# michaelwillett/GPU-ICP-SLAM

Hardware: AMD Instinct MI355X
Metric: particle-scan evals/sec (1081 beams x N particles), full particleFilter step, KD path (higher is better)
Workload: dtype f32; 1 GPU; synthetic 1081-beam scans, 100000 particles/GPU, 100000-point KD map, full SLAM step (disperse+score+weights+ICP/SVD+map update+resample); particles_global=100000, parallelism=particles sharded x1, map replicated, kd_size_end=196248

## Files before the change

### gpu-icp-slam_amd/binding.py

```python
import ctypes as C
import os

import numpy as np

from . import build as _build

NODE_DTYPE = np.dtype(
    [("axis", "<i4"), ("left", "<i4"), ("right", "<i4"), ("parent", "<i4"),
     ("x", "<f4"), ("y", "<f4"), ("z", "<f4"), ("w", "<f4")])
PARTICLE_DTYPE = np.dtype(
    {"names": ["x", "y", "theta", "w", "cluster", "map"],
     "formats": ["<f4", "<f4", "<f4", "<f4", "u1", "<u8"],
     "offsets": [0, 4, 8, 12, 16, 24], "itemsize": 32})

SYMBOLS = [
    "pfslam_default_config", "pfslam_create", "pfslam_destroy", "pfslam_last_error", "pfslam_device_count",
    "pfslam_set_stream", "pfslam_synchronize", "pfslam_step", "pfslam_step_grid", "pfslam_shard_disperse", "pfslam_shard_score", "pfslam_shard_weights", "pfslam_shard_finish", "pfslam_shard_stream", "pfslam_get_pose", "pfslam_get_particles",
    "pfslam_get_map", "pfslam_get_grid", "pfslam_get_trace", "pfslam_get_cells", "pfslam_set_map",
    "pfslam_set_particles", "pfslam_shift_particles", "pfslam_set_scan", "pfslam_set_pose", "pfslam_set_grid", "pfslam_motion_update",
    "pfslam_score_kd", "pfslam_measurement_update", "pfslam_icp", "pfslam_update_map_kd", "pfslam_resample",
    "pfslam_score_grid", "pfslam_update_map_grid", "pfslam_traverse", "pfslam_measurement_local",
    "pfslam_measurement_apply", "pfslam_device_ptr", "pfslam_time_score_kd", "pfslam_set_variant", "pfslam_set_lag",
    "pfslam_kd_create", "pfslam_kd_insert_list", "pfslam_kd_insert_node", "pfslam_kd_balance", "pfslam_set_timing", "pfslam_get_timers", "pfslam_resample_plan", "pfslam_resample_gather", "pfslam_maybe_balance", "pfslam_kd_size", "pfslam_topology_update", "pfslam_find_walls",
    "pfslam_check_loop_closure", "pfslam_get_topology", "pfslam_set_topology", "pfslam_get_closures", "pfslam_score_census", "pfslam_set_census", "pfslam_get_census_log", "pfslam_ubench_gather", "pfslam_plan_stats", "pfslam_cell_stats", "pfslam_kd_parallel_sort", "pfslam_kd_sort_threads", "pfslam_kd_whole_node",
    "pfslam_set_serial", "pfslam_set_trig", "pfslam_debug_check_cells", "pfslam_set_probe", "pfslam_get_probe", "pfslam_probe_name", "pfslam_frame_mode",
    "pfslam_time_score_grid", "pfslam_set_shard_balance", "pfslam_shard_balance_due", "pfslam_shard_balance_build", "pfslam_shard_balance_adopt",
]


class Config(C.Structure):
    _fields_ = [("n_particles", C.c_int32), ("n_beams", C.c_int32),
                ("map_scale_x", C.c_float), ("map_scale_y", C.c_float),
                ("map_res_x", C.c_float), ("map_res_y", C.c_float),
                ("kd_capacity", C.c_int32), ("device", C.c_int32),
                ("strict_host_mirror", C.c_int32), ("free_upload_bug", C.c_int32),
                ("balance_period", C.c_int32), ("global_offset", C.c_int32), ("global_n", C.c_int32),
                ("shard_stride", C.c_int32), ("reserved_", C.c_int32 * 2)]


class PfSlamError(RuntimeError):
    pass


_lib = None


def _one_hip_runtime():
    import importlib.util
    import sys
    if "torch" in sys.modules or os.environ.get("PFSLAM_NO_TORCH_HIP"):
        return
    try:
        spec = importlib.util.find_spec("torch")
    except Exception:
        spec = None
    if spec is None or not spec.origin:
        return
    cand = os.path.join(os.path.dirname(spec.origin), "lib", "libamdhip64.so")
    if os.path.exists(cand):
        try:
            C.CDLL(cand, mode=C.RTLD_GLOBAL)
        except OSError:
            pass


def load():
    global _lib
    if _lib is not None:
        return _lib
    path = os.environ.get("PFSLAM_LIB") or _build.LIB
    try:
        if path == _build.LIB and _build.stale():
            _build.build()
    except Exception as e:
        if not os.path.exists(path):
            raise PfSlamError("libpfslam_hip.so is missing and could not be built: %s" % e)
    _one_hip_runtime()
    L = C.CDLL(path)
    vp, i32, f32 = C.c_void_p, C.c_int, C.c_float
    L.pfslam_last_error.restype = C.c_char_p
    L.pfslam_default_config.restype = None
    L.pfslam_default_config.argtypes = [vp]
    L.pfslam_create.argtypes = [vp, vp]
    L.pfslam_destroy.argtypes = [vp]
    L.pfslam_set_stream.argtypes = [vp, vp]
    L.pfslam_synchronize.argtypes = [vp]
    L.pfslam_step.argtypes = [vp, i32, vp]
    L.pfslam_step_grid.argtypes = [vp, i32, vp]
    L.pfslam_shard_disperse.argtypes = [vp, i32, vp, vp]
    L.pfslam_shard_score.argtypes = [vp]
    L.pfslam_shard_weights.argtypes = [vp]
    L.pfslam_shard_finish.argtypes = [vp]
    L.pfslam_shard_stream.argtypes = [vp, i32, vp]
    L.pfslam_time_score_grid.argtypes = [vp, i32, vp, vp]
    L.pfslam_set_shard_balance.argtypes = [vp, i32]
    L.pfslam_shard_balance_due.argtypes = [vp, i32, vp, vp]
    L.pfslam_shard_balance_build.argtypes = [vp, i32]
    L.pfslam_shard_balance_adopt.argtypes = [vp]
    L.pfslam_get_pose.argtypes = [vp, vp]
    L.pfslam_get_particles.argtypes = [vp, vp, vp]
    L.pfslam_get_map.argtypes = [vp, vp, vp]
    L.pfslam_get_grid.argtypes = [vp, vp, vp, vp]
    L.pfslam_get_trace.argtypes = [vp, vp]
    L.pfslam_get_cells.argtypes = [vp, i32, vp, i32, vp]
    L.pfslam_set_map.argtypes = [vp, vp, i32]
    L.pfslam_set_particles.argtypes = [vp, vp, i32]
    L.pfslam_set_scan.argtypes = [vp, vp, i32]
    L.pfslam_shift_particles.argtypes = [vp, vp]
    L.pfslam_set_pose.argtypes = [vp, vp]
    L.pfslam_set_grid.argtypes = [vp, vp, i32, i32]
    L.pfslam_motion_update.argtypes = [vp, i32]
    L.pfslam_score_kd.argtypes = [vp, vp]
    L.pfslam_measurement_update.argtypes = [vp, vp, vp, vp]
    L.pfslam_icp.argtypes = [vp, vp, vp, vp]
    L.pfslam_update_map_kd.argtypes = [vp]
    L.pfslam_resample.argtypes = [vp, i32, vp, vp]
    L.pfslam_resample_plan.argtypes = [vp, i32, vp, vp]
    L.pfslam_resample_gather.argtypes = [vp]
    L.pfslam_maybe_balance.argtypes = [vp, i32]
    L.pfslam_kd_size.argtypes = [vp]
    L.pfslam_topology_update.argtypes = [vp, vp]
    L.pfslam_find_walls.argtypes = [vp, vp, vp, vp]
    L.pfslam_check_loop_closure.argtypes = [vp, vp, i32, vp]
    L.pfslam_get_topology.argtypes = [vp, vp, i32, vp, vp]
    L.pfslam_set_topology.argtypes = [vp, i32]
    L.pfslam_get_closures.argtypes = [vp, vp, i32, vp]
    L.pfslam_score_census.argtypes = [vp, vp]
    L.pfslam_set_census.argtypes = [vp, i32]
    L.pfslam_get_census_log.argtypes = [vp, vp, i32, vp]
    L.pfslam_ubench_gather.argtypes = [vp, vp]
    L.pfslam_plan_stats.argtypes = [vp, vp]
    L.pfslam_cell_stats.argtypes = [vp, vp]
    L.pfslam_set_serial.argtypes = [vp, i32]
    L.pfslam_set_trig.argtypes = [vp, i32]
    L.pfslam_debug_check_cells.argtypes = [vp, vp]
    L.pfslam_set_probe.argtypes = [vp, i32]
    L.pfslam_get_probe.argtypes = [vp, vp, i32, vp, vp]
    L.pfslam_frame_mode.argtypes = [vp, vp]
    L.pfslam_probe_name.argtypes = [i32]
    L.pfslam_probe_name.restype = C.c_char_p
    L.pfslam_score_grid.argtypes = [vp, vp]
    L.pfslam_update_map_grid.argtypes = [vp]
    L.pfslam_traverse.argtypes = [vp, vp, i32, vp]
    L.pfslam_measurement_local.argtypes = [vp]
    L.pfslam_measurement_apply.argtypes = [vp, vp, vp, vp]
    L.pfslam_device_ptr.argtypes = [vp, i32, vp, vp]
    L.pfslam_time_score_kd.argtypes = [vp, i32, vp]
    L.pfslam_set_variant.argtypes = [vp, i32]
    L.pfslam_set_lag.argtypes = [vp, i32]
    L.pfslam_kd_create.argtypes = [vp, i32, vp]
    L.pfslam_kd_insert_node.argtypes = [vp, vp, i32]
    L.pfslam_kd_insert_list.argtypes = [vp, i32, vp, i32, i32]
    L.pfslam_kd_balance.argtypes = [vp, i32]
    L.pfslam_debug_math.argtypes = [vp, i32, vp, i32, vp]
    L.pfslam_set_timing.argtypes = [vp, i32]
    L.pfslam_get_timers.argtypes = [vp, vp]
    _lib = L
    return L


def _p(a):
    return a.ctypes.data_as(C.c_void_p)


def _chk(rc, what=""):
    if rc != 0:
        raise PfSlamError("%s failed: %s" % (what, load().pfslam_last_error().decode()))


def device_count():
    return load().pfslam_device_count()


def kd_create(points_xyzw):
    pts = np.ascontiguousarray(points_xyzw, dtype=np.float32).reshape(-1, 4)
    out = np.zeros(len(pts), dtype=NODE_DTYPE)
    _chk(load().pfslam_kd_create(_p(pts), len(pts), _p(out)), "pfslam_kd_create")
    return out


def kd_insert_node(nodes, size, p4):
    p = np.ascontiguousarray(p4, dtype=np.float32)
    _chk(load().pfslam_kd_insert_node(_p(p), _p(nodes), size), "pfslam_kd_insert_node")


def kd_balance(nodes, size):
    _chk(load().pfslam_kd_balance(_p(nodes), size), "pfslam_kd_balance")


MGPU_SYMBOLS = ["pfslam_mgpu_make_id", "pfslam_mgpu_create", "pfslam_mgpu_destroy", "pfslam_mgpu_step", "pfslam_mgpu_barrier_max",
                "pfslam_mgpu_stats", "pfslam_mgpu_time_collectives", "pfslam_mgpu_last_error"]
MGPU_ID_BYTES = 256
_mgpu = None


def load_mgpu():
    global _mgpu
    if _mgpu is not None:
        return _mgpu
    load()
    path = os.path.join(os.path.dirname(os.path.abspath(__file__)), "host", "libpfslam_mgpu.so")
    if not os.path.exists(path):
        import subprocess
        subprocess.check_call(["make", "-C", os.path.dirname(path), "libpfslam_mgpu.so"], stdout=subprocess.DEVNULL)
    M = C.CDLL(path, mode=C.RTLD_GLOBAL)
    vp, i32 = C.c_void_p, C.c_int32
    M.pfslam_mgpu_last_error.restype = C.c_char_p
    M.pfslam_mgpu_make_id.argtypes = [vp]
    M.pfslam_mgpu_create.argtypes = [vp, i32, i32, vp, vp]
    M.pfslam_mgpu_destroy.argtypes = [vp]
    M.pfslam_mgpu_step.argtypes = [vp, i32, vp]
    M.pfslam_mgpu_barrier_max.argtypes = [vp, vp]
    M.pfslam_mgpu_stats.argtypes = [vp, vp]
    M.pfslam_mgpu_time_collectives.argtypes = [vp, i32, vp]
    _mgpu = M
    return M


# ... 182 lines not shown
        return did.value, neff.value

    def maybe_balance(self, frame):
        _chk(self.L.pfslam_maybe_balance(self._h, frame), "pfslam_maybe_balance")

    @property
    def kd_size(self):
        return self.L.pfslam_kd_size(self._h)

    def topology_update(self):
        n = C.c_int()
        _chk(self.L.pfslam_topology_update(self._h, C.byref(n)), "pfslam_topology_update")
        return n.value

    def find_walls(self, a_xy, b_xy):
        a = np.ascontiguousarray(a_xy, np.float32); b = np.ascontiguousarray(b_xy, np.float32)
        n = C.c_int()
        _chk(self.L.pfslam_find_walls(self._h, _p(a), _p(b), C.byref(n)), "pfslam_find_walls")
        return n.value

    def check_loop_closure(self, cap=4096):
        pairs = np.zeros((cap, 2), np.int32)
        n = C.c_int()
        _chk(self.L.pfslam_check_loop_closure(self._h, _p(pairs), cap, C.byref(n)), "pfslam_check_loop_closure")
        return pairs[:min(n.value, cap)].copy()

    def set_topology(self, enable=True):
        _chk(self.L.pfslam_set_topology(self._h, int(enable)), "pfslam_set_topology")

    def closures(self, cap=65536):
        pairs = np.zeros((cap, 2), np.int32)
        n = C.c_int()
        _chk(self.L.pfslam_get_closures(self._h, _p(pairs), cap, C.byref(n)), "pfslam_get_closures")
        return pairs[:min(n.value, cap)].copy()

    def topology(self, cap=4096):
        nodes = np.zeros((cap, 3), np.float32)
        n, idx = C.c_int(), C.c_int()
        _chk(self.L.pfslam_get_topology(self._h, _p(nodes), cap, C.byref(n), C.byref(idx)), "pfslam_get_topology")
        return nodes[:n.value].copy(), idx.value

    def score_census(self):
        out = (C.c_ulonglong * 8)()
        _chk(self.L.pfslam_score_census(self._h, out), "pfslam_score_census")
        return {"trips": int(out[0]), "visits": int(out[1]), "tests": int(out[2]), "test_lanes": int(out[3]),
                "uniform_trips": int(out[4]), "prefix_trips": int(out[5]), "redescents": int(out[6]), "redescents_noop": int(out[7])}

    def set_census(self, enable=True):
        _chk(self.L.pfslam_set_census(self._h, int(enable)), "pfslam_set_census")

    def census_log(self, cap=1024):
        out = np.zeros((cap, 8), np.uint64)
        n = C.c_int()
        _chk(self.L.pfslam_get_census_log(self._h, _p(out), cap, C.byref(n)), "pfslam_get_census_log")
        keys = ("trips", "visits", "tests", "test_lanes", "uniform_trips", "prefix_trips", "redescents", "redescents_noop")
        return [dict(zip(keys, (int(v) for v in row))) for row in out[:min(n.value, cap)]]

    def plan_stats(self):
        out = (C.c_double * 10)()
        _chk(self.L.pfslam_plan_stats(self._h, out), "pfslam_plan_stats")
        keys = ("rows", "path_len", "candidates", "frac_complete", "frac_no_plan", "frac_full", "box_dx", "box_dy", "box_dtheta", "waves")
        return dict(zip(keys, [float(v) for v in out]))

    def cell_stats(self):
        out = (C.c_double * 16)()
        _chk(self.L.pfslam_cell_stats(self._h, out), "pfslam_cell_stats")
        keys = ("cells", "rows", "candidates", "redescent_candidates", "cells_without_row", "pool_slots", "window_kx", "window_ky",
                "walked_from_root", "extended", "reused", "claimed", "flags", "updates", "wipes", "suspended")
        return dict(zip(keys, [float(v) for v in out]))

    def set_serial(self, on):
        _chk(self.L.pfslam_set_serial(self._h, int(on)), "pfslam_set_serial")

    def check_cells(self):
        out = (C.c_longlong * 16)()
        _chk(self.L.pfslam_debug_check_cells(self._h, out), "pfslam_debug_check_cells")
        keys = ("records", "unwalked", "fresh", "published", "row_words", "pending_words", "fallback_words", "dead",
                "v_unwalked_not_pending", "v_unpublished_word", "v_row_outside_alloc", "v_row_not_candidate", "v_watched_link_has_child",
                "v_bad_link", "v_dead_has_row", "v_counters")
        d = dict(zip(keys, [int(v) for v in out]))
        d["violations"] = sum(v for k, v in d.items() if k.startswith("v_"))
        return d

    def set_trig(self, devlib):
        _chk(self.L.pfslam_set_trig(self._h, 1 if devlib else 0), "pfslam_set_trig")

    def frame_mode(self):
        out = (C.c_int * 4)()
        _chk(self.L.pfslam_frame_mode(self._h, out), "pfslam_frame_mode")
        return {"round5_frame": bool(out[0]), "gates": bool(out[1]), "serial": bool(out[2]), "publish_lag": int(out[3])}

    def set_probe(self, frames):
        _chk(self.L.pfslam_set_probe(self._h, int(frames)), "pfslam_set_probe")

    def probe(self, frames=4096):
        buf = np.zeros((frames, 32), np.uint64)
        n, last = C.c_int(0), C.c_int(0)
        _chk(self.L.pfslam_get_probe(self._h, _p(buf), frames, C.byref(n), C.byref(last)), "pfslam_get_probe")
        names = []
        for k in range(32):
            s = self.L.pfslam_probe_name(k).decode()
            if not s:
                break
            names.append(s)
        t = buf[:n.value, :len(names)].astype(np.float64) * 0.01
        return names, t, last.value

    def ubench_gather(self):
        out = (C.c_double * 4)()
        _chk(self.L.pfslam_ubench_gather(self._h, out), "pfslam_ubench_gather")
        return {"wave_gathers_per_s": out[0], "cus": int(out[1]), "nominal_ghz": out[2], "cycles_per_wave_gather": out[3]}

    def resample_plan(self, frame):
        did, neff = C.c_int(), C.c_float()
        _chk(self.L.pfslam_resample_plan(self._h, frame, C.byref(did), C.byref(neff)), "pfslam_resample_plan")
        return did.value, neff.value

    def resample_gather(self):
        _chk(self.L.pfslam_resample_gather(self._h), "pfslam_resample_gather")

    def score_grid(self):
        fit = np.empty(self.n, np.int32)
        _chk(self.L.pfslam_score_grid(self._h, _p(fit)), "pfslam_score_grid")
        return fit

    def update_map_grid(self):
        _chk(self.L.pfslam_update_map_grid(self._h), "pfslam_update_map_grid")

    def step(self, frame, scan):
        scan = np.ascontiguousarray(scan, dtype=np.float32)
        _chk(self.L.pfslam_step(self._h, frame, _p(scan)), "pfslam_step")

    def shard_disperse(self, frame, scan):
        scan = np.ascontiguousarray(scan, dtype=np.float32)
        seeded = C.c_int(0)
        _chk(self.L.pfslam_shard_disperse(self._h, frame, _p(scan), C.byref(seeded)), "pfslam_shard_disperse")
        return bool(seeded.value)

    def shard_score(self):
        _chk(self.L.pfslam_shard_score(self._h), "pfslam_shard_score")

    def shard_weights(self):
        _chk(self.L.pfslam_shard_weights(self._h), "pfslam_shard_weights")

    def shard_finish(self):
        _chk(self.L.pfslam_shard_finish(self._h), "pfslam_shard_finish")

    def shard_stream(self, which):
        st = C.c_void_p(0)
        _chk(self.L.pfslam_shard_stream(self._h, which, C.byref(st)), "pfslam_shard_stream")
        return st.value or 0

    def set_shard_balance(self, external):
        _chk(self.L.pfslam_set_shard_balance(self._h, 1 if external else 0), "pfslam_set_shard_balance")

    def shard_balance_due(self, frame):
        due, n = C.c_int(0), C.c_int(0)
        _chk(self.L.pfslam_shard_balance_due(self._h, frame, C.byref(due), C.byref(n)), "pfslam_shard_balance_due")
        return bool(due.value), n.value

    def shard_balance_build(self, frame):
        _chk(self.L.pfslam_shard_balance_build(self._h, frame), "pfslam_shard_balance_build")

    def shard_balance_adopt(self):
        _chk(self.L.pfslam_shard_balance_adopt(self._h), "pfslam_shard_balance_adopt")

# ... 62 lines not shown
```

### gpu-icp-slam_amd/csrc/kd_cells.hip.inc

```

#define PF_CELL_SUB 2
#define PF_CELL_WIN (2560 * PF_CELL_SUB)
#define PF_CELL_LIST_CAP (1 << 19)
#define PF_CELL_POOL_CAP (1 << 22)
#define PF_CELL_MAXC 12
#define PF_CELL_RUN 32
#define PF_CELL_MAXR 14
#define PF_CELL_MARK_MAX 4096
#define PF_CELL_PENDING 0xFFFFFFFFu
#define PF_CELL_FALLBACK 0xFFFFFFFEu
enum { PF_CS_COUNT = 0, PF_CS_POOL, PF_CS_SNAP, PF_CS_PAD3, PF_CS_LIST_CAP, PF_CS_POOL_CAP, PF_CS_FLAGS, PF_CS_PAD, PF_CS_ROWS, PF_CS_N1, PF_CS_N2,
       PF_CS_NONE, PF_CS_CUR_FRESH, PF_CS_CUR_EXT, PF_CS_CUR_REUSED, PF_CS_CUR_CLAIMED, PF_CS_WORDS = 32,
       PF_CS_OX = 128, PF_CS_OY = 129, PF_CS_ALLOC = 256 };
#define PF_CF_LIST_FULL 1
#define PF_CF_POOL_FULL 2
#define PF_CF_NEED_ORIGIN 4
#define PF_CF_FAR 8
#define PF_CELL_DRIFT_MAX 120
#define PF_REC_WORDS 96
#define PF_REC_TERM 4
#define PF_REC_CAND 20
#define PF_REC_PAR 36
#define PF_REC_RC 52
#define PF_REC_POOL 76
#define PF_REC_LAST 80
#define PF_ROW_HEADROOM 2
#define PF_RF_FRESH 1
#define PF_RF_DEAD 2
#define PF_RF_ROVER 4

struct CellGeom { float resx, resy, invx, invy; };

__device__ __forceinline__ void pf_stamp(unsigned long long *__restrict__ slot)
{
    if (slot && blockIdx.x == 0 && blockIdx.y == 0 && threadIdx.x == 0) *slot = wall_clock64();
}

#define PF_LATTICE_KMAX (1 << 20)
__host__ __device__ __forceinline__ int lattice_floor(float q, float res, float inv)
{
    int k = (int)floorf(q * inv);
    if ((float)(k + 1) * res <= q) k++;
    else if (!((float)k * res <= q)) k--;
    return k;
}

__host__ __device__ __forceinline__ int sub_index(float q, float res, float inv)
{
    const int k = lattice_floor(q, res, inv);
    const float mid = (float)k * res + 0.5f * res;
    return PF_CELL_SUB * k + (q >= mid ? 1 : 0);
}
#define PF_SUB_MARGIN 3e-7f
__device__ __forceinline__ int sub_index_fast(float q, float inv2, float &clear)
{
    const float t = q * inv2;
    int k;
    asm("v_cvt_flr_i32_f32 %0, %1" : "=v"(k) : "v"(t));
    const float fr = __builtin_amdgcn_fractf(t);
    clear = __builtin_fmaf(fabsf(t), -PF_SUB_MARGIN, 0.5f - 1e-6f) - fabsf(fr - 0.5f);
    return k;
}
__host__ __device__ __forceinline__ void sub_edges(int S, float res, float &lo, float &hi, float &cell_lo)
{
    const int k = S >> 1;
    cell_lo = (float)k * res;
    const float mid = cell_lo + 0.5f * res;
    lo = (S & 1) ? mid : cell_lo;
    hi = (S & 1) ? (float)(k + 1) * res : mid;
}
static_assert(PF_CELL_SUB == 2, "sub_index / sub_edges halve the lattice cell");

__device__ __forceinline__ bool beam_box(const pf::KdGroupBox &b, int j, float r, float &wxlo, float &wxhi, float &wylo, float &wyhi,
                                         const pf::AngleParts *T = nullptr, const pf::BeamParts *beams = nullptr)
{
    const float tc = 0.5f * (b.tlo + b.thi), dth = 0.5f * (b.thi - b.tlo);
    float cx, cy;
    if (T) beam_end_point(beams, j, r, tc, *T, cx, cy);
    else pf::clean_lidar_scan(j, r, tc, cx, cy);
    const float dd = dth + 1e-6f;
    const float eps = 2e-4f + 1e-5f * fabsf(r) + fabsf(r) * 2.0f * 1.1920929e-7f * (fabsf(tc) + 2.4f + dd);
    const float hx = (fabsf(cy) + fabsf(r) * dd) * dd + eps, hy = (fabsf(cx) + fabsf(r) * dd) * dd + eps;
    wxlo = b.xlo + cx - hx; wxhi = b.xhi + cx + hx; wylo = b.ylo + cy - hy; wyhi = b.yhi + cy + hy;
    return (wxlo == wxlo) && (wxhi == wxhi) && (wylo == wylo) && (wyhi == wyhi) && fabsf(wxlo) < 1e6f && fabsf(wxhi) < 1e6f &&
           fabsf(wylo) < 1e6f && fabsf(wyhi) < 1e6f && (wxhi - wxlo) < 4.0f && (wyhi - wylo) < 4.0f && fabsf(r) < PF_RANGE_NEVER;
}

#define PF_MARK_THREADS 256
#define PF_MARK_GROUPS 8
#define PF_MARK_CLAIMS 2048
#define PF_MARK_WORDS 4096
__global__ __launch_bounds__(PF_MARK_THREADS) void k_cells_mark(const pf::KdGroupBox *__restrict__ box, int groups,
                                                                const float *__restrict__ scan, int nb, CellGeom geo, unsigned *tab,
                                                                int *__restrict__ list, int *cs, const pf::AngleParts *__restrict__ gparts,
                                                                const pf::BeamParts *__restrict__ beams, unsigned long long *__restrict__ probe = nullptr)
{
    pf_stamp(probe);
    __shared__ unsigned bm[PF_MARK_WORDS];
    __shared__ int s_red[4][PF_MARK_THREADS / 64];
    const int t = threadIdx.x, lane = t & 63, wave = t >> 6, j = blockIdx.x;
    const int ox = cs[PF_CS_OX], oy = cs[PF_CS_OY];
    const float r = scan[j];
    int kx0[PF_MARK_GROUPS], kx1[PF_MARK_GROUPS], ky0[PF_MARK_GROUPS], ky1[PF_MARK_GROUPS];
    int ux0 = INT_MAX, ux1 = INT_MIN, uy0 = INT_MAX, uy1 = INT_MIN;
#pragma unroll
    for (int q = 0; q < PF_MARK_GROUPS; q++) {
        const int g = blockIdx.y * (PF_MARK_THREADS * PF_MARK_GROUPS) + q * PF_MARK_THREADS + t;
        kx0[q] = ky0[q] = INT_MAX;
        kx1[q] = ky1[q] = INT_MIN;
// ... 13 lines not shown
    }
    for (int off = 32; off >= 1; off >>= 1) {
        ux0 = min(ux0, __shfl_xor(ux0, off, 64)); ux1 = max(ux1, __shfl_xor(ux1, off, 64));
        uy0 = min(uy0, __shfl_xor(uy0, off, 64)); uy1 = max(uy1, __shfl_xor(uy1, off, 64));
    }
    if (lane == 0) { s_red[0][wave] = ux0; s_red[1][wave] = ux1; s_red[2][wave] = uy0; s_red[3][wave] = uy1; }
    __syncthreads();
    for (int k = 0; k < PF_MARK_THREADS / 64; k++) {
        ux0 = min(ux0, s_red[0][k]); ux1 = max(ux1, s_red[1][k]); uy0 = min(uy0, s_red[2][k]); uy1 = max(uy1, s_red[3][k]);
    }
    if (ux0 > ux1) return;
    const int nx = ux1 - ux0 + 1;
    const long long bits = (long long)nx * (uy1 - uy0 + 1);
    __shared__ int s_claim[PF_MARK_CLAIMS];
    __shared__ int s_nclaim, s_base;
    if (t == 0) s_nclaim = 0;
    __syncthreads();
    auto claim = [&](int idx) {
        if (atomicCAS(&tab[idx], 0u, PF_CELL_PENDING) == 0u) {
            const int k = atomicAdd(&s_nclaim, 1);
            if (k < PF_MARK_CLAIMS) s_claim[k] = idx;
            else {
                const int pos = atomicAdd(&cs[PF_CS_COUNT], 1);
                if (pos < cs[PF_CS_LIST_CAP]) list[pos] = idx;
                else {
                    atomicExch(&tab[idx], PF_CELL_FALLBACK);
                    atomicOr(&cs[PF_CS_FLAGS], PF_CF_LIST_FULL);
                }
            }
        }
    };
    auto flush = [&]() {
        __syncthreads();
        const int nc = min(s_nclaim, PF_MARK_CLAIMS);
        if (t == 0 && nc > 0) {
            s_base = atomicAdd(&cs[PF_CS_COUNT], nc);
            atomicAdd(&cs[PF_CS_CUR_CLAIMED], nc);
        }
        __syncthreads();
        for (int k = t; k < nc; k += PF_MARK_THREADS) {
            const int pos = s_base + k;
            if (pos < cs[PF_CS_LIST_CAP]) list[pos] = s_claim[k];
            else {
                atomicExch(&tab[s_claim[k]], PF_CELL_FALLBACK);
                atomicOr(&cs[PF_CS_FLAGS], PF_CF_LIST_FULL);
            }
        }
    };
    if (bits > (long long)PF_MARK_WORDS * 32) {
#pragma unroll
        for (int q = 0; q < PF_MARK_GROUPS; q++) {
            if (kx0[q] > kx1[q] || (long long)(kx1[q] - kx0[q] + 1) * (ky1[q] - ky0[q] + 1) > PF_CELL_MARK_MAX) continue;
            for (int cy = ky0[q]; cy <= ky1[q]; cy++)
                for (int cx = kx0[q]; cx <= kx1[q]; cx++) claim(2 * cy * PF_CELL_WIN + 2 * cx);
        }
        flush();
        return;
    }
    const int words = (int)((bits + 31) >> 5);
    for (int w = t; w < words; w += PF_MARK_THREADS) bm[w] = 0u;
    __syncthreads();
#pragma unroll
    for (int q = 0; q < PF_MARK_GROUPS; q++)
        for (int cy = ky0[q]; cy <= ky1[q]; cy++) {
            const int b0 = (cy - uy0) * nx - ux0 + kx0[q], b1 = b0 + (kx1[q] - kx0[q]);
            for (int w = b0 >> 5; w <= (b1 >> 5); w++) {
                const int lo = max(b0 - (w << 5), 0), hi = min(b1 - (w << 5), 31);
                const unsigned m = (0xFFFFFFFFu >> (31 - hi)) & (0xFFFFFFFFu << lo);
                if ((bm[w] & m) != m) atomicOr(&bm[w], m);
            }
        }
    __syncthreads();
    for (int bit = t; bit < (int)bits; bit += PF_MARK_THREADS)
        if ((bm[bit >> 5] >> (bit & 31)) & 1u) {
            const int cy = bit / nx;
            claim(2 * (uy0 + cy) * PF_CELL_WIN + 2 * (ux0 + (bit - cy * nx)));
        }
    flush();
}

#define PF_CORNER_F 0.999996f
#define PF_CELL_MAXU 16
#define PF_CELL_MAXRU 24
static_assert(PF_REC_RC + PF_CELL_MAXRU <= PF_REC_POOL && PF_REC_POOL + 2 <= PF_REC_LAST && PF_REC_LAST + 4 <= PF_REC_WORDS && PF_REC_CAND == PF_REC_TERM + PF_CELL_MAXU && PF_REC_PAR == PF_REC_CAND + PF_CELL_MAXU && PF_REC_RC == PF_REC_PAR + PF_CELL_MAXU, "record layout");
__device__ __forceinline__ int link_child(const pf::KdView &t, int link)
{
    const int a = link >> 1;
    const uint4 nd = t.hot[a];
    if ((link & 1) == 0 && t.planar && (nd.z >> 30) == 2u) return __float_as_int(t.z[a]);
    return (link & 1) ? (int)nd.w : pf::hot_left(nd.z);
}
#define PF_CELL_FILTER_WORDS 1024
__device__ __forceinline__ unsigned pf_link_hash(int link) { return ((unsigned)link * 2654435761u) >> 17; }
__device__ __forceinline__ int watched_child(const pf::KdView &t, int link)
{
    const uint4 nd = t.hot[link >> 1];
    return (link & 1) ? (int)nd.w : pf::hot_left(nd.z);
}
#ifdef PF_CELLS_PROFILE
#define PF_STAMP(p)                                                                      \
    do {                                                                                 \
        if (PUBLISH) {                                                                   \
            const long long now_ = (long long)wall_clock64();                            \
            if (lane == 0) {                                                             \
                atomicAdd(&cs[64 + 2 * (p)], (int)(now_ - t_prev_));                     \
                atomicMax(&cs[65 + 2 * (p)], (int)(now_ - t_prev_));                     \
            }                                                                            \
            t_prev_ = now_;                                                              \
        }                                                                                \
    } while (0)
#else
#define PF_STAMP(p)
#endif
struct CellPass { const int *lo; int *w_out; const int *hi; const int *bound; int fault; };
template <bool PUBLISH>
__global__ __launch_bounds__(64) void k_cells_update(pf::KdView tree, CellGeom geo, unsigned *tab, const int *__restrict__ list, int *cs,
                                                     uint4 *__restrict__ pool, int *rec_base, int gen, const int *__restrict__ touched, int pass = 0, int recut = 0, int use_snap = 0,
                                                     CellPass cp = CellPass{nullptr, nullptr, nullptr, nullptr, 0}, unsigned long long *__restrict__ probe = nullptr,
                                                     int *__restrict__ signal_word = nullptr, int signal_ticket = 0)
{
    pf_stamp(probe);
    if (signal_word && blockIdx.x == 0 && threadIdx.x == 0) __hip_atomic_store(signal_word, signal_ticket, __ATOMIC_RELEASE, __HIP_MEMORY_SCOPE_AGENT);
    __shared__ int lds[184][64];
#define S_IDX(k) lds[(k)][lane]
#define S_LB(k) (*(float *)&lds[32 + (k)][lane])
#define S_CX(k) (*(float *)&lds[16 + (k)][lane])
#define S_CY(k) (*(float *)&lds[32 + (k)][lane])
#define S_PP(k) (*(uint32_t *)&lds[48 + (k)][lane])
#define S_PC(k) (*(float *)&lds[64 + (k)][lane])
#define S_CT(k) lds[80 + (k)][lane]
#define S_PI(k) lds[96 + (k)][lane]
#define S_R(k) lds[112 + (k)][lane]
#define S_RX(k) (*(float *)&lds[136 + (k)][lane])
#define S_RY(k) (*(float *)&lds[160 + (k)][lane])
    static_assert(PF_CELL_RUN == 32 && PF_CELL_MAXU == 16 && PF_CELL_MAXRU == 24, "LDS layout of k_cells_update");
    __shared__ unsigned s_filter[PF_CELL_FILTER_WORDS];
    const int n_touched = (PUBLISH && touched) ? touched[0] : 0;
    if (PUBLISH && n_touched > 0) {
        for (int w = threadIdx.x; w < PF_CELL_FILTER_WORDS; w += 64) s_filter[w] = 0u;
        __syncthreads();
        for (int k = threadIdx.x; k < n_touched; k += 64) {
            const unsigned hsh = pf_link_hash(touched[1 + k]);
            atomicOr(&s_filter[hsh >> 5], 1u << (hsh & 31));
        }
        __syncthreads();
    }
    auto maybe_touched = [&](int link) -> bool {
        const unsigned hsh = pf_link_hash(link);
        return (s_filter[hsh >> 5] >> (hsh & 31)) & 1u;
    };
    const int lane = threadIdx.x;
    int count = min(cs[PF_CS_COUNT], cs[PF_CS_LIST_CAP]);
    if ((!PUBLISH || use_snap == 2) && threadIdx.x == 0) cs[PF_CS_SNAP] = count;
    if (PUBLISH && use_snap == 1) count = min(count, cs[PF_CS_SNAP]);
    if (PUBLISH && cp.hi && cp.fault != 1) count = min(count, *cp.hi);
    const int first = (!PUBLISH && cp.lo) ? min(*cp.lo, count) : 0;
    const int bound = cp.bound ? *cp.bound : 0x7fffffff;
    if (cp.w_out && threadIdx.x == 0) *cp.w_out = count;
    const int ox = cs[PF_CS_OX], oy = cs[PF_CS_OY];
    int st_rows = 0, st_n1 = 0, st_n2 = 0, st_none = 0, st_fresh = 0, st_ext = 0, st_reused = 0;
#ifdef PF_CELLS_PROFILE
    long long t_prev_ = (long long)wall_clock64();
    const long long t_start_ = t_prev_;
    if (PUBLISH && lane == 0 && blockIdx.x * 64 < count) atomicAdd(&cs[63], 1);
#endif
    auto bounds = [](float xlo, float xhi, float ylo, float yhi, float nx, float ny, float &lb, float &ub) {
        const float dxn = fmaxf(fmaxf(xlo - nx, nx - xhi), 0.0f), dyn = fmaxf(fmaxf(ylo - ny, ny - yhi), 0.0f);
        const float dxf = fmaxf(fabsf(nx - xlo), fabsf(nx - xhi)), dyf = fmaxf(fabsf(ny - ylo), fabsf(ny - yhi));
        lb = (dxn * dxn + dyn * dyn) * 0.99999f;
        ub = (dxf * dxf + dyf * dyf) * 1.00001f;
    };
    auto corner4 = [](float px, float py, float ixlo, float ixhi, float iylo, float iyhi, float d[4]) {
        const float x0 = (px - ixlo) * (px - ixlo), x1 = (px - ixhi) * (px - ixhi), y0 = (py - iylo) * (py - iylo), y1 = (py - iyhi) * (py - iyhi);
        d[0] = x0 + y0; d[1] = x1 + y0; d[2] = x0 + y1; d[3] = x1 + y1;
    };
    auto unbook = [&](unsigned old) {
        if (old == PF_CELL_FALLBACK) st_none--;
        else if (old != 0u && old < 0x40000000u) {
            st_rows--;
            st_n1 -= (int)(old & 15u);
            st_n2 -= ((old >> 4) & 15u) == 15u ? 0 : (int)((old >> 4) & 15u);
        }
    };
    for (int base = first + blockIdx.x * 64; base < count; base += gridDim.x * 64) {
        const int r = base + lane;
        const bool in = r < count;
        int *rec = rec_base + (size_t)(in ? r : 0) * PF_REC_WORDS;
        const int4 hd = in ? *(const int4 *)rec : make_int4(0, 0, 0, gen);
        int4 pre_ct[4], pre_cand[4], pre_par[4], pre_rc[6];
        int2 pre_pool = make_int2(0, 0);
        int4 pre_last = make_int4(0, 0, 0, 0);
        int pre_cell = 0;
        constexpr bool HOIST = PUBLISH;
        if (HOIST) {
#pragma unroll
            for (int q = 0; q < 4; q++) pre_ct[q] = pre_cand[q] = pre_par[q] = make_int4(-1, -1, -1, -1);
#pragma unroll
            for (int q = 0; q < 6; q++) pre_rc[q] = make_int4(0, 0, 0, 0);
            if (in) {
#pragma unroll
                for (int q = 0; q < 4; q++) {
                    pre_ct[q] = *(const int4 *)(rec + PF_REC_TERM + 4 * q);
                    pre_cand[q] = *(const int4 *)(rec + PF_REC_CAND + 4 * q);
                    pre_par[q] = *(const int4 *)(rec + PF_REC_PAR + 4 * q);
                }
#pragma unroll
                for (int q = 0; q < 6; q++) pre_rc[q] = *(const int4 *)(rec + PF_REC_RC + 4 * q);
                pre_pool = *(const int2 *)(rec + PF_REC_POOL);
                pre_last = *(const int4 *)(rec + PF_REC_LAST);
                pre_cell = list[r];
            }
        }
        const bool scratch = in && hd.w != gen;
        bool work = scratch;
        int m_old = 0, nr = 0, rflags = 0, term0 = -1, child0 = -1;
        float U = INFINITY;
        if (PUBLISH && in && !scratch) {
            U = __int_as_float(hd.x);
            term0 = hd.y;
            m_old = hd.z & 0xff;
            nr = (hd.z >> 8) & 0xff;
            rflags = hd.z >> 16;
            if (!(rflags & PF_RF_DEAD)) {
                int ct[PF_CELL_MAXU];
#pragma unroll
                for (int q = 0; q < PF_CELL_MAXU / 4; q++) {
                    const int4 v = HOIST ? pre_ct[q] : *(const int4 *)(rec + PF_REC_TERM + 4 * q);
                    ct[4 * q] = v.x; ct[4 * q + 1] = v.y; ct[4 * q + 2] = v.z; ct[4 * q + 3] = v.w;
                }
                const bool direct = (rflags & PF_RF_FRESH) != 0 && cp.fault != 2;
                bool changed = false;
                if (direct || n_touched > 0) {
                    if (direct || maybe_touched(term0)) child0 = watched_child(tree, term0);
                    changed = child0 >= 0;
                }
#pragma unroll
                for (int k = 0; k < PF_CELL_MAXU; k++)
                    if (k < m_old) {
                        int c = -1;
                        if (ct[k] >= 0 && (direct || (n_touched > 0 && maybe_touched(ct[k])))) c = watched_child(tree, ct[k]);
                        S_CT(k) = c >= 0 ? -c - 2 : ct[k];
                        changed |= c >= 0;
                    }
                work = changed || (rflags & PF_RF_FRESH) != 0 || recut != 0;
                if (changed && !(rflags & PF_RF_FRESH)) st_ext++;
                if (!work) st_reused++;
            }
        }
        PF_STAMP(0);
        if (__builtin_amdgcn_ballot_w64(work) == 0ull) continue;
        const bool active = in && work;
        if (!active) m_old = nr = 0;
        if (active && scratch) st_fresh++;
        const int cell = HOIST ? pre_cell : (in ? list[r] : 0);
        const int cyw = cell / PF_CELL_WIN, cxw = cell - cyw * PF_CELL_WIN;
        const int Kx = (ox + cxw) >> 1, Ky = (oy + cyw) >> 1;
        const float cxlo = (float)Kx * geo.resx, cxhi = (float)(Kx + 1) * geo.resx, xmid = cxlo + 0.5f * geo.resx;
        const float cylo = (float)Ky * geo.resy, cyhi = (float)(Ky + 1) * geo.resy, ymid = cylo + 0.5f * geo.resy;
        int n = 0, old_off = 0, old_len = 0;
        if (active && !scratch) {
            old_off = HOIST ? pre_pool.x : rec[PF_REC_POOL];
            old_len = recut ? 0 : (HOIST ? pre_pool.y : rec[PF_REC_POOL + 1]);
#pragma unroll
            for (int g4 = 0; g4 < PF_CELL_MAXU / 4; g4++) {
                const int k0 = 4 * g4;
                if (k0 < m_old) {
                    const int4 ci = HOIST ? pre_cand[g4] : *(const int4 *)(rec + PF_REC_CAND + k0);
                    const int4 pi = HOIST ? pre_par[g4] : *(const int4 *)(rec + PF_REC_PAR + k0);
                    const int cv[4] = {ci.x, ci.y, ci.z, ci.w}, pv[4] = {pi.x, pi.y, pi.z, pi.w};
#pragma unroll
                    for (int q = 0; q < 4; q++)
                        if (k0 + q < m_old) {
                            S_IDX(k0 + q) = cv[q];
                            S_LB(k0 + q) = 0.0f;
                            S_PI(k0 + q) = pv[q];
                        }
                }
            }
#pragma unroll
            for (int g4 = 0; g4 < PF_CELL_MAXRU / 4; g4++) {
                const int k0 = 4 * g4;
                if (k0 < nr) {
                    const int4 rv = HOIST ? pre_rc[g4] : *(const int4 *)(rec + PF_REC_RC + k0);
                    const int rw[4] = {rv.x, rv.y, rv.z, rv.w};
#pragma unroll
                    for (int q = 0; q < 4; q++)
                        if (k0 + q < nr) S_R(k0 + q) = rw[q];
                }
            }
            n = m_old;
        }
        int head = !active ? -1 : scratch ? 0 : child0;
        bool give_up = false;
        uint4 nd = tree.hot[max(head, 0)];
        while (head >= 0) {
            int cl = pf::hot_left(nd.z), cr = (int)nd.w;
            if (cl >= bound) cl = -1;
            if (cr >= bound) cr = -1;
            uint4 ndl = nd, ndr = nd;
            if (cl >= 0) ndl = tree.hot[cl];
            if (cr >= 0) ndr = tree.hot[cr];
            const float nx = __uint_as_float(nd.x), ny = __uint_as_float(nd.y);
            const uint32_t axis = nd.z >> 30;
            if (!(fabsf(nx) < 1e6f && fabsf(ny) < 1e6f)) { give_up = true; break; }
            float lb, ub;
            bounds(cxlo, cxhi, cylo, cyhi, nx, ny, lb, ub);
            U = fminf(U, ub);
            if (lb <= U) {
                if (n == PF_CELL_RUN) {
                    int m = 0;
                    for (int k = 0; k < PF_CELL_RUN; k++) {
                        const int ci = S_IDX(k);
                        const float cl = S_LB(k);
                        if (cl <= U) {
                            S_IDX(m) = ci;
                            S_LB(m) = cl;
                            m++;
                        }
                    }
                    n = m;
                    if (n == PF_CELL_RUN) { give_up = true; break; }
                }
                S_IDX(n) = head;
                S_LB(n) = lb;
                n++;
            }
            const bool lt = axis == 0 ? cxlo < nx : (axis == 1 ? cylo < ny : false);
            term0 = head * 2 + (lt ? 0 : 1);
            head = lt ? cl : cr;
            nd = lt ? ndl : ndr;
        }
        PF_STAMP(1);
        int m = 0;
        if (!give_up)
            for (int k = 0; k < n; k++)
                if (S_LB(k) <= U) S_IDX(m++) = S_IDX(k);
        bool dead = active && (give_up || m == 0 || m > PF_CELL_MAXU);
        if (dead || !active) m = 0;
        if (dead) m_old = nr = 0;
        auto parent_plane = [&](int k, const uint4 pn) {
            const uint32_t paxis = pn.z >> 30;
            const bool none = S_PI(k) < 0;
            S_PP(k) = none ? 3u << 30 : paxis << 30;
            S_PC(k) = none ? 0.0f : __uint_as_float(paxis == 0 ? pn.x : pn.y);
        };
        for (int k0 = 0; k0 < max(m, nr); k0 += 4) {
            uint4 cn[4], pn[4], rn[4];
            int par[4];
#pragma unroll
            for (int q = 0; q < 4; q++) {
                const int k = k0 + q;
                if (k < m) {
                    const int ci = S_IDX(k);
                    cn[q] = tree.hot[ci];
                    if (k >= m_old) par[q] = tree.parent[ci];
                    else pn[q] = tree.hot[max(S_PI(k), 0)];
                }
                if (k < nr) rn[q] = tree.hot[S_R(k) & 0x7ffffff];
            }
#pragma unroll
            for (int q = 0; q < 4; q++) {
                const int k = k0 + q;
                if (k < m) {
                    S_CX(k) = __uint_as_float(cn[q].x);
                    S_CY(k) = __uint_as_float(cn[q].y);
                    if (k >= m_old) S_PI(k) = par[q];
                    else parent_plane(k, pn[q]);
                }
                if (k < nr) {
                    S_RX(k) = __uint_as_float(rn[q].x);
                    S_RY(k) = __uint_as_float(rn[q].y);
                }
            }
        }
        PF_STAMP(2);
        if (m > 0 && (m > 1 || m_old > 0)) {
            const uint32_t mask = (1u << m) - 1u;
            uint32_t kept = mask;
            for (int k = 0; k < m_old; k++) {
                float lb, ub;
                bounds(cxlo, cxhi, cylo, cyhi, S_CX(k), S_CY(k), lb, ub);
                if (!(lb <= U)) kept &= ~(1u << k);
            }
            if (m > 1) {
                const float ixlo = nextafterf(cxlo, INFINITY), ixhi = nextafterf(cxhi, -INFINITY), iylo = nextafterf(cylo, INFINITY),
                            iyhi = nextafterf(cyhi, -INFINITY);
                for (int ka = 0; ka < m; ka++) {
// ... 58 lines not shown
                if (k0 + q < m) {
                    const int k = k0 + q, pi = S_PI(k);
                    parent_plane(k, pn[q]);
                    int start = -1, link = -1;
                    if (pi >= 0) {
                        const uint32_t paxis = pn[q].z >> 30;
                        if (paxis == 2) start = __float_as_int(zl[q]);
                        else {
                            const bool plt = (paxis == 0 ? cxlo : cylo) < S_PC(k);
                            link = pi * 2 + (plt ? 1 : 0);
                            start = plt ? (int)pn[q].w : pf::hot_left(pn[q].z);
                        }
                        if (start >= bound) start = -1;
                    }
                    S_CT(k) = start >= 0 ? -start - 2 : link;
                }
        }
        PF_STAMP(3);
        bool r_over = (rflags & PF_RF_ROVER) != 0;
#ifdef PF_CELLS_PROFILE
        const int nr_before_walks_ = nr;
#endif
        {
            int k = -1, h2 = -1, link = -1;
            uint4 nd = make_uint4(0u, 0u, 0u, 0u);
            for (;;) {
                if (h2 < 0 && k < m) {
                    if (k >= 0) S_CT(k) = link;
                    for (k++; k < m && !r_over; k++) {
                        const int c = S_CT(k);
                        if (c <= -2) {
                            h2 = -c - 2;
                            break;
                        }
                    }
                    if (r_over) k = m;
                    if (k < m) nd = tree.hot[h2];
                }
                if (__builtin_amdgcn_ballot_w64(k < m) == 0ull) break;
                if (k < m) {
                    int cl = pf::hot_left(nd.z), cr = (int)nd.w;
                    if (cl >= bound) cl = -1;
                    if (cr >= bound) cr = -1;
                    uint4 ndl = nd, ndr = nd;
                    if (cl >= 0) ndl = tree.hot[cl];
                    if (cr >= 0) ndr = tree.hot[cr];
                    const float nx = __uint_as_float(nd.x), ny = __uint_as_float(nd.y);
                    const uint32_t axis = nd.z >> 30;
                    float lb, ub;
                    bounds(cxlo, cxhi, cylo, cyhi, nx, ny, lb, ub);
                    if (lb <= U || !(fabsf(nx) < 1e6f && fabsf(ny) < 1e6f)) {
                        if (nr == PF_CELL_MAXRU) r_over = true;
                        else {
                            S_R(nr) = h2 | (k << 27);
                            S_RX(nr) = nx;
                            S_RY(nr) = ny;
                            nr++;
                        }
                    }
                    const bool lt = axis == 0 ? cxlo < nx : (axis == 1 ? cylo < ny : false);
                    link = h2 * 2 + (lt ? 0 : 1);
                    h2 = lt ? cl : cr;
                    nd = lt ? ndl : ndr;
                    if (r_over) { h2 = -1; k = m; }
                }
            }
        }
        PF_STAMP(4);
#ifdef PF_CELLS_PROFILE
        if (PUBLISH && active && !scratch && !(rflags & PF_RF_FRESH) && !recut) {
            atomicAdd(&cs[60], 1);
            if (m == m_old && nr == nr_before_walks_) atomicAdd(&cs[61], 1);
        }
#endif
        if (active) {
            const int fl = (dead ? PF_RF_DEAD : 0) | (r_over ? PF_RF_ROVER : 0) | (PUBLISH ? 0 : PF_RF_FRESH);
            *(int4 *)rec = make_int4(__float_as_int(U), term0, m | (nr << 8) | (fl << 16), gen);
            for (int k = 0; k < m; k++) {
                rec[PF_REC_CAND + k] = S_IDX(k);
                rec[PF_REC_TERM + k] = r_over ? -1 : S_CT(k);
                rec[PF_REC_PAR + k] = S_PI(k);
            }
            for (int k = 0; k < nr; k++) rec[PF_REC_RC + k] = S_R(k);
            if (!PUBLISH) rec[PF_REC_POOL] = rec[PF_REC_POOL + 1] = 0;
        }
        PF_STAMP(5);
        if (!PUBLISH) continue;
        float Ub[4] = {INFINITY, INFINITY, INFINITY, INFINITY};
        uint32_t keep[4] = {0u, 0u, 0u, 0u};
        int mb[4], rb[4] = {0, 0, 0, 0}, total = 0;
        const float bxlo[4] = {cxlo, xmid, cxlo, xmid}, bxhi[4] = {xmid, cxhi, xmid, cxhi}, bylo[4] = {cylo, cylo, ymid, ymid}, byhi[4] = {ymid, ymid, cyhi, cyhi};
        for (int k = 0; k < m; k++) {
            const float px = S_CX(k), py = S_CY(k);
#pragma unroll
            for (int b4 = 0; b4 < 4; b4++) {
                float lb, ub;
                bounds(bxlo[b4], bxhi[b4], bylo[b4], byhi[b4], px, py, lb, ub);
                Ub[b4] = fminf(Ub[b4], ub);
            }
        }
        for (int k = 0; k < m; k++) {
            const float px = S_CX(k), py = S_CY(k);
#pragma unroll
            for (int b4 = 0; b4 < 4; b4++) {
                float lb, ub;
                bounds(bxlo[b4], bxhi[b4], bylo[b4], byhi[b4], px, py, lb, ub);
                if (lb <= Ub[b4]) keep[b4] |= 1u << k;
            }
        }
#pragma unroll
        for (int b4 = 0; b4 < 4; b4++) {
            const uint32_t mask = keep[b4];
            uint32_t kept = mask;
            if (mask & (mask - 1u)) {
                const float ixlo = nextafterf(bxlo[b4], INFINITY), ixhi = nextafterf(bxhi[b4], -INFINITY), iylo = nextafterf(bylo[b4], INFINITY),
                            iyhi = nextafterf(byhi[b4], -INFINITY);
                for (uint32_t ra = mask; ra; ra &= ra - 1u) {
                    const int ka = __ffs(ra) - 1;
                    float a[4];
                    corner4(S_CX(ka), S_CY(ka), ixlo, ixhi, iylo, iyhi, a);
                    for (uint32_t rc = mask & ~(1u << ka); rc; rc &= rc - 1u) {
                        const int kc = __ffs(rc) - 1;
                        float c[4];
                        corner4(S_CX(kc), S_CY(kc), ixlo, ixhi, iylo, iyhi, c);
                        if (c[0] < a[0] * PF_CORNER_F && c[1] < a[1] * PF_CORNER_F && c[2] < a[2] * PF_CORNER_F && c[3] < a[3] * PF_CORNER_F) {
                            kept &= ~(1u << ka);
                            break;
                        }
                    }
                }
            }
            keep[b4] = kept;
        }
        for (int k = 0; k < nr; k++) {
            const float rx = S_RX(k), ry = S_RY(k);
            const int ow = (S_R(k) >> 27) & 15;
#pragma unroll
            for (int b4 = 0; b4 < 4; b4++) {
                float lb, ub;
                bounds(bxlo[b4], bxhi[b4], bylo[b4], byhi[b4], rx, ry, lb, ub);
                rb[b4] += (lb <= Ub[b4] || !(lb == lb)) && ((keep[b4] >> ow) & 1u);
            }
        }
#pragma unroll
        for (int b4 = 0; b4 < 4; b4++) {
            int mm = __popc(keep[b4]);
            if (r_over || rb[b4] > PF_CELL_MAXR) rb[b4] = 15;
            if (mm > PF_CELL_MAXC) mm = 0;
            mb[b4] = mm;
            total += mm ? mm + (rb[b4] == 15 ? 0 : rb[b4]) : 0;
        }
        PF_STAMP(6);
        const bool in_place = active && total <= old_len;
        const int alloc = (!active || in_place || total == 0) ? 0 : total + PF_ROW_HEADROOM;
        int incl = alloc;
        for (int off = 1; off < 64; off <<= 1) {
            const int u = __shfl_up(incl, off, 64);
            if (lane >= off) incl += u;
        }
        const int wave_total = __shfl(incl, 63, 64);
        int wave_base = 0;
        if (lane == 0 && wave_total > 0) wave_base = atomicAdd(&cs[PF_CS_POOL], wave_total);
        wave_base = __shfl(wave_base, 0, 64);
        int off = in_place ? old_off : wave_base + incl - alloc;
        PF_STAMP(7);
        if (!active) continue;
        const bool pool_full = !in_place && off + alloc > cs[PF_CS_POOL_CAP];
        if (pool_full && total > 0) atomicOr(&cs[PF_CS_FLAGS], PF_CF_POOL_FULL);
        rec[PF_REC_POOL] = pool_full ? 0 : off;
        rec[PF_REC_POOL + 1] = pool_full ? 0 : (in_place ? old_len : alloc);
        unsigned word[4];
#pragma unroll
        for (int b4 = 0; b4 < 4; b4++) {
            if (mb[b4] == 0 || pool_full) {
                word[b4] = PF_CELL_FALLBACK;
                st_none++;
                continue;
            }
            const float xlo = bxlo[b4], xhi = bxhi[b4], ylo = bylo[b4], yhi = byhi[b4];
            const float u = Ub[b4];
            const uint32_t kept = keep[b4];
            int w = off;
            for (int k = 0; k < m; k++)
                if ((kept >> k) & 1u)
                    pool[w++] = make_uint4(__float_as_uint(S_CX(k)), __float_as_uint(S_CY(k)), (uint32_t)S_IDX(k) | S_PP(k),
                                           __float_as_uint(S_PC(k)));
            if (rb[b4] != 15)
                for (int k = 0; k < nr; k++) {
                    float lb, ub;
                    const int e = S_R(k), ow = (e >> 27) & 15;
                    bounds(xlo, xhi, ylo, yhi, S_RX(k), S_RY(k), lb, ub);
                    if ((lb <= u || !(lb == lb)) && ((kept >> ow) & 1u))
                        pool[w++] = make_uint4(__float_as_uint(S_RX(k)), __float_as_uint(S_RY(k)), (uint32_t)(e & 0x7ffffff),
                                               (uint32_t)S_IDX(ow));
                }
            word[b4] = ((uint32_t)off << 8) | ((uint32_t)rb[b4] << 4) | (uint32_t)mb[b4];
            off = w;
            st_rows++;
            st_n1 += mb[b4];
            st_n2 += rb[b4] == 15 ? 0 : rb[b4];
        }
        const int4 last_words = HOIST ? pre_last : *(const int4 *)(rec + PF_REC_LAST);
        *(int4 *)(rec + PF_REC_LAST) = make_int4((int)word[0], (int)word[1], (int)word[2], (int)word[3]);
        if (!(scratch || (rflags & PF_RF_FRESH))) {
            const int4 last = last_words;
            unbook((unsigned)last.x); unbook((unsigned)last.y); unbook((unsigned)last.z); unbook((unsigned)last.w);
        }
#pragma unroll
        for (int b4 = 0; b4 < 4; b4++) __hip_atomic_store(&tab[cell + (b4 & 1) + ((b4 & 2) ? PF_CELL_WIN : 0)], word[b4], __ATOMIC_RELAXED, __HIP_MEMORY_SCOPE_AGENT);
        PF_STAMP(8);
    }
#ifdef PF_CELLS_PROFILE
    if (PUBLISH && lane == 0) {
        const int dt = (int)((long long)wall_clock64() - t_start_);
        atomicMax(&cs[96 + (pass & 15)], dt);
        if (dt > 2000) atomicAdd(&cs[112 + (pass & 15)], 1);
    }
#endif
    for (int off = 32; off >= 1; off >>= 1) {
        st_rows += __shfl_xor(st_rows, off, 64); st_n1 += __shfl_xor(st_n1, off, 64);
        st_n2 += __shfl_xor(st_n2, off, 64); st_none += __shfl_xor(st_none, off, 64);
        st_fresh += __shfl_xor(st_fresh, off, 64); st_ext += __shfl_xor(st_ext, off, 64); st_reused += __shfl_xor(st_reused, off, 64);
    }
    if (PUBLISH && probe && lane == 0) atomicMax(probe + (PB_UPDATE_END - PB_UPDATE), (unsigned long long)wall_clock64());
    if (lane == 0) {
        if (st_rows) atomicAdd(&cs[PF_CS_ROWS], st_rows);
        if (st_n1) atomicAdd(&cs[PF_CS_N1], st_n1);
        if (st_n2) atomicAdd(&cs[PF_CS_N2], st_n2);
        if (st_none) atomicAdd(&cs[PF_CS_NONE], st_none);
        if (st_fresh) atomicAdd(&cs[PF_CS_CUR_FRESH], st_fresh);
        if (st_ext) atomicAdd(&cs[PF_CS_CUR_EXT], st_ext);
        if (st_reused) atomicAdd(&cs[PF_CS_CUR_REUSED], st_reused);
    }
}

#undef S_IDX
#undef S_LB
#undef S_CX
#undef S_CY
#undef S_PP
#undef S_PC
#undef S_CT
#undef S_PI
#undef S_R
#undef S_RX
#undef S_RY
__device__ __forceinline__ float cell_dist2(const uint4 cd, float wx, float wy)
{
    typedef float f32x2 __attribute__((ext_vector_type(2)));
    const f32x2 nxy = {__uint_as_float(cd.x), __uint_as_float(cd.y)};
    const f32x2 pxy = {wx, wy};
    const f32x2 d = nxy - pxy;
    const f32x2 dd = d * d;
    return dd.x + dd.y;
}
__device__ __forceinline__ bool cell_visit(const uint4 cd, float wx, float wy, float &sBest)
{
    const float s = cell_dist2(cd, wx, wy);
    const float sGuard = sBest * PF_GUARD_K;
    bool take = s < sGuard;
    const bool inBand = (s < sBest) != take;
    if (__builtin_amdgcn_ballot_w64(inBand) != 0ull) {
        float sb = sBest;
        asm volatile("" : "+v"(sb));
        take = take | (inBand && pf::fsqrt(s) < pf::fsqrt(sb));
    }
    sBest = take ? s : sBest;
    return take;
}

#define PF_ROW_SLACK 4
template <bool CENSUS = false, int GUARD = 1>
__global__ __launch_bounds__(64) void k_score_kd_cells(const float *__restrict__ px, const float *__restrict__ py,
                                                       const float *__restrict__ pth, int n, const float *__restrict__ scan,
                                                       const pf::BeamParts *__restrict__ beams, int nb, int beams_per_chunk, pf::KdView tree,
                                                       CellGeom geo, const unsigned *__restrict__ tab, const uint4 *__restrict__ pool,
                                                       const int *__restrict__ cs, const int *__restrict__ order, int direct,
                                                       float *__restrict__ out, int out_mode, pf::KdCensus *__restrict__ census = nullptr,
                                                       unsigned long long *__restrict__ probe = nullptr, const double2 *__restrict__ tparts = nullptr)
{
    pf_stamp(probe);
    const int g = blockIdx.x, slot = g * 64 + threadIdx.x;
    const int j0 = blockIdx.y * beams_per_chunk;
    const int j1 = min(nb, j0 + beams_per_chunk);
    const bool real = slot < n;
    const int i = order ? order[min(slot, n - 1)] : min(slot, n - 1);
    const float x = px[i], y = py[i], th = pth[i];
    pf::AngleParts T;
    if (tparts) {
        const double2 tp = tparts[i];
        T.c = tp.x;
        T.s = tp.y;
        T.a = (double)th;
    } else T = pf::angle_parts(th);
    const int ox = cs[PF_CS_OX], oy = cs[PF_CS_OY];
    const float inv2x = 2.0f * geo.invx, inv2y = 2.0f * geo.invy;
    const pf::kd_rsrc_t tab_rsrc = pf::kd_rsrc(tab), pool_rsrc = pf::kd_rsrc(pool);
    float acc = 0.0f, wpend = 0.0f;
    pf::KdCensusLocal cl = {0, 0, 0, 0, 0, 0, 0, 0};
    auto stage_a = [&](int j, float &wx, float &wy, unsigned &e) -> bool {
        const float r = scan[j];
        if (!(fabsf(r) < PF_RANGE_NEVER)) return false;
        beam_end_point<GUARD>(beams, j, r, th, T, wx, wy);
        if (!(fabsf(wx) < PF_LIDAR_RANGE && fabsf(wy) < PF_LIDAR_RANGE)) return false;
        wx += x;
        wy += y;
        e = 0u;
        float gx, gy;
        int cx = sub_index_fast(wx, inv2x, gx), cy = sub_index_fast(wy, inv2y, gy);
        const float g = fminf(gx, gy);
        bool ok = g > 0.0f;
        if (__builtin_amdgcn_fcmpf(g, 0.0f, 2 ) != __builtin_amdgcn_ballot_w64(true)) {
            if (!ok && fabsf(wx) < 1e6f && fabsf(wy) < 1e6f) {
                cx = sub_index(wx, geo.resx, geo.invx);
                cy = sub_index(wy, geo.resy, geo.invy);
                float lox, loy, hi, cell_lo;
                sub_edges(cx, geo.resx, lox, hi, cell_lo);
                sub_edges(cy, geo.resy, loy, hi, cell_lo);
                ok = wx != lox && wy != loy;
            }
        }
        cx -= ox;
        cy -= oy;
        if (ok && (unsigned)cx < (unsigned)PF_CELL_WIN && (unsigned)cy < (unsigned)PF_CELL_WIN) {
            if (CENSUS) { unsigned dummy = 0; pf::census_add(cl.uniform, dummy); }
            int off;
            asm("v_mad_u32_u24 %0, %1, %2, %3" : "=v"(off) : "v"(cy), "s"(PF_CELL_WIN * 4), "v"(cx << 2));
            e = (unsigned)pf::kd_load_i32_bytes(tab_rsrc, off);
        }
        return true;
    };
    auto resolve = [&](float wx, float wy, float sBest, int b, int roff, int n2) -> int {
        bool changed = n2 == 15;
        if (n2 != 15) {
            const uint32_t owner = (uint32_t)b;
            for (int k0 = 0; k0 < n2; k0 += 2) {
                uint4 cd[2];
                const int base = (roff + k0) << 4;
#pragma unroll
                for (int q = 0; q < 2; q++) cd[q] = pf::kd_load_hot_at(pool_rsrc, base, q * 16);
                if (CENSUS) for (int q = 0; q < 2; q++) pf::census_add(cl.trips, cl.lanes);
#pragma unroll
                for (int q = 0; q < 2; q++)
                    if (k0 + q < n2 && cd[q].w == owner && cell_visit(cd[q], wx, wy, sBest)) {
                        b = (int)cd[q].z;
                        changed = true;
                    }
            }
        }
        if (changed) {
            if (CENSUS) cl.redesc++;
            b = pf::kd_resume<true, CENSUS>(tree, wx, wy, 0.0f, sBest, b, -1, &cl);
        }
// ... 82 lines not shown
```

### gpu-icp-slam_amd/csrc/pfslam_frame.hip.inc

```

#define PF_FRAME_RING 4
enum { PF_FS_BOUND = 0, PF_FS_WALKED = 4, PF_FS_TICKET = 8, PF_FS_ICP = 9, PF_FS_WORDS = 16 };
enum { PF_WC_WALLS = 0, PF_WC_NEW, PF_WC_FLAGS, PF_WC_SIZE, PF_WC_WORDS = 4 };

enum { PF_FL_REDUCED = 0, PF_FL_TREE, PF_FL_ORDER, PF_FL_ICP, PF_FL_SCAN, PF_FL_FTAIL, PF_FL_POSEG , PF_FL_WORDS = 8 };
__device__ __forceinline__ void flag_store(int *word, int ticket) { __hip_atomic_store(word, ticket, __ATOMIC_RELEASE, __HIP_MEMORY_SCOPE_AGENT); }
__device__ __forceinline__ bool flag_wait(const int *word, int ticket, int *err)
{
    const unsigned long long t0 = wall_clock64(), limit = g_gate_ticks;
    while (__hip_atomic_load(word, __ATOMIC_ACQUIRE, __HIP_MEMORY_SCOPE_AGENT) - ticket < 0) {
        __builtin_amdgcn_s_sleep(8);
        if (wall_clock64() - t0 > limit) {
            if (err) __hip_atomic_store(err, ticket, __ATOMIC_RELAXED, __HIP_MEMORY_SCOPE_SYSTEM);
            return false;
        }
    }
    return true;
}
__global__ void k_gate(const int *__restrict__ word, int ticket, int *__restrict__ err)
{
    if (threadIdx.x == 0) flag_wait(word, ticket, err);
}
__global__ void k_gate_signal(int *__restrict__ done_word, int done_ticket, const int *__restrict__ word, int ticket, int *__restrict__ err)
{
// ... 363 lines not shown
            pend = __syncthreads_or(pend);
        }
        for (int k = threadIdx.x; k < n_ins; k += 1024) {
            const int g = old + k, ax = lax[k];
            const int left = ll[k] == PF_KD_NULL ? -1 : old + (int)ll[k], right = lr[k] == PF_KD_NULL ? -1 : old + (int)lr[k];
            hot[g] = pf::pack_hot(lx[k], ly[k], ax, left, right, planar);
            parent[g] = lpar[k];
            kz[g] = (planar && ax == 2) ? __int_as_float(left) : lz[k];
            kw[g] = -100.0f;
        }
    }
    __syncthreads();
    if (threadIdx.x == 0) {
        if (touched) touched[0] = s_touched;
        const int cf = cell_state ? cell_state[PF_CS_FLAGS] : 0;
        const int cflag = ((cf & PF_CF_FAR) ? PF_HDR_CELLS_WIPE : 0) | ((cf & (PF_CF_LIST_FULL | PF_CF_POOL_FULL)) ? PF_HDR_CELLS_FULL : 0);
        wcounts[PF_WC_WALLS] = n;
        wcounts[PF_WC_NEW] = n_new;
        wcounts[PF_WC_FLAGS] = (full ? PF_HDR_KD_FULL : 0) | cflag;
        wcounts[PF_WC_SIZE] = old + n_ins;
        kd_state[0] = old + n_ins;
        *bound_next = old + n_ins;
        if (probe) probe[PB_WALLS_END - PB_WALLS] = wall_clock64();
    }
}

__global__ __launch_bounds__(64) void k_wall_runs(const float *__restrict__ scan, const pf::BeamParts *__restrict__ beams, int nb, PoseSrc src,
                                                  float *__restrict__ start_out, float *__restrict__ pose_out, long long *__restrict__ stats_next, int cx,
                                                  int cy, int dimx, int dimy, float resx, float resy, uint32_t *__restrict__ runs_g,
                                                  uint32_t *__restrict__ keys_s, unsigned long long *__restrict__ probe, int *__restrict__ flags, int ticket,
                                                  int *__restrict__ gate_err, int wait_poseg, int trig)
{
    pf_stamp(probe);
    const int lane = threadIdx.x;
    if (flags) {
        if (lane == 0) {
            if (blockIdx.x == 0) flag_store(flags + PF_FL_REDUCED, ticket);
            flag_wait(flags + PF_FL_ICP, ticket, gate_err);
            if (wait_poseg) flag_wait(flags + PF_FL_POSEG, ticket, gate_err);
        }
        __syncthreads();
    }
    float ps[3], st[3];
    frame_pose(src, st, ps);
    if (blockIdx.x == 0 && lane == 0) {
        for (int k = 0; k < 3; k++) { start_out[k] = st[k]; pose_out[k] = ps[k]; }
        start_out[3] = 0.0f;
        pose_out[3] = 0.0f;
        stats_next[0] = LLONG_MIN;
        stats_next[1] = LLONG_MIN;
    }
    const float pt = ps[2];
    const pf::AngleParts T = pf::angle_parts(pt);
    const int j = blockIdx.x * 64 + lane;
    uint32_t key = 0xFFFFFFFFu;
    if (j < nb) {
        float wx, wy;
        beam_end_point_rt(beams, j, scan[j], pt, T, wx, wy, trig);
        if (fabsf(wx) < PF_LIDAR_RANGE && fabsf(wy) < PF_LIDAR_RANGE) {
            wx = roundf(pf::fdiv(wx, resx));
            wy = roundf(pf::fdiv(wy, resy));
            wx += (float)cx;
            wy += (float)cy;
            if (wx >= 0 && wx < dimx && wy >= 0 && wy < dimy) key = (uint32_t)(int)(wx * dimx + wy);
        }
    }
#pragma unroll
    for (int k = 2; k <= 64; k <<= 1)
#pragma unroll
        for (int q = k >> 1; q > 0; q >>= 1) {
            const uint32_t other = (uint32_t)__shfl_xor((int)key, q, 64);
            const bool asc = (lane & k) == 0, lower = (lane & q) == 0;
            key = (lower == asc) ? min(key, other) : max(key, other);
        }
    runs_g[j] = key;
    keys_s[j] = 0xFFFFFFFFu;
    if (probe && blockIdx.x == 0 && lane == 0) probe[PB_WALLS_KEYS - PB_WALLS] = wall_clock64();
}

template <bool PLANAR>
__global__ __launch_bounds__(64) void k_walls_rank_traverse(const uint32_t *__restrict__ runs_g, int sort_n, const float *__restrict__ pose, int dimx, float resx,
                                                            float resy, float scalex, float scaley, pf::KdView tree, uint32_t *__restrict__ keys_s,
                                                            float2 *__restrict__ xy_s, int *__restrict__ c2_s, int *__restrict__ leaf_s,
                                                            int *__restrict__ new_s, unsigned long long *__restrict__ probe, int split)
{
    pf_stamp(probe);
    extern __shared__ uint32_t s_dyn[];
    uint32_t *runs = s_dyn;
    const int lane = threadIdx.x, n_runs = sort_n >> 6, mine = blockIdx.x / split, per = 64 / split, pos = (blockIdx.x % split) * per + lane;
    for (int i = lane; i < sort_n; i += 64) runs[i] = runs_g[i];
    __syncthreads();
    if (lane >= per) return;
    const int i = mine * 64 + pos;
    const uint32_t key = runs[i];
    if (key == 0xFFFFFFFFu) return;
    int rank = pos;
    bool dup = pos > 0 && runs[i - 1] == key;
    for (int r0 = 0; r0 < n_runs; r0 += 4) {
        int lo[4] = {0, 0, 0, 0};
        uint32_t pk[4];
        bool on[4];
#pragma unroll
        for (int u = 0; u < 4; u++) {
            const int r = r0 + u;
            on[u] = r < n_runs && r != mine && !(r > mine && key == 0u);
            pk[u] = r < mine ? key : key - 1u;
        }
#pragma unroll
        for (int step = 32; step >= 1; step >>= 1)
#pragma unroll
            for (int u = 0; u < 4; u++)
                if (on[u]) lo[u] += (runs[(r0 + u) * 64 + lo[u] + step - 1] <= pk[u]) ? step : 0;
#pragma unroll
        for (int u = 0; u < 4; u++)
            if (on[u]) {
                const int cnt = lo[u] + ((lo[u] == 63 && runs[(r0 + u) * 64 + 63] <= pk[u]) ? 1 : 0);
                rank += cnt;
                if (r0 + u < mine && cnt > 0 && runs[(r0 + u) * 64 + cnt - 1] == key) dup = true;
            }
    }
    if (dup) return;
    const float4 p = cell_to_point((int)key, dimx, resx, resy, scalex, scaley, pose[0], pose[1]);
    int leaf;
    const int b = pf::kd_resume<PLANAR, false, true>(tree, p.x, p.y, p.z, INFINITY, 0, 0, nullptr, &leaf);
    const float cellDiag = pf::fsqrt(resx * resx + resy * resy), minDist = cellDiag / 2.0f;
    keys_s[rank] = key;
    xy_s[rank] = make_float2(p.x, p.y);
    c2_s[rank] = b;
    leaf_s[rank] = leaf;
    new_s[rank] = node_dist(tree, b, p) > minDist ? 1 : 0;
}

template <bool PLANAR>
__global__ __launch_bounds__(256) void k_free_traverse(float4 *__restrict__ free_pts, int *__restrict__ free_idx, int free_cap, int wall_cap,
                                                       const int *__restrict__ counts, pf::KdView tree, int zero_tail, float *kw, float resx,
                                                       float resy, const int *__restrict__ bound_ptr, unsigned long long *__restrict__ probe)
{
    pf_stamp(probe);
    const int n_wall = min(counts[0], wall_cap), n_free = min(counts[1], free_cap);
    const int bound = *bound_ptr;
    const float cellDiag = pf::fsqrt(resx * resx + resy * resy);
    for (int i = blockIdx.x * 256 + threadIdx.x; i < n_free; i += gridDim.x * 256) {
        float4 p = free_pts[i];
        if (zero_tail && i >= n_wall) {
            p = make_float4(0.0f, 0.0f, 0.0f, 0.0f);
            free_pts[i] = p;
        }
        const int b = pf::kd_resume<PLANAR, false, false, true>(tree, p.x, p.y, p.z, INFINITY, 0, 0, nullptr, nullptr, bound);
        free_idx[i] = b;
        const bool hit = node_dist(tree, b, p) < cellDiag;
        if (zero_tail && i >= n_wall) {
            const unsigned long long m = __ballot(hit);
            if (hit && (int)(threadIdx.x & 63) == __ffsll((long long)m) - 1) map_weight_add(kw, b, PF_FREE_WEIGHT, __popcll(m));
        } else if (hit) map_weight_add(kw, b, PF_FREE_WEIGHT);
    }
}

__global__ __launch_bounds__(1024) void k_wall_weights(const float4 *__restrict__ wall_pts, const int *__restrict__ wall_cell, int wall_cap,
                                                      const int *__restrict__ wall_c2, const int *__restrict__ counts,
                                                      const int *__restrict__ wcounts, pf::KdView tree, float *kw, float resx, float resy,
                                                      const float *__restrict__ pose, HostHeader *__restrict__ hdr, int seq,
                                                      unsigned long long *__restrict__ probe)
{
    pf_stamp(probe);
    const int n_wall = min(counts[0], wall_cap);
    const float cellDiag = pf::fsqrt(resx * resx + resy * resy);
    for (int i = threadIdx.x; i < n_wall; i += 1024) {
        const int b = wall_c2[i];
        if (node_dist(tree, b, wall_pts[i]) < cellDiag) map_weight_add(kw, b, PF_OCCUPIED_WEIGHT);
    }
    if (threadIdx.x != 0 || !hdr) return;
    const int bad = counts[0] != wcounts[PF_WC_WALLS] ? PF_HDR_INTERNAL : 0;
    hdr->n_wall = counts[0];
    hdr->n_free = counts[1];
    hdr->n_new = wcounts[PF_WC_NEW];
    hdr->kd_size = wcounts[PF_WC_SIZE];
    hdr->flags = wcounts[PF_WC_FLAGS] | bad;
    for (int k = 0; k < 4; k++) hdr->pose[k] = pose[k];
    __threadfence_system();
    __hip_atomic_store(&hdr->seq, seq, __ATOMIC_RELEASE, __HIP_MEMORY_SCOPE_SYSTEM);
}

__global__ __launch_bounds__(256) void k_weights_tiles(float *__restrict__ w, float *__restrict__ wm, const float *__restrict__ fit, int n,
                                                       int mirror_count, const long long *__restrict__ stats, float *__restrict__ tile_r,
                                                       float *__restrict__ tile_r2, float *__restrict__ tile_tot,
                                                       unsigned long long *__restrict__ probe)
{
    pf_stamp(probe);
    __shared__ float s_w[PF_SUM_TILE];
    const int t0 = blockIdx.x * PF_SUM_TILE, cnt = min(PF_SUM_TILE, n - t0);
    const long long kmax = stats[0], kmin = stats[1];
    const float fmax = ordered_to_f32((int)(kmax >> 32));
    const float fmin = -ordered_to_f32((int)(kmin >> 32));
    const float rng = fmax - fmin;
    float c = 0.0f;
    int mint = 0;
    if (rng > 0.0f) {
        c = pf::fdiv(1.0f, rng);
        mint = (int)fmin;
    }
    for (int k = threadIdx.x; k < cnt; k += 256) {
        const int i = t0 + k;
        float wi = w[i];
        if (rng > 0.0f) wi = wi * (fit[i] - (float)mint) * c;
        w[i] = wi;
        if (i < mirror_count) wm[i] = wi;
        s_w[k] = wi;
    }
    __syncthreads();
    const int lane = threadIdx.x & 63, wave = threadIdx.x >> 6;
    const int c0 = wave * PF_SCAN_TILE + lane * PF_SCAN_CHUNK;
    if (wave * PF_SCAN_TILE < cnt) {
        float local[PF_SCAN_CHUNK];
// ... 399 lines not shown
}

static int probe_slot_ptr(pfslam_handle *h, int id, unsigned long long **out)
{
    *out = (h->probe && h->probe_frames > 0) ? h->probe + (size_t)(h->cur_seq % h->probe_frames) * PF_PROBE_SLOTS + id : nullptr;
    return 0;
}
#define PB(id) (h->probe ? h->probe + (size_t)(seq % h->probe_frames) * PF_PROBE_SLOTS + (id) : (unsigned long long *)nullptr)

struct FvCtx {
    hipStream_t P, C, F, K;
    int seq, s4, s2, lag, groups, world;
    bool gates, serial, sync_cells, sharded, multi, ftail_gate;
    CellGeom geo;
    pf::KdView tv;
    long long *stats, *stats_next;
    float *sig, *sig_next, *icp_dbg;
    int *order, *fl;
    HostHeader *hdr;
    PoseSrc psrc;
};
static FvCtx fv_ctx(pfslam_handle *h)
{
    FvCtx c;
    const auto &fv = h->fv;
    c.serial = fv.serial;
    c.sync_cells = fv.sync_cells;
    c.sharded = fv.sharded;
    c.world = h->world;
    c.multi = fv.sharded && h->world > 1;
    c.gates = fv.gates;
    c.ftail_gate = fv.ftail_gate;
    c.P = h->stream;
    c.C = c.serial ? c.P : h->aux;
    c.F = c.serial ? c.P : h->fstream;
    c.K = c.serial ? c.P : h->cstream;
    c.seq = h->cur_seq;
    c.s4 = c.seq & 3;
    c.s2 = c.seq & 1;
    c.lag = h->publish_lag;
    c.groups = (h->n + 63) / 64;
    c.geo = CellGeom{h->cfg.map_res_x, h->cfg.map_res_y, 1.0f / h->cfg.map_res_x, 1.0f / h->cfg.map_res_y};
    c.tv = kd_view(h);
    c.stats = h->fstats + 4 * c.s2;
    c.stats_next = h->fstats + 4 * (c.s2 ^ 1);
    c.sig = h->sigr + 80 * c.s4;
    c.sig_next = h->sigr + 80 * ((c.seq + 1) & 3);
    c.order = h->order_ring + (size_t)c.s4 * h->n;
    c.hdr = header_dev(h, c.seq);
    c.fl = h->flags;
    c.icp_dbg = h->icp_dbg + 32 * c.s2;
    c.psrc = PoseSrc{(const long long *)c.stats, h->x_frame, h->y_frame, h->th_frame, (const float *)c.icp_dbg, h->n,
                     c.multi ? (const long long *)h->gkeys : (const long long *)nullptr, c.multi ? (const float *)h->gpose : (const float *)nullptr, h->world, h->stride};
    return c;
}
#define FV_EDGE_WAIT(st, word, ev, back)                                                                                                      \
    do {                                                                                                                                      \
        if (c.gates) {                                                                                                                        \
            hipLaunchKernelGGL(k_gate, dim3(1), dim3(64), 0, st, (const int *)(c.fl + (word)), seq - (back), h->gate_err_dev);                \
            HIPCHK(hipGetLastError());                                                                                                        \
        } else HIPCHK(hipStreamWaitEvent(st, ev, 0));                                                                                         \
    } while (0)

static int fv_cells_passes(pfslam_handle *h, const FvCtx &c)
{
    const int seq = c.seq, s4 = c.s4, groups = c.groups;
    hipStream_t K = c.K;
    const bool mark_early = h->mark_early != 0;
    if (!c.sync_cells) {
        if (mark_early) FV_EDGE_WAIT(K, PF_FL_ORDER, h->ev_order, 0);
        else FV_EDGE_WAIT(K, PF_FL_REDUCED, h->ev_reduced, 0);
    }
    hipLaunchKernelGGL(k_group_box, dim3(groups), dim3(64), 0, K, h->x_frame, h->y_frame, h->th_frame, h->n, (const int *)c.order, h->group_box, h->group_parts, h->d_sigma);
    const int per_block = PF_MARK_THREADS * PF_MARK_GROUPS;
    hipLaunchKernelGGL(k_cells_mark, dim3(h->nb, (groups + per_block - 1) / per_block), dim3(PF_MARK_THREADS), 0, K, (const pf::KdGroupBox *)h->group_box,
                       groups, (const float *)h->scan, h->nb, c.geo, h->cell_tab, h->cell_list, h->cell_state, (const pf::AngleParts *)h->group_parts,
                       (const pf::BeamParts *)h->beam_angle, PB(PB_MARK));
    HIPCHK(hipGetLastError());
    HIPCHK(hipEventRecord(h->ev_marked_r[s4], K));
    if (!c.sync_cells && h->pipe_live) FV_EDGE_WAIT(K, PF_FL_TREE, h->ev_tree2, 1);
    if (c.sync_cells) {
        h->cells_passes++;
        hipLaunchKernelGGL(k_cells_update<true>, dim3(PF_CELLS_GRID), dim3(64), 0, K, c.tv, c.geo, h->cell_tab, (const int *)h->cell_list, h->cell_state, h->cell_pool,
                           h->cell_rec, h->cells_gen, (const int *)nullptr, 0, 0, 0, CellPass{nullptr, nullptr, nullptr, nullptr, 0}, PB(PB_WALK));
        hipLaunchKernelGGL(k_fs_walked, dim3(1), dim3(64), 0, K, h->fs, (const int *)h->cell_state);
    } else {
        hipLaunchKernelGGL(k_cells_update<false>, dim3(PF_CELLS_WALK_GRID), dim3(64), 0, K, c.tv, c.geo, h->cell_tab, (const int *)h->cell_list, h->cell_state,
                           h->cell_pool, h->cell_rec, h->cells_gen, (const int *)nullptr, 0, 0, 0,
                           CellPass{h->fs + PF_FS_WALKED + ((seq - 1) & 3), h->fs + PF_FS_WALKED + s4, nullptr, h->fs + PF_FS_BOUND + s4, 0}, PB(PB_WALK));
    }
    HIPCHK(hipGetLastError());
    HIPCHK(hipEventRecord(h->ev_walked_r[s4], K));
    return 0;
}

static int frame_v2_begin(pfslam_handle *h, int frame, const float *scan_host, int used, int bpc, bool sharded)
{
    CHK(frame_alloc(h));
    if (!h->cell_tab) CHK(cells_alloc(h));
    const int groups = (h->n + 63) / 64;
    if (!h->group_box) CHK(dalloc(&h->group_box, (size_t)groups));
    if (!h->group_parts) CHK(dalloc(&h->group_parts, (size_t)groups));
    {
        const size_t need = (size_t)groups * used * 64;
        if (need > h->pgroup_elems) {
            if (h->pgroup) HIPCHK(hipFree(h->pgroup));
            h->pgroup = nullptr;
            CHK(dalloc(&h->pgroup, need));
            h->pgroup_elems = need;
        }
    }
    bool gates = false;
    CHK(gates_decide(h, &gates));
    const bool sync_cells = h->cells_wipe_pending;
    const bool serial = h->serial != 0 || sync_cells;
    if (!h->pipe_live) {
        CHK(settle(h));
        HIPCHK(hipStreamSynchronize(h->stream));
        HIPCHK(hipStreamSynchronize(h->aux));
        HIPCHK(hipStreamSynchronize(h->cstream));
        HIPCHK(hipStreamSynchronize(h->istream));
        hipLaunchKernelGGL(k_fs_init, dim3(1), dim3(64), 0, h->stream, h->fs, (const int *)h->kd_state,
                           sync_cells ? (const int *)nullptr : (const int *)h->cell_state, h->fstats);
        HIPCHK(hipMemsetAsync(h->sigr, 0, (size_t)PF_FRAME_RING * 80 * 4, h->stream));
        HIPCHK(hipGetLastError());
        h->cloud_valid = false;
        h->shift_pending = false;
        h->icp_forked = h->map_forked = h->walk_pending = h->cells_snap = h->tree_event = h->mark_on_aux = false;
        HIPCHK(hipStreamSynchronize(h->stream));
    } else if (serial) {
        CHK(join_all(h));
    }
    const int seq = ++h->seq;
    h->cur_seq = seq;
    h->cur_frame = frame;
    h->fv.used = used;
    h->fv.bpc = bpc;
    h->fv.frame = frame;
    h->fv.sync_cells = sync_cells;
    h->fv.serial = serial;
    h->fv.sharded = sharded;
    h->fv.gates = gates;
    h->fv.ftail_gate = gates && !serial;
    h->x_frame = h->x; h->y_frame = h->y; h->th_frame = h->th;
    const FvCtx c = fv_ctx(h);
    hipStream_t P = c.P, F = c.F;
    int *fl = c.fl;
    const bool ftail_gate = c.ftail_gate;

    if (sync_cells) CHK(cells_wipe(h));
    {
        const int bits = h->n <= 400000 ? 6 : PF_CELL_BITS_MAX, ncell = 1 << (3 * bits);
        int *hist = h->cells, *cursor = h->cells + ncell, *tile_tot = h->cells + 2 * ncell;
        float *cloud_in = h->cloud + 4 * (c.s2 ^ 1), *cloud_out = h->cloud + 4 * c.s2;
        {
            float *hs = h->h_scan + (size_t)(seq % PF_HDR_SLOTS) * h->nb;
            h->scan = h->scan_base + (size_t)(seq % PF_HDR_SLOTS) * h->nb;
            memcpy(hs, scan_host, (size_t)h->nb * 4);
            scan_reach_of(h, hs);
            if (h->probe && h->probe_frames > 0)
                HIPCHK(hipMemsetAsync(h->probe + (size_t)(seq % h->probe_frames) * PF_PROBE_SLOTS, 0, (size_t)PF_PROBE_SLOTS * 8, P));
            HIPCHK(hipMemcpyAsync(h->scan, hs, (size_t)h->nb * 4, hipMemcpyHostToDevice, P));
            if (gates && !serial) hipLaunchKernelGGL(k_signal, dim3(1), dim3(64), 0, P, fl + PF_FL_SCAN, seq);
        }
        const float reach = h->scan_reach;
        h->tparts_cur = nullptr;
        if (!h->cloud_valid) {
            hipLaunchKernelGGL(k_cloud_seed, dim3(1), dim3(256), 0, P, (const float *)h->x, (const float *)h->y, (const float *)h->th, h->n, reach, cloud_in, c.sig);
            h->cloud_valid = true;
        }
        hipLaunchKernelGGL(k_motion_count, dim3((h->n + 255) / 256), dim3(256), 0, P, h->x, h->y, h->th, h->w, (const float *)h->wm, h->n, frame, h->goff,
// ... 38 lines not shown
static int frame_v2_score(pfslam_handle *h)
{
    const FvCtx c = fv_ctx(h);
    const int seq = c.seq, used = h->fv.used, bpc = h->fv.bpc, groups = c.groups;
    hipStream_t P = c.P, C = c.C;
    if (c.multi) {
        hipLaunchKernelGGL(k_theta_gmax, dim3(std::min(256, (h->world * h->stride + 255) / 256)), dim3(256), 0, P, (const float *)h->gpose, h->world, h->stride, h->gtheta,
                           seq, c.gates ? c.fl + PF_FL_POSEG : (int *)nullptr);
        HIPCHK(hipGetLastError());
        if (!c.gates) HIPCHK(hipEventRecord(h->ev_poseg, P));
    }
    FV_EDGE_WAIT(C, PF_FL_ORDER, h->ev_order, 0);
    hipEvent_t t_a = nullptr, t_b = nullptr;
    if (h->timing) {
        CHK(timer_event(h, &t_a));
        CHK(timer_event(h, &t_b));
        HIPCHK(hipEventRecord(t_a, C));
    }
    const bool guard = !(h->theta_bound < 0.5f * PF_SUM_THETA_MAX) || (c.multi && !h->theta_global_known);
    const dim3 grid64(groups, used);
#define PF_CELLS_ARGS grid64, dim3(64), 0, C, h->x_frame, h->y_frame, h->th_frame, h->n, h->scan, (const pf::BeamParts *)h->beam_angle, h->nb, bpc, c.tv, c.geo, \
                      (const unsigned *)h->cell_tab, (const uint4 *)h->cell_pool, (const int *)h->cell_state, (const int *)c.order, 0
    if (h->trig) hipLaunchKernelGGL((k_score_kd_cells<false, PF_TRIG_DEVLIB>), PF_CELLS_ARGS, (float *)h->pgroup, 4, (pf::KdCensus *)nullptr, PB(PB_SCORE), (const double2 *)nullptr);
    else if (guard) hipLaunchKernelGGL((k_score_kd_cells<false, true>), PF_CELLS_ARGS, (float *)h->pgroup, 4, (pf::KdCensus *)nullptr, PB(PB_SCORE), (const double2 *)nullptr);
    else hipLaunchKernelGGL((k_score_kd_cells<false, false>), PF_CELLS_ARGS, (float *)h->pgroup, 4, (pf::KdCensus *)nullptr, PB(PB_SCORE), (const double2 *)nullptr);
    HIPCHK(hipGetLastError());
    if (t_a) {
        HIPCHK(hipEventRecord(t_b, C));
        h->ev_pending.push_back(pfslam_handle::TimedSpan{t_a, t_b, PF_T_SCORE});
    }
    if (h->census_log && h->census_n < PF_CENSUS_LOG) {
        if (h->trig) hipLaunchKernelGGL((k_score_kd_cells<true, PF_TRIG_DEVLIB>), PF_CELLS_ARGS, (float *)h->pgroup, 2, h->census_log + h->census_n++, (unsigned long long *)nullptr);
        else hipLaunchKernelGGL((k_score_kd_cells<true, true>), PF_CELLS_ARGS, (float *)h->pgroup, 2, h->census_log + h->census_n++, (unsigned long long *)nullptr);
        HIPCHK(hipGetLastError());
    }
#undef PF_CELLS_ARGS
    if (!c.gates) HIPCHK(hipStreamWaitEvent(C, h->ev_icp, 0));
    if (used >= 256)
        hipLaunchKernelGGL((k_reduce_groups<4>), dim3(groups), dim3(256), 0, C, (const short *)h->pgroup, h->n, groups, used, (const int *)c.order, h->fit, c.stats,
                           PB(PB_REDUCE), h->goff);
    else {
        hipLaunchKernelGGL((k_reduce_groups<1>), dim3(std::min((groups + 3) / 4, PF_REDUCE_WGS)), dim3(256), 0, C, (const short *)h->pgroup, h->n, groups, used,
                           (const int *)c.order, h->fit, c.stats, PB(PB_REDUCE), h->goff);
    }
    HIPCHK(hipGetLastError());
    return 0;
}

static int frame_v2_chain(pfslam_handle *h)
{
    const FvCtx c = fv_ctx(h);
    const int seq = c.seq, s4 = c.s4, lag = c.lag;
    hipStream_t P = c.P, C = c.C;
    const bool gates = c.gates, serial = c.serial, sync_cells = c.sync_cells;
    int *fl = c.fl;
    {
        if (!gates) {
            HIPCHK(hipEventRecord(h->ev_reduced, C));
            if (c.multi) HIPCHK(hipStreamWaitEvent(C, h->ev_poseg, 0));
        }
        if (!sync_cells && h->mark_early == 0) CHK(fv_cells_passes(h, c));
        const int sort_n = (h->nb + 63) / 64 * 64;
        const size_t lds = (size_t)sort_n * 9 * sizeof(uint32_t);
        if (!h->walls_attr_set) {
            HIPCHK(hipFuncSetAttribute((const void *)k_walls<0>, hipFuncAttributeMaxDynamicSharedMemorySize, (int)lds));
            HIPCHK(hipFuncSetAttribute((const void *)k_walls<3>, hipFuncAttributeMaxDynamicSharedMemorySize, (int)lds));
            h->walls_attr_set = true;
        }
        const int cx = (int)roundf(0.5f * h->dimx + h->cfg.map_res_x / 2), cy = (int)roundf(0.5f * h->dimy + h->cfg.map_res_y / 2);
        const int wait_poseg = c.multi ? 1 : 0;
#define PF_WALLS_ARGS dim3(1), dim3(1024), lds, C, (const float *)h->scan, (const pf::BeamParts *)h->beam_angle, h->nb, sort_n, c.psrc, h->start, h->pose, c.stats_next, \
                      cx, cy, h->dimx, h->dimy, h->cfg.map_res_x, h->cfg.map_res_y, h->cfg.map_scale_x, h->cfg.map_scale_y, c.tv, h->hot, h->parent, h->kz, h->kw,   \
                      h->kd_state, h->kd_cap, sort_n, h->wall_c2, h->wcounts, h->fs + PF_FS_BOUND + ((seq + 1) & 3), (const int *)h->cell_state, h->cell_touched
        if (h->planar == 0) {
            hipLaunchKernelGGL(k_walls<0>, PF_WALLS_ARGS, PB(PB_WALLS), h->wall_xy2, h->wall_leaf2, h->wall_new2, gates ? fl : (int *)nullptr, seq, h->gate_err_dev,
                               (const uint32_t *)nullptr, (const int *)nullptr, wait_poseg, h->trig);
        } else {
            hipLaunchKernelGGL(k_wall_runs, dim3(sort_n / 64), dim3(64), 0, C, (const float *)h->scan, (const pf::BeamParts *)h->beam_angle, h->nb, c.psrc, h->start, h->pose,
                               c.stats_next, cx, cy, h->dimx, h->dimy, h->cfg.map_res_x, h->cfg.map_res_y, h->wall_runs, h->wall_keys_s, PB(PB_WALLS),
                               gates ? fl : (int *)nullptr, seq, h->gate_err_dev, wait_poseg, h->trig);
            const int walls_split = 4;
            hipLaunchKernelGGL(k_walls_rank_traverse<true>, dim3(sort_n / 64 * walls_split), dim3(64), (size_t)sort_n * 4, C, (const uint32_t *)h->wall_runs, sort_n,
                               (const float *)h->pose, h->dimx, h->cfg.map_res_x, h->cfg.map_res_y, h->cfg.map_scale_x, h->cfg.map_scale_y, c.tv, h->wall_keys_s,
                               h->wall_xy2, h->wall_c2s, h->wall_leaf2, h->wall_new2, PB(PB_WALLS_REP), walls_split);
            hipLaunchKernelGGL(k_walls<3>, PF_WALLS_ARGS, PB(PB_WALLS), h->wall_xy2, h->wall_leaf2, h->wall_new2, (int *)nullptr, seq, (int *)nullptr,
                               (const uint32_t *)h->wall_keys_s, (const int *)h->wall_c2s);
        }
#undef PF_WALLS_ARGS
        HIPCHK(hipGetLastError());
        if (!gates) HIPCHK(hipEventRecord(h->ev_tree2, C));
        const int recut = h->cells_passes > 0 && h->cells_passes % PF_CELLS_RECUT_EVERY == 0 ? 1 : 0;
        if (recut) HIPCHK(hipMemsetAsync(h->cell_state + PF_CS_POOL, 0, 4, C));
        hipLaunchKernelGGL(k_cells_update<true>, dim3(PF_CELLS_GRID), dim3(64), 0, C, c.tv, c.geo, h->cell_tab, (const int *)h->cell_list, h->cell_state, h->cell_pool,
                           h->cell_rec, h->cells_gen, (const int *)h->cell_touched, (int)(h->cells_passes & 15), recut, 0,
                           CellPass{nullptr, nullptr, h->fs + PF_FS_WALKED + ((seq - (sync_cells ? 0 : lag)) & 3), nullptr, h->fault}, PB(PB_UPDATE),
                           gates ? fl + PF_FL_TREE : (int *)nullptr, seq);
        HIPCHK(hipGetLastError());
        h->cells_passes++;
    }
    {
        FV_EDGE_WAIT(P, PF_FL_REDUCED, h->ev_reduced, 0);
        if (!serial) {
            HIPCHK(hipStreamWaitEvent(P, h->ev_marked_r[(seq - 1) & 3], 0));
            HIPCHK(hipStreamWaitEvent(P, h->ev_walked_r[(seq + 1 - lag) & 3], 0));
        }
        if (c.sharded) {
            hipLaunchKernelGGL(k_weights_apply_sharded, dim3((h->n + 255) / 256), dim3(256), 0, P, h->w, h->wm, (const float *)h->fit, h->n, h->goff, mirror_count(h),
                               (const long long *)c.stats, c.multi ? (const long long *)h->gkeys : (const long long *)nullptr, h->world, (const float *)h->gpose, h->stride,
                               h->mkeys, (float *)nullptr, (const float *)nullptr, (float *)nullptr, PB(PB_WEIGHTS));
            HIPCHK(hipGetLastError());
        }
    }
    (void)s4;
    return 0;
}

static int frame_v2_finish(pfslam_handle *h)
{
    const FvCtx c = fv_ctx(h);
    const int seq = c.seq, s4 = c.s4, frame = h->fv.frame;
    hipStream_t P = c.P, F = c.F;
    {
        const double thr = PF_EFFECTIVE_PARTICLES * h->gn;
        if (c.sharded) {
            const int gn = h->gn, n = h->n;
            const int nts = (gn + PF_SUM_TILE - 1) / PF_SUM_TILE, nt = (gn + PF_SCAN_TILE - 1) / PF_SCAN_TILE;
            hipLaunchKernelGGL(k_weight_scan_tiles, dim3(nts), dim3(256), 0, P, (const float *)h->gw, gn, h->tile_r, h->tile_r2, h->tile_tot);
            hipLaunchKernelGGL(k_scan_apply2, dim3(nt), dim3(64), 0, P, (const float *)h->gw, gn, (const float *)h->tile_r, (const float *)h->tile_r2, nts,
                               (const float *)h->tile_tot, h->sums, h->cdf, h->chunk_max, h->tile_pmax, thr, c.hdr, seq, (const long long *)h->mkeys,
                               (const float *)c.sig, PB(PB_APPLY), c.multi ? (const float *)(h->gtheta + s4) : (const float *)nullptr);
            if (c.multi)
                hipLaunchKernelGGL((k_sample_gather<true, true>), dim3((n + 255) / 256), dim3(256), 0, P, (const float *)h->cdf, (const float *)h->chunk_max,
                                   (const float *)h->tile_pmax, gn, n, h->goff, frame, (const float *)h->sums, h->src, (const float *)h->gpose, h->pblk2, h->stride, h->w,
                                   h->wm, thr);
            else
                hipLaunchKernelGGL((k_sample_gather<true, false>), dim3((n + 255) / 256), dim3(256), 0, P, (const float *)h->cdf, (const float *)h->chunk_max,
                                   (const float *)h->tile_pmax, n, n, 0, frame, (const float *)h->sums, h->src, (const float *)h->pblk, h->pblk2, h->stride, h->w,
                                   h->wm, thr);
        } else {
            const int n = h->n;
            if (n <= PF_SUM_TILE) {
                hipLaunchKernelGGL(k_weights_small<float>, dim3(1), dim3(256), 0, P, h->w, h->wm, (const float *)h->fit, n, mirror_count(h), (const long long *)c.stats,
                                   h->x, h->y, h->th, (float *)nullptr, h->sums, (const float *)nullptr, h->pose);
                hipLaunchKernelGGL(k_header_a, dim3(1), dim3(64), 0, P, (const float *)h->sums, (const long long *)c.stats, (const float *)c.sig, c.hdr, seq);
                hipLaunchKernelGGL(k_resample_small, dim3(1), dim3(1024), 0, P, (const float *)h->w, n, h->cdf, h->chunk_max, h->tile_pmax, frame,
                                   (const float *)h->sums, h->src, (const float *)h->pblk, h->pblk2, h->stride, h->w, h->wm, thr);
            } else {
                const int nts = (n + PF_SUM_TILE - 1) / PF_SUM_TILE, nt = (n + PF_SCAN_TILE - 1) / PF_SCAN_TILE;
                hipLaunchKernelGGL(k_weights_tiles, dim3(nts), dim3(256), 0, P, h->w, h->wm, (const float *)h->fit, n, mirror_count(h), (const long long *)c.stats,
                                   h->tile_r, h->tile_r2, h->tile_tot, PB(PB_WEIGHTS));
                hipLaunchKernelGGL(k_scan_apply2, dim3(nt), dim3(64), 0, P, (const float *)h->w, n, (const float *)h->tile_r, (const float *)h->tile_r2, nts,
                                   (const float *)h->tile_tot, h->sums, h->cdf, h->chunk_max, h->tile_pmax, thr, c.hdr, seq, (const long long *)c.stats,
                                   (const float *)c.sig, PB(PB_APPLY));
                hipLaunchKernelGGL((k_sample_gather<true, false>), dim3((n + 255) / 256), dim3(256), 0, P, (const float *)h->cdf, (const float *)h->chunk_max,
                                   (const float *)h->tile_pmax, n, n, 0, frame, (const float *)h->sums, h->src, (const float *)h->pblk, h->pblk2, h->stride, h->w,
                                   h->wm, thr);
            }
        }
        HIPCHK(hipGetLastError());
        swap_pose_blocks(h);
    }
    {
        FV_EDGE_WAIT(F, PF_FL_REDUCED, h->ev_reduced, 0);
        if (c.multi) FV_EDGE_WAIT(F, PF_FL_POSEG, h->ev_poseg, 0);
        const int cx = (int)roundf(0.5f * h->dimx + h->cfg.map_res_x / 2), cy = (int)roundf(0.5f * h->dimy + h->cfg.map_res_y / 2);
        const int M = h->dimx * h->dimy, nblk = (M + 4095) / 4096;
        if (!h->masks_cleared) HIPCHK(hipMemsetAsync(h->free_mask, 0, (size_t)2 * M, F));
        hipLaunchKernelGGL(k_get_walls, dim3((h->nb + 3) / 4), dim3(256), 0, F, h->scan, h->nb, h->pose, cx, cy, h->free_mask, h->wall_mask, h->dimx, h->dimy,
                           h->cfg.map_res_x, h->cfg.map_res_y, 0, c.psrc, h->trig);
        hipLaunchKernelGGL(k_count_cells, dim3(nblk), dim3(256), 0, F, h->free_mask, h->wall_mask, M, h->blk_cnt);
        hipLaunchKernelGGL(k_scatter_cells, dim3(nblk), dim3(256), 0, F, h->free_mask, h->wall_mask, M, h->blk_cnt, h->counts, h->dimx, h->cfg.map_res_x,
                           h->cfg.map_res_y, h->cfg.map_scale_x, h->cfg.map_scale_y, h->pose, h->wall_cell, h->wall_pts, h->max_wall, h->free_cell,
                           h->free_pts, h->max_free, 1, c.psrc);
        h->masks_cleared = true;
        if (h->planar)
            hipLaunchKernelGGL(k_free_traverse<true>, dim3(1024), dim3(256), 0, F, h->free_pts, h->free_c, h->max_free, h->max_wall, (const int *)h->counts, c.tv,
                               h->cfg.free_upload_bug, h->kw, h->cfg.map_res_x, h->cfg.map_res_y, (const int *)(h->fs + PF_FS_BOUND + s4), PB(PB_FREE));
// ... 37 lines not shown
```

### gpu-icp-slam_amd/csrc/pfslam_hip.hip

```cpp
#include "../../include/pfslam.h"
#include "kd_device.h"
#include "pf_math.h"

#include <hip/hip_runtime.h>

#include <algorithm>
#include <atomic>
#include <deque>
#include <thread>
#include <cmath>
#include <cstdio>
#include <chrono>
#include <cstring>
#include <string>
#include <vector>

#define PF_LIDAR_RANGE 20.0f
#define PF_RANGE_NEVER 28.4f
#define PF_FREE_WEIGHT (-1)
#define PF_OCCUPIED_WEIGHT 4
#define PF_EFFECTIVE_PARTICLES .7
#define PF_CLAMP_VAL 113.0f
#define PF_SVD_EPSILON 0.00001f
#define PF_SUM_TILE 4096
// ... 72 lines not shown
    int *order2 = nullptr;
    int *cells = nullptr;
    int64_t *stats = nullptr;
    float *pose = nullptr;
    float *start = nullptr;
    float h_pose[3] = {0, 0, 0};
    float *icp_tar = nullptr, *icp_cor = nullptr, *icp_dbg = nullptr;
    uint8_t *free_mask = nullptr, *wall_mask = nullptr;
    int *blk_cnt = nullptr;
    int *wall_cell = nullptr, *free_cell = nullptr;
    float4 *wall_pts = nullptr, *free_pts = nullptr;
    int *wall_c = nullptr, *free_c = nullptr;
    int *wall_leaf = nullptr;
    int *counts = nullptr;
    int *kd_state = nullptr;
    int max_free = 0, max_wall = 0;
    float *tile_r = nullptr, *tile_r2 = nullptr, *sums = nullptr;
    float *cdf = nullptr, *chunk_max = nullptr, *tile_tot = nullptr, *tile_off = nullptr, *tile_pmax = nullptr;
    int *src = nullptr;
    int8_t *grid = nullptr;
    int32_t *fit_i = nullptr;
    std::vector<int8_t> h_grid;
    struct TopoNode { float x, y, dist; };
    std::vector<TopoNode> topo_nodes{TopoNode{0.0f, 0.0f, 0.0f}};
    std::vector<std::vector<unsigned>> topo_edges{std::vector<unsigned>()};
    unsigned topo_idx = 0;
    int *d_count = nullptr;
    int topo_in_step = 0;
    hipStream_t topo_stream = nullptr;
    std::vector<int32_t> frame_closures;
    HostHeader *h_hdr = nullptr, *hdr_dev = nullptr;
    float *h_scan = nullptr;
    struct Frame { int seq, frame, kind; bool boxes = false; bool v2 = false; bool gtheta = false; };
    std::deque<Frame> in_flight;
    int seq = 0;
    int cur_seq = 0, cur_frame = 0;
    int shard_stage = 0;
    bool shard_v2 = false;
    bool shard_call = false;
    bool theta_global_known = true;
    struct FrameV2 { int used = 0, bpc = 0, frame = 0; bool sync_cells = false, serial = false, sharded = false, gates = false, ftail_gate = false; } fv;
    bool gates_tested = false;
    bool gates_ok = false;
    bool gates_live = false;
    hipEvent_t ev_poseg = nullptr;
    int lag = 1;
    float scan_reach = 8.0f;
    std::vector<pfslam_particle> h_particles;
    std::vector<float> h_tmp;
    int32_t trace[8] = {0};
    hipEvent_t ev0 = nullptr, ev1 = nullptr;
    hipStream_t aux = nullptr;
    hipEvent_t ev_fork = nullptr, ev_join = nullptr;
    hipEvent_t ev_mapfork = nullptr, ev_map = nullptr;
    bool map_forked = false;
    bool scan_front_done = false;
    bool header_packed = false;
    bool lds_attr_set = false;
    bool mirror_stale = false;
    int mirror_n = 0;
    bool icp_forked = false;
    bool icp_delta_ready = false;
    bool masks_cleared = false;
    bool stats_clean = false;
    int timing = 0;
    struct TimedSpan { hipEvent_t a, b; int slot; bool keep_b = false; };
    std::vector<hipEvent_t> ev_pool;
    std::vector<TimedSpan> ev_pending;
    hipEvent_t phase_ev = nullptr;
    double timer_ms[PF_TIMER_SLOTS] = {0};
    long timer_count[PF_TIMER_SLOTS] = {0};
    pf::KdCensus *d_census = nullptr;
    pf::KdCensus *census_store = nullptr, *census_log = nullptr;
    int census_n = 0;
    pf::KdPlanRow *plan = nullptr;
    size_t plan_rows = 0;
    bool plan_valid = false;
    pf::KdGroupBox *group_box = nullptr;
    pf::AngleParts *group_parts = nullptr;
    bool lattice_ok = false;
    bool cells_valid = false;
    unsigned *cell_tab = nullptr;
    int *cell_list = nullptr, *cell_state = nullptr, *cell_rec = nullptr;
    int *cell_touched = nullptr;
    uint4 *cell_pool = nullptr;
    bool cells_wipe_pending = false;
    float cloud_sigma = 0.0f;
    float *d_sigma = nullptr;
    float theta_bound = 0.0f, theta_shift = 0.0f;
    int theta_shift_seq = 0;
    bool cells_suspended = false;
    int cells_full_frame = -1;
    bool balance_external = false;
    int cells_wipe_seq = 0;
    bool score_on_aux = false;
    bool scored_on_aux = false;
    hipEvent_t ev_scored = nullptr;
    bool cells_async = false;
    long cells_wipes = 0;
    long cells_passes = 0;
    int cells_gen = 0;
    hipEvent_t ev_boxes = nullptr;
    hipEvent_t ev_marked = nullptr;
    bool mark_on_aux = false;
    hipStream_t istream = nullptr;
    hipEvent_t ev_tree = nullptr;
    void *pin_tree = nullptr;
    bool tree_event = false;
    hipStream_t cstream = nullptr;
    hipEvent_t ev_walked = nullptr;
    bool walk_pending = false;
    bool update_unsnapped = false;
    bool cells_snap = false;
    pf::BeamParts *beam_angle = nullptr;
    int trig = 0;
    int serial = 0;
    bool pipe_live = false;
    bool cloud_valid = false;
    int publish_lag = 2;
    int *fs = nullptr;
    int *wcounts = nullptr;
    float2 *wall_xy2 = nullptr;
    int *wall_leaf2 = nullptr, *wall_new2 = nullptr;
    int *wall_c2 = nullptr;
    uint32_t *wall_runs = nullptr, *wall_keys_s = nullptr;
    double2 *tparts = nullptr, *tparts_cur = nullptr;
    int *wall_c2s = nullptr;
    long long *fstats = nullptr;
    float *cloud = nullptr;
    float *sigr = nullptr;
    int *order_ring = nullptr;
    short *pgroup = nullptr;
    size_t pgroup_elems = 0;
    hipStream_t fstream = nullptr;
    hipEvent_t ev_reduced = nullptr, ev_tree2 = nullptr, ev_order = nullptr, ev_icp = nullptr, ev_ftail = nullptr, ev_shift = nullptr;
    hipEvent_t ev_marked_r[4] = {nullptr, nullptr, nullptr, nullptr}, ev_walked_r[4] = {nullptr, nullptr, nullptr, nullptr};
    hipEvent_t ev_tail[3] = {nullptr, nullptr, nullptr};
    int fault = 0;
    int stable_order = 0;
    int *order_tmp = nullptr;
    int mark_early = 1;
    int gates = 1;
    bool ftail_recorded = false;
    int *flags = nullptr;
    int *gate_err = nullptr, *gate_err_dev = nullptr;
    const float *x_frame = nullptr, *y_frame = nullptr, *th_frame = nullptr;
    bool shift_pending = false;
    bool balance_done = false;
    bool walls_attr_set = false;
    unsigned long long *probe = nullptr;
    int probe_frames = 0;
};
#define PF_PROBE_SLOTS 32
enum { PB_ICP = 0, PB_MOTION, PB_SCATTER, PB_BOX, PB_MARK, PB_WALK, PB_SCORE, PB_REDUCE, PB_WALLS, PB_UPDATE, PB_WEIGHTS, PB_APPLY, PB_GATHER, PB_RAYS, PB_COUNT,
       PB_LISTS, PB_FREE, PB_WALLW, PB_REDUCE_LAST, PB_WALLS_KEYS, PB_WALLS_SORTED, PB_WALLS_TRAV, PB_WALLS_END, PB_WALLS_REP, PB_ICP_SOLVE, PB_ICP_END, PB_UPDATE_END, PB_REDUCE_END, PB_END };
static const char *const pb_names[PB_END] = {"K icp", "P motion+cells", "P scatter", "K boxes", "K mark", "K walk", "C scan-match", "C reduce", "C walls+insert",
                                             "C cells update", "P weights", "P scan apply", "P sample+gather", "F rays", "F count", "F lists", "F free pass", "F wall weights",
                                             "C reduce: last wg", "C walls: keys", "C walls: sorted", "C walls: traversed", "C walls: end", "C walls: traversal launch", "K icp: solve", "K icp: end", "C cells update: last wg ends", "C reduce: last wg ends"};
static_assert(PB_END <= PF_PROBE_SLOTS, "probe slots");


__global__ __launch_bounds__(256) void k_motion(float *__restrict__ x, float *__restrict__ y,
                                                float *__restrict__ th, float *__restrict__ w,
                                                const float *__restrict__ wm, int n, int frame, int goff, int trig = 0)
{
    int i = blockIdx.x * 256 + threadIdx.x;
// ... 577 lines not shown
}

extern "C" int pfslam_create(const pfslam_config *cfg, pfslam_handle **out)
{
    if (!cfg || !out) return fail("pfslam_create: null argument");
    if (cfg->n_particles <= 0 || cfg->n_beams <= 0 || cfg->kd_capacity <= 0)
        return fail("pfslam_create: n_particles, n_beams and kd_capacity must be positive");
    if (cfg->n_particles > (1 << 24)) return fail("pfslam_create: at most 2^24 particles per handle");
    if (cfg->n_beams > 4096) return fail("pfslam_create: at most 4096 beams per scan (the map insert keeps a frame's new walls in LDS)");
    if (cfg->kd_capacity > PF_KD_MAX_NODES) return fail("pfslam_create: kd_capacity above 2^27 - 1 nodes (32-bit byte offsets of the map records)");
    if (!(cfg->map_res_x > 0.0f && cfg->map_res_y > 0.0f && cfg->map_scale_x > 0.0f && cfg->map_scale_y > 0.0f))
        return fail("pfslam_create: map scale and resolution must be positive");
    {
        const int dx = (int)(cfg->map_scale_x / cfg->map_res_x), dy = (int)(cfg->map_scale_y / cfg->map_res_y);
        if (dx != dy) return fail("pfslam_create: the map must have as many cells in x as in y (reference cell index is x * dim.x + y)");
        if (dx < 2 || dx > 16384) return fail("pfslam_create: map dimensions out of range (2 .. 16384 cells per side)");
    }
    int ndev = 0;
    hipError_t e = hipGetDeviceCount(&ndev);
    if (e != hipSuccess || ndev <= 0)
        return fail(std::string("pfslam_create: no HIP device available (") + hipGetErrorString(e) +
                    "); this library has no CPU fallback");
    if (cfg->device < 0 || cfg->device >= ndev) return fail("pfslam_create: bad device ordinal");
    HIPCHK(hipSetDevice(cfg->device));
    pfslam_handle *h = new pfslam_handle();
    g_live_handles.fetch_add(1);
    h->cfg = *cfg;
    const int rc = create_impl(h);
    if (rc) {
        const std::string msg = g_err;
        pfslam_destroy(h);
        g_err = msg;
        return rc;
    }
    *out = h;
    return 0;
}

extern "C" int pfslam_destroy(pfslam_handle *h)
{
    if (!h) return 0;
    (void)hipSetDevice(h->cfg.device);
    (void)settle(h);
    if (h->stream) (void)hipStreamSynchronize(h->stream);
    void *bufs[] = {h->pblk, h->pblk2, h->w, h->wm, h->gkeys, h->mkeys, h->gtheta, h->scan_base, h->hot, h->parent, h->kz, h->kw,
                    h->fit, h->fit_i, h->partial, h->mkey, h->order2, h->cells, h->stats, h->pose, h->start, h->icp_tar, h->icp_cor, h->icp_dbg,
                    h->free_mask, h->blk_cnt, h->wall_cell, h->free_cell, h->wall_pts, h->free_pts,
                    h->wall_c, h->free_c, h->counts, h->tile_r, h->tile_r2, h->sums, h->cdf,
                    h->chunk_max, h->tile_tot, h->tile_off, h->tile_pmax, h->src, h->grid, h->d_count, h->wall_leaf, h->kd_state, h->d_sigma};
    for (void *b : bufs)
        if (b) (void)hipFree(b);
    if (h->own_global) {
        (void)hipFree(h->gw); (void)hipFree(h->gpose);
    }
    if (h->pin_tree) (void)hipHostFree(h->pin_tree);
    if (h->h_hdr) (void)hipHostFree(h->h_hdr);
    if (h->h_scan) (void)hipHostFree(h->h_scan);
    if (h->ev0) (void)hipEventDestroy(h->ev0);
    if (h->ev1) (void)hipEventDestroy(h->ev1);
    if (h->aux) { (void)hipStreamSynchronize(h->aux); (void)hipStreamDestroy(h->aux); }
    if (h->cstream) { (void)hipStreamSynchronize(h->cstream); (void)hipStreamDestroy(h->cstream); }
    if (h->istream) { (void)hipStreamSynchronize(h->istream); (void)hipStreamDestroy(h->istream); }
    if (h->ev_tree) (void)hipEventDestroy(h->ev_tree);
    if (h->ev_scored) (void)hipEventDestroy(h->ev_scored);
    if (h->ev_walked) (void)hipEventDestroy(h->ev_walked);
    if (h->topo_stream) { (void)hipStreamSynchronize(h->topo_stream); (void)hipStreamDestroy(h->topo_stream); }
    if (h->ev_fork) (void)hipEventDestroy(h->ev_fork);
    if (h->ev_join) (void)hipEventDestroy(h->ev_join);
    if (h->ev_mapfork) (void)hipEventDestroy(h->ev_mapfork);
    if (h->ev_map) (void)hipEventDestroy(h->ev_map);
    for (auto &e : h->ev_pool) (void)hipEventDestroy(e);
    for (auto &e : h->ev_pending) { (void)hipEventDestroy(e.a); if (!e.keep_b) (void)hipEventDestroy(e.b); }
    if (h->phase_ev) (void)hipEventDestroy(h->phase_ev);
    if (h->d_census) (void)hipFree(h->d_census);
    if (h->census_store) (void)hipFree(h->census_store);
    if (h->plan) (void)hipFree(h->plan);
    if (h->group_box) (void)hipFree(h->group_box);
    if (h->group_parts) (void)hipFree(h->group_parts);
    if (h->cell_tab) (void)hipFree(h->cell_tab);
    if (h->cell_list) (void)hipFree(h->cell_list);
    if (h->cell_state) (void)hipFree(h->cell_state);
    if (h->cell_pool) (void)hipFree(h->cell_pool);
    if (h->cell_rec) (void)hipFree(h->cell_rec);
    if (h->cell_touched) (void)hipFree(h->cell_touched);
    if (h->ev_boxes) (void)hipEventDestroy(h->ev_boxes);
    if (h->ev_marked) (void)hipEventDestroy(h->ev_marked);
    if (h->beam_angle) (void)hipFree(h->beam_angle);
    frame_free(h);
    if (h->own_stream && h->stream) (void)hipStreamDestroy(h->stream);
    delete h;
    g_live_handles.fetch_sub(1);
    return 0;
}

extern "C" int pfslam_set_stream(pfslam_handle *h, void *hip_stream)
{
    if (!h) return fail("null handle");
    CHK(settle(h));
    if (h->stream) HIPCHK(hipStreamSynchronize(h->stream));
    if (h->own_stream && h->stream) {
        HIPCHK(hipStreamSynchronize(h->stream));
        HIPCHK(hipStreamDestroy(h->stream));
    }
    h->stream = (hipStream_t)hip_stream;
    h->own_stream = false;
    h->gates_tested = false;
    return 0;
}

extern "C" int pfslam_synchronize(pfslam_handle *h)
{
    if (!h) return fail("null handle");
    CHK(settle(h));
    HIPCHK(hipStreamSynchronize(h->stream));
    return 0;
}

static int flush_timers(pfslam_handle *h)
{
    for (auto &e : h->ev_pending) {
        HIPCHK(hipEventSynchronize(e.b));
        float ms = 0.0f;
        HIPCHK(hipEventElapsedTime(&ms, e.a, e.b));
        h->timer_ms[e.slot] += ms;
        h->timer_count[e.slot] += 1;
        h->ev_pool.push_back(e.a);
        if (!e.keep_b) h->ev_pool.push_back(e.b);
    }
    h->ev_pending.clear();
    return 0;
}
static int timer_event(pfslam_handle *h, hipEvent_t *e)
{
    if (h->ev_pending.size() >= 512) CHK(flush_timers(h));
    if (h->ev_pool.empty()) {
        HIPCHK(pf_event_create(e, 0));
    } else {
        *e = h->ev_pool.back();
        h->ev_pool.pop_back();
    }
    return 0;
}
static int phase_begin(pfslam_handle *h)
{
    if (h->timing < 2) return 0;
    if (h->phase_ev) h->ev_pool.push_back(h->phase_ev);
    CHK(timer_event(h, &h->phase_ev));
    HIPCHK(hipEventRecord(h->phase_ev, h->stream));
    return 0;
}
static int phase_end(pfslam_handle *h, int slot)
{
    if (h->timing < 2 || !h->phase_ev) return 0;
    hipEvent_t e = nullptr;
    CHK(timer_event(h, &e));
    HIPCHK(hipEventRecord(e, h->stream));
    h->ev_pending.push_back(pfslam_handle::TimedSpan{h->phase_ev, e, slot});
    h->phase_ev = nullptr;
    CHK(timer_event(h, &h->phase_ev));
    HIPCHK(hipEventRecord(h->phase_ev, h->stream));
    return 0;
}
extern "C" int pfslam_set_timing(pfslam_handle *h, int enable)
{
    if (!h) return fail("null handle");
    CHK(flush_timers(h));
// ... 309 lines not shown
    return 0;
}

extern "C" int pfslam_get_trace(pfslam_handle *h, int32_t out[8])
{
    if (!h || !out) return fail("pfslam_get_trace: bad argument");
    CHK(settle(h));
    memcpy(out, h->trace, sizeof(h->trace));
    return 0;
}

extern "C" int pfslam_motion_update(pfslam_handle *h, int frame)
{
    if (!h) return fail("null handle");
    HIPCHK(hipSetDevice(h->cfg.device));
    CHK(settle_staged(h));
    hipLaunchKernelGGL(k_motion, dim3((h->n + 255) / 256), dim3(256), 0, h->stream, h->x, h->y, h->th, h->w, h->wm,
                       h->n, frame, h->goff, h->trig);
    HIPCHK(hipGetLastError());
    h->theta_bound += 0.1f;
    return 0;
}

__global__ __launch_bounds__(256) void k_shift(float *__restrict__ x, float *__restrict__ y, float *__restrict__ th, int n, float dx, float dy,
                                               float dt, float *__restrict__ pose, float *__restrict__ cloud)
{
    const int i = blockIdx.x * 256 + threadIdx.x;
    if (i == 0) { pose[0] = pose[0] + dx; pose[1] = pose[1] + dy; pose[2] = pose[2] + dt; }
    if (i < 2 && cloud) {
        cloud[4 * i] += dx; cloud[4 * i + 1] += dy; cloud[4 * i + 2] += dt;
    }
    if (i >= n) return;
    x[i] = x[i] + dx;
    y[i] = y[i] + dy;
    th[i] = th[i] + dt;
}
extern "C" int pfslam_shift_particles(pfslam_handle *h, const float delta[3])
{
    if (!h || !delta) return fail("pfslam_shift_particles: bad argument");
    HIPCHK(hipSetDevice(h->cfg.device));
    CHK(join_map(h));
    if (h->pipe_live && !h->serial) {
        HIPCHK(hipEventRecord(h->ev_tail[0], h->aux));
        HIPCHK(hipStreamWaitEvent(h->stream, h->ev_tail[0], 0));
        if (!h->ftail_recorded) {
            HIPCHK(hipEventRecord(h->ev_ftail, h->fstream));
            h->ftail_recorded = true;
        }
        HIPCHK(hipStreamWaitEvent(h->stream, h->ev_ftail, 0));
    }
    const float ad = delta[2] == delta[2] ? fabsf(delta[2]) : INFINITY;
    h->theta_shift += ad;
    h->theta_bound += ad;
    h->theta_shift_seq = h->seq;
    hipLaunchKernelGGL(k_shift, dim3((h->n + 255) / 256), dim3(256), 0, h->stream, h->x, h->y, h->th, h->n, delta[0], delta[1], delta[2], h->pose,
                       h->cloud_valid ? h->cloud : (float *)nullptr);
    HIPCHK(hipGetLastError());
    if (h->pipe_live) {
        HIPCHK(hipEventRecord(h->ev_shift, h->stream));
        h->shift_pending = true;
    }
    return 0;
}

static int score_chunks(const pfslam_handle *h)
{
    const int groups = (h->n + 63) / 64;
    const int target = std::max(24576, std::min(65536, groups * 160));
    int chunks = (target + groups - 1) / groups;
    chunks = std::max(1, std::min(chunks, h->nb));
    if (!h->integral_w) chunks = 1;
    return chunks;
}

#define PF_CELLS_WALK_GRID 32
#define PF_CELLS_GRID 512
#define PF_CELLS_RECUT_EVERY 16
#define PF_CELLS_BOX_MAX 24.0f
struct CellArgs { unsigned *tab; int *list, *cs; uint4 *pool; int *rec; };
__global__ void k_cells_reset(int *cs, int list_cap, int pool_cap)
{
    if (threadIdx.x < PF_CS_WORDS)
        cs[threadIdx.x] = threadIdx.x == PF_CS_FLAGS ? PF_CF_NEED_ORIGIN : threadIdx.x == PF_CS_LIST_CAP ? list_cap : threadIdx.x == PF_CS_POOL_CAP ? pool_cap : 0;
}
static int cells_wipe(pfslam_handle *h)
{
    HIPCHK(hipMemsetAsync(h->cell_tab, 0, (size_t)PF_CELL_WIN * PF_CELL_WIN * 4, h->stream));
    static const int list_cap = getenv("PFSLAM_CELL_LIST_CAP") ? std::min(std::max(atoi(getenv("PFSLAM_CELL_LIST_CAP")), 64), PF_CELL_LIST_CAP) : PF_CELL_LIST_CAP;
    static const int pool_cap = getenv("PFSLAM_CELL_POOL_CAP") ? std::min(std::max(atoi(getenv("PFSLAM_CELL_POOL_CAP")), 64), PF_CELL_POOL_CAP) : PF_CELL_POOL_CAP;
    hipLaunchKernelGGL(k_cells_reset, dim3(1), dim3(64), 0, h->stream, h->cell_state, list_cap, pool_cap);
    HIPCHK(hipGetLastError());
    h->cells_wipe_pending = false;
    h->cells_wipe_seq = h->seq;
    h->cells_wipes++;
    h->cells_gen++;
    h->cells_passes = 0;
    return 0;
}
static int launch_cells_update(pfslam_handle *h, hipStream_t st)
{
    if (!h->cell_tab || h->cells_wipe_pending) return 0;
    const CellGeom geo{h->cfg.map_res_x, h->cfg.map_res_y, 1.0f / h->cfg.map_res_x, 1.0f / h->cfg.map_res_y};
    const int recut = h->cells_passes > 0 && h->cells_passes % PF_CELLS_RECUT_EVERY == 0 ? 1 : 0;
    if (recut) HIPCHK(hipMemsetAsync(h->cell_state + PF_CS_POOL, 0, 4, st));
    hipLaunchKernelGGL(k_cells_update<true>, dim3(PF_CELLS_GRID), dim3(64), 0, st, kd_view(h), geo, h->cell_tab, (const int *)h->cell_list, h->cell_state,
                       h->cell_pool, h->cell_rec, h->cells_gen, (const int *)h->cell_touched, (int)(h->cells_passes & 15), recut, h->cells_snap ? 1 : 0);
    h->update_unsnapped = !h->cells_snap;
    h->cells_snap = false;
    HIPCHK(hipGetLastError());
    h->cells_passes++;
    return 0;
}

static int plan_min_particles()
{
    static const int v = getenv("PFSLAM_PLAN_MIN_N") ? atoi(getenv("PFSLAM_PLAN_MIN_N")) : 4608;
    return v;
}
static bool org_use_cells(const pfslam_handle *h, bool *use_plan, bool frame_loop = false)
{
    static const bool env_min = getenv("PFSLAM_PLAN_MIN_N") != nullptr;
    const int plan_min_n = (frame_loop && !env_min) ? 65 : plan_min_particles();
    const bool organised = h->planar && h->variant != 2 && h->variant != 1 && h->n > 64 && (h->n >= plan_min_n || h->variant >= 3);
    const float Dside = h->n <= 400000 ? 64.0f : 128.0f;
    const float box_cells = 2.0f * (6.4f * h->cloud_sigma / Dside) * cbrtf(64.0f * Dside * Dside * Dside / (float)h->n) / std::min(h->cfg.map_res_x, h->cfg.map_res_y);
    const bool narrow = h->variant == 3 || !(box_cells > PF_CELLS_BOX_MAX);
    const bool use_cells = organised && h->lattice_ok && h->variant != 4 && !h->cells_suspended && narrow;
    if (use_plan) *use_plan = !use_cells && h->planar && h->variant != 2 && (h->n >= plan_min_n || h->variant >= 3);
    return use_cells;
}
__global__ void k_reduce_partials_minmax(const float *partial, int n, int chunks, const int *order, float *fit, int goff, long long *stats,
                                         const float *x, const float *y, const float *th, int p16);
__global__ void k_reduce_partials_minmax_wide(const float *partial, int n, int chunks, const int *order, float *fit, long long *stats);
template <typename T> __global__ void k_minmax(const T *fit, int n, int goff, long long *stats);
static int join_icp(pfslam_handle *h);
static int launch_stats_reset(pfslam_handle *h, hipStream_t st);

static int cells_alloc(pfslam_handle *h)
{
    CHK(dalloc(&h->cell_tab, (size_t)PF_CELL_WIN * PF_CELL_WIN));
    CHK(dalloc(&h->cell_list, (size_t)PF_CELL_LIST_CAP));
    HIPCHK(hipMemsetAsync(h->cell_list, 0, (size_t)PF_CELL_LIST_CAP * 4, h->stream));
    CHK(dalloc(&h->cell_state, PF_CS_ALLOC));
    HIPCHK(hipMemsetAsync(h->cell_state, 0, PF_CS_ALLOC * 4, h->stream));
    CHK(dalloc(&h->cell_rec, (size_t)PF_CELL_LIST_CAP * PF_REC_WORDS));
    HIPCHK(hipMemsetAsync(h->cell_rec, 0, (size_t)PF_CELL_LIST_CAP * PF_REC_WORDS * 4, h->stream));
    CHK(dalloc(&h->cell_pool, (size_t)PF_CELL_POOL_CAP + PF_ROW_SLACK));
    CHK(dalloc(&h->cell_touched, (size_t)h->max_wall + 1));
    HIPCHK(hipMemsetAsync(h->cell_touched, 0, 4, h->stream));
    HIPCHK(pf_event_create(&h->ev_boxes, hipEventDisableTiming));
    HIPCHK(pf_event_create(&h->ev_marked, hipEventDisableTiming));
    HIPCHK(pf_event_create(&h->ev_walked, hipEventDisableTiming));
    h->cells_wipe_pending = true;
    return 0;
}

static int launch_score(pfslam_handle *h, bool fuse_minmax = false, pf::KdCensus *census = nullptr, bool sharded = false)
{
    if (h->kd_size <= 0) return fail("pfslam_score_kd: no map loaded");
    const int chunks = score_chunks(h);
    const int bpc = (h->nb + chunks - 1) / chunks;
    const int used = (h->nb + bpc - 1) / bpc;
    float *out = h->fit;
    if (used > 1) {
        const size_t need = (size_t)used * h->n;
        if (need > h->partial_elems) {
            if (h->partial) HIPCHK(hipFree(h->partial));
            h->partial = nullptr;
            CHK(dalloc(&h->partial, need));
            h->partial_elems = need;
        }
        out = h->partial;
    }
    const int *order = nullptr;
    bool use_plan_ = false;
    const bool use_cells_ = org_use_cells(h, &use_plan_);
    const bool use_cells = use_cells_, use_plan = use_plan_;
    const CellGeom geo{h->cfg.map_res_x, h->cfg.map_res_y, 1.0f / h->cfg.map_res_x, 1.0f / h->cfg.map_res_y};
    if (use_cells && !h->cell_tab) CHK(cells_alloc(h));
    const bool cells_sync = use_cells && (!h->cells_async || h->cells_wipe_pending || census != nullptr);
    if (use_cells && h->cells_wipe_pending) {
        CHK(join_map(h));
        CHK(cells_wipe(h));
    }
    if (h->variant != 1 && h->n > 64) {
        const int bits = h->n <= 400000 ? 6 : PF_CELL_BITS_MAX, ncell = 1 << (3 * bits);
        int *hist = h->cells, *cursor = h->cells + ncell, *tile_tot = h->cells + 2 * ncell;
        hipLaunchKernelGGL(k_cell_count, dim3((h->n + 255) / 256), dim3(256), 0, h->stream, h->x, h->y, h->th, h->n, h->scan_reach, bits, h->mkey, hist,
                           use_cells ? h->cell_state : (int *)nullptr, geo, h->d_sigma);
        hipLaunchKernelGGL(k_cell_scan, dim3(ncell / 1024), dim3(256), 0, h->stream, hist, cursor, tile_tot);
        hipLaunchKernelGGL(k_cell_scatter, dim3((h->n + 255) / 256), dim3(256), 0, h->stream, h->mkey, h->n, cursor, tile_tot, ncell / 1024, h->order2);
        HIPCHK(hipGetLastError());
        order = h->order2;
    }
    const int direct = used > 1 ? 0 : 1;
    const bool wide_reduce = used >= 256 && fuse_minmax && !sharded && h->goff == 0;
    const bool p16 = use_cells && h->integral_w && used > 1 && fuse_minmax && !wide_reduce && (float)bpc * h->w_absmax <= 32767.0f;
    h->plan_valid = use_plan;
    h->cells_valid = use_cells;
    if (use_plan || use_cells) {
        const int groups = (h->n + 63) / 64;
        if (!h->group_box) CHK(dalloc(&h->group_box, (size_t)groups));
        if (!h->group_parts) CHK(dalloc(&h->group_parts, (size_t)groups));
        const size_t rows = (size_t)groups * h->nb;
        if (use_plan && rows > h->plan_rows) {
            if (h->plan) HIPCHK(hipFree(h->plan));
            h->plan = nullptr;
            CHK(dalloc(&h->plan, rows));
            h->plan_rows = rows;
        }
        if (h->mark_on_aux) {
            HIPCHK(hipStreamWaitEvent(h->stream, h->ev_marked, 0));
            h->mark_on_aux = false;
        }
        hipLaunchKernelGGL(k_group_box, dim3(groups), dim3(64), 0, h->stream, h->x, h->y, h->th, h->n, order, h->group_box, h->group_parts, h->d_sigma);
    }
    hipEvent_t t_a = nullptr, t_b = nullptr;
    if (h->timing && !census) {
        CHK(timer_event(h, &t_a));
        CHK(timer_event(h, &t_b));
        HIPCHK(hipEventRecord(t_a, h->stream));
    }
    const CellArgs ca{h->cell_tab, h->cell_list, h->cell_state, h->cell_pool, h->cell_rec};
    if (use_cells) {
        hipStream_t st = h->stream;
        if (!cells_sync) {
            HIPCHK(hipEventRecord(h->ev_boxes, h->stream));
            HIPCHK(hipStreamWaitEvent(h->cstream, h->ev_boxes, 0));
            st = h->cstream;
        }
        if (h->update_unsnapped) {
            HIPCHK(hipStreamWaitEvent(st, h->ev_map, 0));
            h->update_unsnapped = false;
        }
        const int groups = (h->n + 63) / 64, per_block = PF_MARK_THREADS * PF_MARK_GROUPS;
        hipLaunchKernelGGL(k_cells_mark, dim3(h->nb, (groups + per_block - 1) / per_block), dim3(PF_MARK_THREADS), 0, st,
                           (const pf::KdGroupBox *)h->group_box, groups, (const float *)h->scan, h->nb, geo, h->cell_tab, h->cell_list, h->cell_state,
                           (const pf::AngleParts *)h->group_parts, (const pf::BeamParts *)h->beam_angle);
        if (!cells_sync) {
            HIPCHK(hipEventRecord(h->ev_marked, st));
            h->mark_on_aux = true;
            HIPCHK(hipStreamWaitEvent(st, h->ev_map, 0));
            hipLaunchKernelGGL(k_cells_update<false>, dim3(PF_CELLS_WALK_GRID), dim3(64), 0, st, kd_view(h), geo, ca.tab, (const int *)ca.list, ca.cs, ca.pool, ca.rec, h->cells_gen, (const int *)nullptr, 0);
            HIPCHK(hipEventRecord(h->ev_walked, st));
            h->walk_pending = true;
            h->cells_snap = true;
        }
        HIPCHK(hipGetLastError());
    }
    const bool on_aux = h->score_on_aux && use_cells && !cells_sync && fuse_minmax && !census && !sharded;
    h->scored_on_aux = on_aux;
    struct StreamSwap {
        pfslam_handle *h;
        hipStream_t keep;
        ~StreamSwap() { h->stream = keep; }
    } swap_guard{h, h->stream};
    if (on_aux) {
        HIPCHK(hipStreamWaitEvent(h->aux, h->ev_boxes, 0));
        h->stream = h->aux;
    }
    CHK(join_map(h));
    const dim3 grid64((h->n + 63) / 64, used), grid256((h->n + 255) / 256, used);
    auto scan_match = [&](pf::KdCensus *cen) {
        if (use_cells) {
#define PF_CELLS_ARGS grid64, dim3(64), 0, h->stream, h->x, h->y, h->th, h->n, h->scan, (const pf::BeamParts *)h->beam_angle, h->nb, bpc, kd_view(h), geo, \
                      (const unsigned *)h->cell_tab, (const uint4 *)h->cell_pool, (const int *)h->cell_state, order, direct
            const bool guard = !(h->theta_bound < 0.5f * PF_SUM_THETA_MAX) || h->own_global;
            if (h->trig && cen) hipLaunchKernelGGL((k_score_kd_cells<true, PF_TRIG_DEVLIB>), PF_CELLS_ARGS, out, p16 ? 3 : 0, cen);
            else if (h->trig) hipLaunchKernelGGL((k_score_kd_cells<false, PF_TRIG_DEVLIB>), PF_CELLS_ARGS, out, p16 ? 3 : 0, (pf::KdCensus *)nullptr);
            else if (cen) hipLaunchKernelGGL((k_score_kd_cells<true, true>), PF_CELLS_ARGS, out, p16 ? 3 : 0, cen);
            else if (guard) hipLaunchKernelGGL((k_score_kd_cells<false, true>), PF_CELLS_ARGS, out, p16 ? 3 : 0, (pf::KdCensus *)nullptr);
            else hipLaunchKernelGGL((k_score_kd_cells<false, false>), PF_CELLS_ARGS, out, p16 ? 3 : 0, (pf::KdCensus *)nullptr);
#undef PF_CELLS_ARGS
        } else if (use_plan) {
            if (cen)
                hipLaunchKernelGGL((k_score_kd_plan<true>), grid64, dim3(64), 0, h->stream, h->x, h->y, h->th, h->n, h->scan, (const pf::BeamParts *)h->beam_angle, h->nb, bpc,
                                   kd_view(h), (const pf::KdPlanRow *)h->plan, order, direct, out, cen, h->trig);
            else
                hipLaunchKernelGGL((k_score_kd_plan<false>), grid64, dim3(64), 0, h->stream, h->x, h->y, h->th, h->n, h->scan, (const pf::BeamParts *)h->beam_angle, h->nb, bpc,
                                   kd_view(h), (const pf::KdPlanRow *)h->plan, order, direct, out, (pf::KdCensus *)nullptr, h->trig);
        } else if (h->planar && cen)
            hipLaunchKernelGGL((k_score_kd<true, true>), grid64, dim3(64), 0, h->stream, h->x, h->y, h->th, h->n, h->scan, (const pf::BeamParts *)h->beam_angle, h->nb, bpc,
                               kd_view(h), order, direct, out, cen, h->trig);
        else if (cen)
            hipLaunchKernelGGL((k_score_kd<false, true>), grid256, dim3(256), 0, h->stream, h->x, h->y, h->th, h->n, h->scan, (const pf::BeamParts *)h->beam_angle, h->nb, bpc,
                               kd_view(h), order, direct, out, cen, h->trig);
        else if (h->planar)
            hipLaunchKernelGGL((k_score_kd<true, false>), grid64, dim3(64), 0, h->stream, h->x, h->y, h->th, h->n, h->scan, (const pf::BeamParts *)h->beam_angle, h->nb, bpc,
                               kd_view(h), order, direct, out, (pf::KdCensus *)nullptr, h->trig);
        else
            hipLaunchKernelGGL((k_score_kd<false, false>), grid256, dim3(256), 0, h->stream, h->x, h->y, h->th, h->n, h->scan, (const pf::BeamParts *)h->beam_angle, h->nb, bpc,
                               kd_view(h), order, direct, out, (pf::KdCensus *)nullptr, h->trig);
    };
    if (use_plan || use_cells) {
        const int groups = (h->n + 63) / 64;
        if (use_cells) {
            if (cells_sync) h->cells_passes++;
            if (cells_sync)
                hipLaunchKernelGGL(k_cells_update<true>, dim3(PF_CELLS_GRID), dim3(64), 0, h->stream, kd_view(h), geo, ca.tab, (const int *)ca.list, ca.cs, ca.pool, ca.rec, h->cells_gen, (const int *)nullptr, 0, 0, 2);
            if (cells_sync) h->cells_snap = true;
        } else
            hipLaunchKernelGGL(k_plan, dim3((groups + 63) / 64, h->nb), dim3(64), 0, h->stream, (const pf::KdGroupBox *)h->group_box, groups,
                               (const float *)h->scan, h->nb, kd_view(h), h->plan);
        if (t_a) {
            hipEvent_t t_p = nullptr;
            CHK(timer_event(h, &t_p));
            HIPCHK(hipEventRecord(t_p, h->stream));
            h->ev_pending.push_back(pfslam_handle::TimedSpan{t_a, t_p, PF_T_PLAN, true});
            t_a = t_p;
        }
    }
    scan_match(census);
    HIPCHK(hipGetLastError());
    if (t_a) {
        HIPCHK(hipEventRecord(t_b, h->stream));
        h->ev_pending.push_back(pfslam_handle::TimedSpan{t_a, t_b, PF_T_SCORE});
    }
    if (h->census_log && !census && h->census_n < PF_CENSUS_LOG) {
        scan_match(h->census_log + h->census_n++);
        HIPCHK(hipGetLastError());
    }
    if (fuse_minmax) {
        if (h->icp_forked) CHK(join_icp(h));
        if (!h->stats_clean) CHK(launch_stats_reset(h, h->stream));
        h->stats_clean = false;
    }
    if (wide_reduce) {
        hipLaunchKernelGGL(k_reduce_partials_minmax_wide, dim3((h->n + 63) / 64), dim3(1024), 0, h->stream, h->partial, h->n, used, order,
                           h->fit, (long long *)h->stats);
        HIPCHK(hipGetLastError());
    } else if (used > 1 && fuse_minmax) {
#define PF_REDUCE4_WGS 128
        hipLaunchKernelGGL(k_reduce_partials_minmax, dim3(std::min((h->n + 255) / 256, PF_REDUCE4_WGS)), dim3(256), 0, h->stream, h->partial, h->n,
                           used, order, h->fit, h->goff, (long long *)h->stats, h->x, h->y, h->th, p16 ? 1 : 0);
        HIPCHK(hipGetLastError());
    } else {
        if (used > 1) {
            hipLaunchKernelGGL(k_reduce_partials, dim3((h->n + 255) / 256), dim3(256), 0, h->stream, h->partial, h->n,
                               used, order, h->fit);
            HIPCHK(hipGetLastError());
        }
        if (fuse_minmax) {
            const int blocks = std::min(1024, (h->n + 255) / 256);
            hipLaunchKernelGGL(k_minmax<float>, dim3(blocks), dim3(256), 0, h->stream, (const float *)h->fit, h->n, h->goff, (long long *)h->stats);
            HIPCHK(hipGetLastError());
        }
    }
    return 0;
}

extern "C" int pfslam_score_census(pfslam_handle *h, unsigned long long out[8])
{
    if (!h || !out) return fail("pfslam_score_census: bad argument");
    HIPCHK(hipSetDevice(h->cfg.device));
    CHK(settle_staged(h));
    if (!h->d_census) CHK(dalloc(&h->d_census, 1));
    HIPCHK(hipMemsetAsync(h->d_census, 0, sizeof(pf::KdCensus), h->stream));
    CHK(launch_score(h, false, h->d_census));
    pf::KdCensus c;
    HIPCHK(hipMemcpyAsync(&c, h->d_census, sizeof(c), hipMemcpyDeviceToHost, h->stream));
    HIPCHK(hipStreamSynchronize(h->stream));
    out[0] = c.trips; out[1] = c.lanes; out[2] = c.tests; out[3] = c.test_lanes; out[4] = c.uniform; out[5] = c.prefix; out[6] = c.redesc; out[7] = c.redesc_noop;
    return 0;
}

extern "C" int pfslam_set_census(pfslam_handle *h, int enable)
{
    if (!h) return fail("null handle");
    HIPCHK(hipSetDevice(h->cfg.device));
    CHK(settle(h));
    HIPCHK(hipStreamSynchronize(h->stream));
    if (enable) {
        if (!h->census_store) CHK(dalloc(&h->census_store, (size_t)PF_CENSUS_LOG));
        HIPCHK(hipMemsetAsync(h->census_store, 0, sizeof(pf::KdCensus) * PF_CENSUS_LOG, h->stream));
        HIPCHK(hipStreamSynchronize(h->stream));
        h->census_n = 0;
    }
    h->census_log = enable ? h->census_store : nullptr;
    return 0;
}
extern "C" int pfslam_get_census_log(pfslam_handle *h, unsigned long long *out, int cap, int *n)
{
// ... 133 lines not shown
#endif
    return 0;
}

__global__ __launch_bounds__(256) void k_cells_check(pf::KdView tree, const unsigned *__restrict__ tab, const int *__restrict__ list, const int *__restrict__ cs,
                                                     const uint4 *__restrict__ pool, const int *__restrict__ rec_base, int gen, unsigned long long *__restrict__ out)
{
    const int count = min(cs[PF_CS_COUNT], cs[PF_CS_LIST_CAP]);
    unsigned long long c[16] = {0};
    for (int r = blockIdx.x * 256 + threadIdx.x; r < count; r += gridDim.x * 256) {
        const int *rec = rec_base + (size_t)r * PF_REC_WORDS;
        const int cell = list[r];
        c[0]++;
        const unsigned w0 = tab[cell];
        if (rec[3] != gen) { c[1]++; if (w0 != PF_CELL_PENDING) c[8]++; continue; }
        const int m = rec[2] & 0xff, fl = rec[2] >> 16;
        if (fl & PF_RF_FRESH) { c[2]++; if (w0 != PF_CELL_PENDING) c[9]++; continue; }
        const unsigned wd[4] = {w0, tab[cell + 1], tab[cell + PF_CELL_WIN], tab[cell + PF_CELL_WIN + 1]};
        if (fl & PF_RF_DEAD) {
            c[7]++;
            for (int b = 0; b < 4; b++) if (wd[b] != PF_CELL_FALLBACK || (unsigned)rec[PF_REC_LAST + b] != wd[b]) c[14]++;
            continue;
        }
        c[3]++;
        const int p0 = rec[PF_REC_POOL], plen = rec[PF_REC_POOL + 1];
        for (int b = 0; b < 4; b++) {
            if ((unsigned)rec[PF_REC_LAST + b] != wd[b]) { c[10]++; continue; }
            if (wd[b] == PF_CELL_FALLBACK) continue;
            if (wd[b] == 0u || wd[b] >= 0x40000000u) { c[9]++; continue; }
            const int n1 = (int)(wd[b] & 15u), n2 = (int)((wd[b] >> 4) & 15u), off = (int)(wd[b] >> 8);
            if (off < p0 || off + n1 + (n2 == 15 ? 0 : n2) > p0 + plen || n1 < 1) { c[10]++; continue; }
            int pos = 0;
            for (int k = 0; k < n1; k++) {
                const int node = (int)(pool[off + k].z & 0x3fffffffu);
                while (pos < m && rec[PF_REC_CAND + pos] != node) pos++;
                if (pos == m) { c[11]++; break; }
                pos++;
            }
        }
        if (rec[1] < 0 || watched_child(tree, rec[1]) >= 0) c[12]++;
        if (!(fl & PF_RF_ROVER))
            for (int k = 0; k < m; k++) {
                const int ct = rec[PF_REC_TERM + k];
                if (ct < -1) c[13]++;
                else if (ct >= 0 && watched_child(tree, ct) >= 0) c[12]++;
            }
    }
    for (size_t i = (size_t)blockIdx.x * 256 + threadIdx.x; i < (size_t)PF_CELL_WIN * PF_CELL_WIN; i += (size_t)gridDim.x * 256) {
        const unsigned w = tab[i];
        if (w == 0u) continue;
        if (w == PF_CELL_PENDING) c[5]++;
        else if (w == PF_CELL_FALLBACK) c[6]++;
        else c[4]++;
    }
    for (int k = 0; k < 15; k++) {
        unsigned long long v = c[k];
        for (int off = 32; off >= 1; off >>= 1) v += __shfl_xor(v, off, 64);
        if ((threadIdx.x & 63) == 0 && v) atomicAdd(&out[k], v);
    }
}
extern "C" int pfslam_debug_check_cells(pfslam_handle *h, long long out[16])
{
    if (!h || !out) return fail("pfslam_debug_check_cells: bad argument");
    for (int k = 0; k < 16; k++) out[k] = 0;
    if (!h->cell_tab || !h->cells_valid || h->cells_wipe_pending) return 0;
    HIPCHK(hipSetDevice(h->cfg.device));
    CHK(settle(h));
    unsigned long long *d = nullptr;
    CHK(dalloc(&d, 16));
    HIPCHK(hipMemsetAsync(d, 0, 128, h->stream));
    hipLaunchKernelGGL(k_cells_check, dim3(2048), dim3(256), 0, h->stream, kd_view(h), (const unsigned *)h->cell_tab, (const int *)h->cell_list,
                       (const int *)h->cell_state, (const uint4 *)h->cell_pool, (const int *)h->cell_rec, h->cells_gen, d);
    HIPCHK(hipGetLastError());
    int cs[PF_CS_WORDS];
    HIPCHK(hipMemcpyAsync(out, d, 128, hipMemcpyDeviceToHost, h->stream));
    HIPCHK(hipMemcpyAsync(cs, h->cell_state, sizeof(cs), hipMemcpyDeviceToHost, h->stream));
    HIPCHK(hipStreamSynchronize(h->stream));
    HIPCHK(hipFree(d));
    if (!(cs[PF_CS_FLAGS] & (PF_CF_LIST_FULL | PF_CF_POOL_FULL)))
        out[15] = (out[4] != cs[PF_CS_ROWS]) + (out[6] != cs[PF_CS_NONE]) + (out[5] != out[1] + out[2]);
    return 0;
}

extern "C" int pfslam_set_probe(pfslam_handle *h, int frames)
{
    if (!h || frames < 0 || frames > 4096) return fail("pfslam_set_probe: 0 .. 4096 frames");
    HIPCHK(hipSetDevice(h->cfg.device));
    CHK(settle(h));
    HIPCHK(hipStreamSynchronize(h->stream));
    if (h->probe) HIPCHK(hipFree(h->probe));
    h->probe = nullptr;
    h->probe_frames = 0;
    if (frames > 0) {
        CHK(dalloc(&h->probe, (size_t)frames * PF_PROBE_SLOTS));
        HIPCHK(hipMemset(h->probe, 0, (size_t)frames * PF_PROBE_SLOTS * 8));
        h->probe_frames = frames;
    }
    return 0;
}
extern "C" int pfslam_get_probe(pfslam_handle *h, unsigned long long *out, int cap_frames, int *n_frames, int *last_ticket)
{
    if (!h || !n_frames || (cap_frames > 0 && !out)) return fail("pfslam_get_probe: bad argument");
    *n_frames = 0;
    if (last_ticket) *last_ticket = h->seq;
    if (!h->probe) return 0;
    HIPCHK(hipSetDevice(h->cfg.device));
    CHK(settle(h));
    HIPCHK(hipStreamSynchronize(h->stream));
    const int n = std::min(std::min(cap_frames, h->probe_frames), h->seq);
    std::vector<unsigned long long> all((size_t)h->probe_frames * PF_PROBE_SLOTS);
    HIPCHK(hipMemcpy(all.data(), h->probe, all.size() * 8, hipMemcpyDeviceToHost));
    for (int k = 0; k < n; k++) {
        const int ticket = h->seq - n + 1 + k;
        memcpy(out + (size_t)k * PF_PROBE_SLOTS, &all[(size_t)(ticket % h->probe_frames) * PF_PROBE_SLOTS], PF_PROBE_SLOTS * 8);
    }
    *n_frames = n;
    return 0;
}
extern "C" int pfslam_frame_mode(pfslam_handle *h, int out[4])
{
    if (!h || !out) return fail("pfslam_frame_mode: bad argument");
    out[0] = h->pipe_live ? 1 : 0;
    out[1] = h->pipe_live ? (h->gates_live ? 1 : 0) : h->gates;
    out[2] = h->serial;
    out[3] = h->publish_lag;
    return 0;
}
extern "C" const char *pfslam_probe_name(int slot) { return slot >= 0 && slot < PB_END ? pb_names[slot] : ""; }
extern "C" int pfslam_set_trig(pfslam_handle *h, int devlib)
{
    if (!h || devlib < 0 || devlib > 1) return fail("pfslam_set_trig: 0 (specification) or 1 (device library)");
    HIPCHK(hipSetDevice(h->cfg.device));
    CHK(settle(h));
    h->trig = devlib;
    return 0;
}
extern "C" int pfslam_set_serial(pfslam_handle *h, int serial)
{
    if (!h) return fail("null handle");
    HIPCHK(hipSetDevice(h->cfg.device));
    CHK(settle(h));
    HIPCHK(hipStreamSynchronize(h->stream));
    h->serial = serial != 0;
    h->pipe_live = false;
    return 0;
}

__global__ __launch_bounds__(256) void k_ubench_gather(const unsigned *__restrict__ table, int n_rec, int iters, unsigned *__restrict__ out)
{
    const pf::kd_rsrc_t r = pf::kd_rsrc(table);
    const unsigned gid = blockIdx.x * 256 + threadIdx.x;
    unsigned state = (gid >> 6) * 2654435761u + 12345u, acc = 0;
    for (int it = 0; it < iters; it++) {
        int idx[8];
#pragma unroll
        for (int k = 0; k < 8; k++) {
            state = state * 1664525u + 1013904223u;
            idx[k] = (int)((state >> 8) & (unsigned)(n_rec - 1));
        }
#pragma unroll
        for (int k = 0; k < 8; k++) {
            const uint4 v = pf::kd_load_hot(r, idx[k]);
            acc += v.x ^ v.y ^ v.z ^ v.w;
        }
    }
    out[gid] = acc;
// ... 127 lines not shown
```

### gpu-icp-slam_amd/csrc/pfslam_stages.hip.inc

```

__device__ __forceinline__ long long wave_max_i64(long long v)
{
    for (int off = 32; off >= 1; off >>= 1) {
        long long o = __shfl_xor(v, off, 64);
        v = o > v ? o : v;
    }
    return v;
}
__device__ __forceinline__ float wave_max_f32(float v)
{
    for (int off = 32; off >= 1; off >>= 1) v = fmaxf(v, __shfl_xor(v, off, 64));
    return v;
}
template <typename F>
__device__ __forceinline__ float wave_sum_canonical(int n, F elem)
{
    const int lane = threadIdx.x & 63;
    float acc = 0.0f;
    for (int i = lane; i < n; i += 64) acc = acc + elem(i);
    for (int off = 32; off >= 1; off >>= 1) acc = acc + __shfl_xor(acc, off, 64);
    return acc;
}

__device__ __forceinline__ int f32_to_ordered(float f)
// ... 534 lines not shown
        long long kmax, kmin;
        frame_keys(s.stats, s.gkeys, s.world, kmax, kmin);
        const uint32_t best = 0xFFFFFFFFu - (uint32_t)(kmax & 0xFFFFFFFFll);
        const uint32_t r = best / (uint32_t)s.stride, j = best - r * (uint32_t)s.stride;
        const bool ok = r < (uint32_t)s.world;
        const float *blk = s.gpose + (size_t)(ok ? r : 0u) * 3 * s.stride;
        start[0] = ok ? blk[j] : 0.0f;
        start[1] = ok ? blk[s.stride + j] : 0.0f;
        start[2] = ok ? blk[2 * s.stride + j] : 0.0f;
    } else {
        const uint32_t best = 0xFFFFFFFFu - (uint32_t)(s.stats[0] & 0xFFFFFFFFll);
        const bool mine = best < (uint32_t)s.n;
        start[0] = mine ? s.x[best] : 0.0f;
        start[1] = mine ? s.y[best] : 0.0f;
        start[2] = mine ? s.th[best] : 0.0f;
    }
    pose[0] = start[0] + s.icp[24];
    pose[1] = start[1] + s.icp[25];
    pose[2] = start[2] + s.icp[27];
}
__global__ __launch_bounds__(256) void k_get_walls(const float *__restrict__ scan, int nb, const float *__restrict__ pose,
                                                   int cx, int cy, uint8_t *__restrict__ free_mask,
                                                   uint8_t *__restrict__ wall_mask, int dimx, int dimy, float resx, float resy,
                                                   int centre_from_pose, PoseSrc src = PoseSrc{nullptr, nullptr, nullptr, nullptr, nullptr, 0, nullptr, nullptr, 1, 0},
                                                   int trig = 0)
{
    const int i = blockIdx.x * 4 + (threadIdx.x >> 6);
    const int lane = threadIdx.x & 63;
    if (i >= nb) return;
    float ps[3], st[3];
    if (src.stats) frame_pose(src, st, ps);
    else { ps[0] = pose[0]; ps[1] = pose[1]; ps[2] = pose[2]; }
    if (centre_from_pose) {
        cx = (int)roundf(0.5f * (float)dimx + pf::fdiv(ps[0], resx) + resx / 2);
        cy = (int)roundf(0.5f * (float)dimy + pf::fdiv(ps[1], resy) + resy / 2);
    }
    float wx, wy;
    pf::clean_lidar_scan(i, scan[i], ps[2], wx, wy, trig);
    if (fabsf(wx) < PF_LIDAR_RANGE && fabsf(wy) < PF_LIDAR_RANGE) {
        wx = roundf(pf::fdiv(wx, resx));
        wy = roundf(pf::fdiv(wy, resy));
        wx += (float)cx;
        wy += (float)cy;
        trace_ray_wave(cx, cy, (int)wx, (int)wy, dimx, dimy, free_mask, lane);
        if (lane == 0 && wx >= 0 && wx < dimx && wy >= 0 && wy < dimy) wall_mask[(int)(wx * dimx + wy)] = 1;
    }
}

__device__ __forceinline__ int popcount_bytes16(const uint4 v)
{
    return __popc(v.x) + __popc(v.y) + __popc(v.z) + __popc(v.w);
}

__global__ __launch_bounds__(256) void k_count_cells(const uint8_t *__restrict__ free_mask, const uint8_t *__restrict__ wall_mask,
                                                     int M, int *__restrict__ blk_cnt)
{
    const int base = (blockIdx.x * 256 + threadIdx.x) * 16;
    int cw = 0, cf = 0;
    if (base + 16 <= M) {
        cw = popcount_bytes16(*(const uint4 *)(wall_mask + base));
        cf = popcount_bytes16(*(const uint4 *)(free_mask + base));
    } else {
        for (int k = base; k < M; k++) {
            cw += wall_mask[k] != 0;
            cf += free_mask[k] != 0;
        }
    }
    for (int off = 32; off >= 1; off >>= 1) {
        cw += __shfl_xor(cw, off, 64);
        cf += __shfl_xor(cf, off, 64);
    }
    __shared__ int sw[4], sf[4];
    if ((threadIdx.x & 63) == 0) {
        sw[threadIdx.x >> 6] = cw;
        sf[threadIdx.x >> 6] = cf;
    }
    __syncthreads();
    if (threadIdx.x == 0) {
        blk_cnt[2 * blockIdx.x] = sw[0] + sw[1] + sw[2] + sw[3];
        blk_cnt[2 * blockIdx.x + 1] = sf[0] + sf[1] + sf[2] + sf[3];
    }
}

__device__ __forceinline__ float4 cell_to_point(int idx, int dimx, float resx, float resy, float scalex, float scaley,
                                                float rx, float ry)
{
    const int cx = idx / dimx, cy = idx - cx * dimx;
    float px = (float)cx * resx - scalex / 2.0f + rx;
    float py = (float)cy * resy - scaley / 2.0f + ry;
    px = roundf(pf::fdiv(px, resx)) * resx;
    py = roundf(pf::fdiv(py, resy)) * resy;
    return make_float4(px, py, 0.0f, 0.0f);
}

__global__ __launch_bounds__(256) void k_scatter_cells(uint8_t *free_mask, uint8_t *wall_mask,
                                                       int M, const int *__restrict__ blk_cnt, int *__restrict__ counts, int dimx, float resx, float resy,
                                                       float scalex, float scaley, const float *__restrict__ pose,
                                                       int *__restrict__ wall_cell, float4 *__restrict__ wall_pts, int wall_cap,
                                                       int *__restrict__ free_cell, float4 *__restrict__ free_pts, int free_cap, int clear,
                                                       PoseSrc src = PoseSrc{nullptr, nullptr, nullptr, nullptr, nullptr, 0, nullptr, nullptr, 1, 0})
{
    const int base = (blockIdx.x * 256 + threadIdx.x) * 16;
    uint8_t mw[16], mf[16];
    int cw = 0, cf = 0;
    if (base + 16 <= M) {
        const uint4 vw = *(const uint4 *)(wall_mask + base), vf = *(const uint4 *)(free_mask + base);
        if (clear) {
            if (vw.x | vw.y | vw.z | vw.w) *(uint4 *)(wall_mask + base) = make_uint4(0, 0, 0, 0);
            if (vf.x | vf.y | vf.z | vf.w) *(uint4 *)(free_mask + base) = make_uint4(0, 0, 0, 0);
        }
        const uint32_t ww[4] = {vw.x, vw.y, vw.z, vw.w}, wf[4] = {vf.x, vf.y, vf.z, vf.w};
#pragma unroll
        for (int k = 0; k < 16; k++) {
            mw[k] = (ww[k >> 2] >> (8 * (k & 3))) & 0xff;
            mf[k] = (wf[k >> 2] >> (8 * (k & 3))) & 0xff;
            cw += mw[k] != 0;
            cf += mf[k] != 0;
        }
    } else {
        for (int k = 0; k < 16; k++) {
            const bool in = base + k < M;
            mw[k] = in ? wall_mask[base + k] : 0;
            mf[k] = in ? free_mask[base + k] : 0;
            cw += mw[k] != 0;
            cf += mf[k] != 0;
            if (clear && in) wall_mask[base + k] = free_mask[base + k] = 0;
        }
    }
    const int lane = threadIdx.x & 63, wave = threadIdx.x >> 6;
    int iw = cw, jf = cf;
    for (int off = 1; off < 64; off <<= 1) {
        const int a = __shfl_up(iw, off, 64), b = __shfl_up(jf, off, 64);
        if (lane >= off) {
            iw += a;
            jf += b;
        }
    }
    __shared__ int sw[4], sf[4];
    if (lane == 63) {
        sw[wave] = iw;
        sf[wave] = jf;
    }
    int pw = 0, pfr = 0;
    for (int b = threadIdx.x; b < (int)blockIdx.x; b += 256) {
        pw += blk_cnt[2 * b];
        pfr += blk_cnt[2 * b + 1];
    }
    for (int off = 32; off >= 1; off >>= 1) {
        pw += __shfl_xor(pw, off, 64);
        pfr += __shfl_xor(pfr, off, 64);
    }
    __shared__ int spw[4], spf[4];
    if (lane == 0) {
        spw[wave] = pw;
        spf[wave] = pfr;
    }
    __syncthreads();
    const int base_w = spw[0] + spw[1] + spw[2] + spw[3], base_f = spf[0] + spf[1] + spf[2] + spf[3];
    if (blockIdx.x == gridDim.x - 1 && threadIdx.x == 0) {
        counts[0] = base_w + sw[0] + sw[1] + sw[2] + sw[3];
        counts[1] = base_f + sf[0] + sf[1] + sf[2] + sf[3];
    }
    __shared__ unsigned short lw[4096], lf[4096];
    int ow = iw - cw, of = jf - cf;
    for (int k = 0; k < wave; k++) {
        ow += sw[k];
        of += sf[k];
    }
    const int tw = sw[0] + sw[1] + sw[2] + sw[3], tf = sf[0] + sf[1] + sf[2] + sf[3];
    if (tw == 0 && tf == 0) return;
    const int local = threadIdx.x * 16;
#pragma unroll
    for (int k = 0; k < 16; k++) {
        if (mw[k]) lw[ow++] = (unsigned short)(local + k);
        if (mf[k]) lf[of++] = (unsigned short)(local + k);
// ... 1964 lines not shown
```

### include/pfslam.h

```cpp
#ifndef PFSLAM_H
#define PFSLAM_H

#include <stddef.h>
#include <stdint.h>

#ifdef __cplusplus
extern "C" {
#endif

typedef struct pfslam_node {
    int32_t axis, left, right, parent;
    float x, y, z, w;
} pfslam_node;

typedef struct pfslam_particle {
    float x, y, theta, w;
    uint8_t cluster;
    uint8_t pad_[7];
    void *map;
} pfslam_particle;

typedef struct pfslam_config {
    int32_t n_particles;
    int32_t n_beams;
// ... 8 lines not shown
    int32_t global_n;
    int32_t shard_stride;
    int32_t reserved_[2];
} pfslam_config;

typedef struct pfslam_handle pfslam_handle;

void pfslam_default_config(pfslam_config *cfg);
int pfslam_create(const pfslam_config *cfg, pfslam_handle **out);
int pfslam_destroy(pfslam_handle *h);
const char *pfslam_last_error(void);
int pfslam_device_count(void);
int pfslam_set_stream(pfslam_handle *h, void *hip_stream);
int pfslam_synchronize(pfslam_handle *h);

int pfslam_step(pfslam_handle *h, int frame, const float *scan_host);
int pfslam_set_lag(pfslam_handle *h, int frames);
int pfslam_step_grid(pfslam_handle *h, int frame, const float *scan_host);

int pfslam_get_pose(pfslam_handle *h, float pose[3]);
int pfslam_get_particles(pfslam_handle *h, const pfslam_particle **out, int *n);
int pfslam_get_map(pfslam_handle *h, const pfslam_node **out, int *n);
int pfslam_get_grid(pfslam_handle *h, const int8_t **grid, int *dimx, int *dimy);
int pfslam_get_trace(pfslam_handle *h, int32_t out[8]);
int pfslam_get_cells(pfslam_handle *h, int which, int32_t *out, int cap, int *n);

int pfslam_set_map(pfslam_handle *h, const pfslam_node *nodes, int n);
int pfslam_set_particles(pfslam_handle *h, const pfslam_particle *p, int n);
int pfslam_set_scan(pfslam_handle *h, const float *scan_host, int n_beams);
int pfslam_set_pose(pfslam_handle *h, const float pose[3]);
int pfslam_set_grid(pfslam_handle *h, const int8_t *grid, int dimx, int dimy);

int pfslam_motion_update(pfslam_handle *h, int frame);
int pfslam_shift_particles(pfslam_handle *h, const float delta[3]);
int pfslam_score_kd(pfslam_handle *h, float *fit_host);
int pfslam_measurement_update(pfslam_handle *h, int *best, float *fmin, float *fmax);
int pfslam_icp(pfslam_handle *h, const float start[3], float pose_out[3], float *dbg29);
int pfslam_update_map_kd(pfslam_handle *h);
int pfslam_resample(pfslam_handle *h, int frame, int *resampled, float *neff);
int pfslam_resample_plan(pfslam_handle *h, int frame, int *resampled, float *neff);
int pfslam_resample_gather(pfslam_handle *h);
int pfslam_score_grid(pfslam_handle *h, int32_t *fit_host);
int pfslam_update_map_grid(pfslam_handle *h);

int pfslam_traverse(pfslam_handle *h, const float *xyz_host, int n, int32_t *best_host);

int pfslam_set_topology(pfslam_handle *h, int enable);
int pfslam_get_closures(pfslam_handle *h, int32_t *pairs, int cap, int *n);
int pfslam_topology_update(pfslam_handle *h, int *n_nodes);
int pfslam_find_walls(pfslam_handle *h, const float a_xy[2], const float b_xy[2], int *n_walls);
int pfslam_check_loop_closure(pfslam_handle *h, int32_t *pairs, int cap, int *n);
int pfslam_get_topology(pfslam_handle *h, float *nodes_xyd, int cap, int *n, int *node_idx);

int pfslam_maybe_balance(pfslam_handle *h, int frame);
int pfslam_kd_size(pfslam_handle *h);

int pfslam_shard_disperse(pfslam_handle *h, int frame, const float *scan_host, int *seeded);
int pfslam_shard_score(pfslam_handle *h);
int pfslam_shard_weights(pfslam_handle *h);
int pfslam_shard_finish(pfslam_handle *h);
int pfslam_shard_stream(pfslam_handle *h, int which, void **hip_stream);
int pfslam_set_shard_balance(pfslam_handle *h, int external);
int pfslam_shard_balance_due(pfslam_handle *h, int frame, int *due, int *n_nodes);
int pfslam_shard_balance_build(pfslam_handle *h, int frame);
int pfslam_shard_balance_adopt(pfslam_handle *h);
int pfslam_measurement_local(pfslam_handle *h);
int pfslam_measurement_apply(pfslam_handle *h, int *best_global, float *fmin, float *fmax);
int pfslam_device_ptr(pfslam_handle *h, int which, void **ptr, size_t *bytes);

int pfslam_time_score_kd(pfslam_handle *h, int iters, float *ms_per_launch);
int pfslam_set_timing(pfslam_handle *h, int enable);
int pfslam_get_timers(pfslam_handle *h, double out[12]);
int pfslam_score_census(pfslam_handle *h, unsigned long long out[8]);
int pfslam_set_census(pfslam_handle *h, int enable);
int pfslam_get_census_log(pfslam_handle *h, unsigned long long *out, int cap, int *n);
int pfslam_ubench_gather(pfslam_handle *h, double out[4]);
int pfslam_plan_stats(pfslam_handle *h, double out[10]);
int pfslam_cell_stats(pfslam_handle *h, double out[16]);
int pfslam_time_score_grid(pfslam_handle *h, int iters, float *ms_kernel, float *ms_pass);
int pfslam_set_variant(pfslam_handle *h, int variant);
int pfslam_set_trig(pfslam_handle *h, int devlib);
int pfslam_set_serial(pfslam_handle *h, int serial);
int pfslam_debug_check_cells(pfslam_handle *h, long long out[16]);
int pfslam_set_probe(pfslam_handle *h, int frames);
int pfslam_get_probe(pfslam_handle *h, unsigned long long *out, int cap_frames, int *n_frames, int *last_ticket);
const char *pfslam_probe_name(int slot);
int pfslam_frame_mode(pfslam_handle *h, int out[4]);

int pfslam_kd_create(const float *pts_xyzw, int n, pfslam_node *out);
int pfslam_kd_insert_list(const float *pts_xyzw, int n, pfslam_node *list, int idx, int parent);
int pfslam_kd_insert_node(const float p[4], pfslam_node *list, int list_size);
int pfslam_kd_balance(pfslam_node *list, int n);
int pfslam_kd_parallel_sort(void);
int pfslam_kd_sort_threads(void);
void pfslam_kd_whole_node(int on);

#ifdef __cplusplus
}
#endif
#endif
```

Before: 174.2 million particle-scan evals/s.

## Memoize per-cell nearest KD node to seed wall-point traversal

During the cell walk, each cell record now tracks the nearest tree node to its corner and stores it with its distance in a new memo slot. A new cell map indexes records by lattice coordinate. The wall rank/traverse kernel looks up that memo and resumes the KD search from the stored best instead of descending from the root. This cuts tree traversal work for wall points in map update. In exchange it adds a memo store per walk, a map memset on wipe, counters, and a debug checker, and it relies on the memo staying valid for the current generation.

Result: no change. 174.7 million particle-scan evals/s, median of 4 (+0.3%).

```diff
diff --git a/gpu-icp-slam_amd/binding.py b/gpu-icp-slam_amd/binding.py
--- a/gpu-icp-slam_amd/binding.py
+++ b/gpu-icp-slam_amd/binding.py
@@ -23,7 +23,7 @@
     "pfslam_measurement_apply", "pfslam_device_ptr", "pfslam_time_score_kd", "pfslam_set_variant", "pfslam_set_lag",
     "pfslam_kd_create", "pfslam_kd_insert_list", "pfslam_kd_insert_node", "pfslam_kd_balance", "pfslam_set_timing", "pfslam_get_timers", "pfslam_resample_plan", "pfslam_resample_gather", "pfslam_maybe_balance", "pfslam_kd_size", "pfslam_topology_update", "pfslam_find_walls",
     "pfslam_check_loop_closure", "pfslam_get_topology", "pfslam_set_topology", "pfslam_get_closures", "pfslam_score_census", "pfslam_set_census", "pfslam_get_census_log", "pfslam_ubench_gather", "pfslam_plan_stats", "pfslam_cell_stats", "pfslam_kd_parallel_sort", "pfslam_kd_sort_threads", "pfslam_kd_whole_node",
-    "pfslam_set_serial", "pfslam_set_trig", "pfslam_debug_check_cells", "pfslam_set_probe", "pfslam_get_probe", "pfslam_probe_name", "pfslam_frame_mode",
+    "pfslam_set_serial", "pfslam_set_trig", "pfslam_debug_check_cells", "pfslam_debug_wall_memo", "pfslam_set_probe", "pfslam_get_probe", "pfslam_probe_name", "pfslam_frame_mode",
     "pfslam_time_score_grid", "pfslam_set_shard_balance", "pfslam_shard_balance_due", "pfslam_shard_balance_build", "pfslam_shard_balance_adopt",
 ]
 
@@ -134,6 +134,7 @@
     L.pfslam_set_serial.argtypes = [vp, i32]
     L.pfslam_set_trig.argtypes = [vp, i32]
     L.pfslam_debug_check_cells.argtypes = [vp, vp]
+    L.pfslam_debug_wall_memo.argtypes = [vp, vp]
     L.pfslam_set_probe.argtypes = [vp, i32]
     L.pfslam_get_probe.argtypes = [vp, vp, i32, vp, vp]
     L.pfslam_frame_mode.argtypes = [vp, vp]
@@ -482,6 +483,11 @@
         d["violations"] = sum(v for k, v in d.items() if k.startswith("v_"))
         return d
 
+    def wall_memo(self):
+        out = (C.c_longlong * 4)()
+        _chk(self.L.pfslam_debug_wall_memo(self._h, out), "pfslam_debug_wall_memo")
+        return dict(zip(("walls_memo", "walls_generic", "checked", "differing"), [int(v) for v in out]))
+
     def set_trig(self, devlib):
         _chk(self.L.pfslam_set_trig(self._h, 1 if devlib else 0), "pfslam_set_trig")
 
diff --git a/gpu-icp-slam_amd/csrc/kd_cells.hip.inc b/gpu-icp-slam_amd/csrc/kd_cells.hip.inc
--- a/gpu-icp-slam_amd/csrc/kd_cells.hip.inc
+++ b/gpu-icp-slam_amd/csrc/kd_cells.hip.inc
@@ -11,7 +11,8 @@
 #define PF_CELL_FALLBACK 0xFFFFFFFEu
 enum { PF_CS_COUNT = 0, PF_CS_POOL, PF_CS_SNAP, PF_CS_PAD3, PF_CS_LIST_CAP, PF_CS_POOL_CAP, PF_CS_FLAGS, PF_CS_PAD, PF_CS_ROWS, PF_CS_N1, PF_CS_N2,
        PF_CS_NONE, PF_CS_CUR_FRESH, PF_CS_CUR_EXT, PF_CS_CUR_REUSED, PF_CS_CUR_CLAIMED, PF_CS_WORDS = 32,
-       PF_CS_OX = 128, PF_CS_OY = 129, PF_CS_ALLOC = 256 };
+       PF_CS_OX = 128, PF_CS_OY = 129,
+       PF_CS_WALL_MEMO = 192, PF_CS_WALL_GENERIC = 193, PF_CS_ALLOC = 256 };
 #define PF_CF_LIST_FULL 1
 #define PF_CF_POOL_FULL 2
 #define PF_CF_NEED_ORIGIN 4
@@ -25,6 +26,8 @@
 #define PF_REC_POOL 76
 #define PF_REC_LAST 80
 #define PF_ROW_HEADROOM 2
+#define PF_REC_MEMO 84
+#define PF_CELL_MAP_SIDE (PF_CELL_WIN / PF_CELL_SUB)
 #define PF_RF_FRESH 1
 #define PF_RF_DEAD 2
 #define PF_RF_ROVER 4
@@ -204,7 +207,30 @@
 #define PF_CORNER_F 0.999996f
 #define PF_CELL_MAXU 16
 #define PF_CELL_MAXRU 24
-static_assert(PF_REC_RC + PF_CELL_MAXRU <= PF_REC_POOL && PF_REC_POOL + 2 <= PF_REC_LAST && PF_REC_LAST + 4 <= PF_REC_WORDS && PF_REC_CAND == PF_REC_TERM + PF_CELL_MAXU && PF_REC_PAR == PF_REC_CAND + PF_CELL_MAXU && PF_REC_RC == PF_REC_PAR + PF_CELL_MAXU, "record layout");
+static_assert(PF_REC_RC + PF_CELL_MAXRU <= PF_REC_POOL && PF_REC_POOL + 2 <= PF_REC_LAST && PF_REC_LAST + 4 <= PF_REC_MEMO && PF_REC_MEMO + 2 <= PF_REC_WORDS && PF_REC_MEMO / 32 == PF_REC_POOL / 32 && PF_REC_CAND == PF_REC_TERM + PF_CELL_MAXU && PF_REC_PAR == PF_REC_CAND + PF_CELL_MAXU && PF_REC_RC == PF_REC_PAR + PF_CELL_MAXU, "record layout");
+__device__ __forceinline__ float cell_dist2(const uint4 cd, float wx, float wy)
+{
+    typedef float f32x2 __attribute__((ext_vector_type(2)));
+    const f32x2 nxy = {__uint_as_float(cd.x), __uint_as_float(cd.y)};
+    const f32x2 pxy = {wx, wy};
+    const f32x2 d = nxy - pxy;
+    const f32x2 dd = d * d;
+    return dd.x + dd.y;
+}
+__device__ __forceinline__ bool cell_visit(const uint4 cd, float wx, float wy, float &sBest)
+{
+    const float s = cell_dist2(cd, wx, wy);
+    const float sGuard = sBest * PF_GUARD_K;
+    bool take = s < sGuard;
+    const bool inBand = (s < sBest) != take;
+    if (__builtin_amdgcn_ballot_w64(inBand) != 0ull) {
+        float sb = sBest;
+        asm volatile("" : "+v"(sb));
+        take = take | (inBand && pf::fsqrt(s) < pf::fsqrt(sb));
+    }
+    sBest = take ? s : sBest;
+    return take;
+}
 __device__ __forceinline__ int link_child(const pf::KdView &t, int link)
 {
     const int a = link >> 1;
@@ -237,7 +263,7 @@
 struct CellPass { const int *lo; int *w_out; const int *hi; const int *bound; int fault; };
 template <bool PUBLISH>
 __global__ __launch_bounds__(64) void k_cells_update(pf::KdView tree, CellGeom geo, unsigned *tab, const int *__restrict__ list, int *cs,
-                                                     uint4 *__restrict__ pool, int *rec_base, int gen, const int *__restrict__ touched, int pass = 0, int recut = 0, int use_snap = 0,
+                                                     uint4 *__restrict__ pool, int *rec_base, int *__restrict__ cell_map, int gen, const int *__restrict__ touched, int pass = 0, int recut = 0, int use_snap = 0,
                                                      CellPass cp = CellPass{nullptr, nullptr, nullptr, nullptr, 0}, unsigned long long *__restrict__ probe = nullptr,
                                                      int *__restrict__ signal_word = nullptr, int signal_ticket = 0)
 {
@@ -312,6 +338,7 @@
         int4 pre_ct[4], pre_cand[4], pre_par[4], pre_rc[6];
         int2 pre_pool = make_int2(0, 0);
         int4 pre_last = make_int4(0, 0, 0, 0);
+        int2 pre_memo = make_int2(0, 0);
         int pre_cell = 0;
         constexpr bool HOIST = PUBLISH;
         if (HOIST) {
@@ -330,6 +357,7 @@
                 for (int q = 0; q < 6; q++) pre_rc[q] = *(const int4 *)(rec + PF_REC_RC + 4 * q);
                 pre_pool = *(const int2 *)(rec + PF_REC_POOL);
                 pre_last = *(const int4 *)(rec + PF_REC_LAST);
+                pre_memo = *(const int2 *)(rec + PF_REC_MEMO);
                 pre_cell = list[r];
             }
         }
@@ -414,6 +442,13 @@
         }
         int head = !active ? -1 : scratch ? 0 : child0;
         bool give_up = false;
+        float sBestP = INFINITY;
+        int bestP = 0;
+        if (active && !scratch) {
+            const int2 mm = HOIST ? pre_memo : *(const int2 *)(rec + PF_REC_MEMO);
+            sBestP = __int_as_float(mm.x);
+            bestP = mm.y;
+        }
         uint4 nd = tree.hot[max(head, 0)];
         while (head >= 0) {
             int cl = pf::hot_left(nd.z), cr = (int)nd.w;
@@ -425,6 +460,7 @@
             const float nx = __uint_as_float(nd.x), ny = __uint_as_float(nd.y);
             const uint32_t axis = nd.z >> 30;
             if (!(fabsf(nx) < 1e6f && fabsf(ny) < 1e6f)) { give_up = true; break; }
+            if (cell_visit(nd, cxlo, cylo, sBestP)) bestP = head;
             float lb, ub;
             bounds(cxlo, cxhi, cylo, cyhi, nx, ny, lb, ub);
             U = fminf(U, ub);
@@ -649,6 +685,7 @@
                 rec[PF_REC_PAR + k] = S_PI(k);
             }
             for (int k = 0; k < nr; k++) rec[PF_REC_RC + k] = S_R(k);
+            *(int2 *)(rec + PF_REC_MEMO) = make_int2(__float_as_int(sBestP), dead ? -1 : bestP);
             if (!PUBLISH) rec[PF_REC_POOL] = rec[PF_REC_POOL + 1] = 0;
         }
         PF_STAMP(5);
@@ -775,6 +812,7 @@
         }
 #pragma unroll
         for (int b4 = 0; b4 < 4; b4++) __hip_atomic_store(&tab[cell + (b4 & 1) + ((b4 & 2) ? PF_CELL_WIN : 0)], word[b4], __ATOMIC_RELAXED, __HIP_MEMORY_SCOPE_AGENT);
+        if (cell_map && (scratch || (rflags & PF_RF_FRESH))) cell_map[(cyw >> 1) * PF_CELL_MAP_SIDE + (cxw >> 1)] = r + 1;
         PF_STAMP(8);
     }
 #ifdef PF_CELLS_PROFILE
@@ -812,30 +850,27 @@
 #undef S_R
 #undef S_RX
 #undef S_RY
-__device__ __forceinline__ float cell_dist2(const uint4 cd, float wx, float wy)
-{
-    typedef float f32x2 __attribute__((ext_vector_type(2)));
-    const f32x2 nxy = {__uint_as_float(cd.x), __uint_as_float(cd.y)};
-    const f32x2 pxy = {wx, wy};
-    const f32x2 d = nxy - pxy;
-    const f32x2 dd = d * d;
-    return dd.x + dd.y;
-}
-__device__ __forceinline__ bool cell_visit(const uint4 cd, float wx, float wy, float &sBest)
-{
-    const float s = cell_dist2(cd, wx, wy);
-    const float sGuard = sBest * PF_GUARD_K;
-    bool take = s < sGuard;
-    const bool inBand = (s < sBest) != take;
-    if (__builtin_amdgcn_ballot_w64(inBand) != 0ull) {
-        float sb = sBest;
-        asm volatile("" : "+v"(sb));
-        take = take | (inBand && pf::fsqrt(s) < pf::fsqrt(sb));
-    }
-    sBest = take ? s : sBest;
-    return take;
-}
 
+struct WallMemo { const int *map; const int *rec; const int *cs; int gen; };
+__device__ __forceinline__ int wall_memo_record(const WallMemo &wm, int kx, int ky)
+{
+    if (!wm.map) return 0;
+    const int wx = kx - (wm.cs[PF_CS_OX] >> 1), wy = ky - (wm.cs[PF_CS_OY] >> 1);
+    if ((unsigned)wx >= (unsigned)PF_CELL_MAP_SIDE || (unsigned)wy >= (unsigned)PF_CELL_MAP_SIDE) return 0;
+    return wm.map[wy * PF_CELL_MAP_SIDE + wx];
+}
+__device__ __forceinline__ bool wall_memo_get(const WallMemo &wm, int r1, float &sBest, int &best, int &leaf)
+{
+    if (r1 <= 0) return false;
+    const int *rec = wm.rec + (size_t)(r1 - 1) * PF_REC_WORDS;
+    const int4 hd = *(const int4 *)rec;
+    const int2 mm = *(const int2 *)(rec + PF_REC_MEMO);
+    if (hd.w != wm.gen || ((hd.z >> 16) & (PF_RF_FRESH | PF_RF_DEAD)) != 0 || hd.y < 0 || mm.y < 0) return false;
+    sBest = __int_as_float(mm.x);
+    best = mm.y;
+    leaf = hd.y;
+    return true;
+}
 #define PF_ROW_SLACK 4
 template <bool CENSUS = false, int GUARD = 1>
 __global__ __launch_bounds__(64) void k_score_kd_cells(const float *__restrict__ px, const float *__restrict__ py,
diff --git a/gpu-icp-slam_amd/csrc/pfslam_frame.hip.inc b/gpu-icp-slam_amd/csrc/pfslam_frame.hip.inc
--- a/gpu-icp-slam_amd/csrc/pfslam_frame.hip.inc
+++ b/gpu-icp-slam_amd/csrc/pfslam_frame.hip.inc
@@ -469,7 +469,8 @@
 __global__ __launch_bounds__(64) void k_walls_rank_traverse(const uint32_t *__restrict__ runs_g, int sort_n, const float *__restrict__ pose, int dimx, float resx,
                                                             float resy, float scalex, float scaley, pf::KdView tree, uint32_t *__restrict__ keys_s,
                                                             float2 *__restrict__ xy_s, int *__restrict__ c2_s, int *__restrict__ leaf_s,
-                                                            int *__restrict__ new_s, unsigned long long *__restrict__ probe, int split)
+                                                            int *__restrict__ new_s, unsigned long long *__restrict__ probe, int split, WallMemo wm,
+                                                            int *__restrict__ wall_counts)
 {
     pf_stamp(probe);
     extern __shared__ uint32_t s_dyn[];
@@ -481,41 +482,60 @@
     const int i = mine * 64 + pos;
     const uint32_t key = runs[i];
     if (key == 0xFFFFFFFFu) return;
+    float kxf, kyf;
+    const float4 p = cell_to_point_k((int)key, dimx, resx, resy, scalex, scaley, pose[0], pose[1], kxf, kyf);
+    const int r1 = (PLANAR && fabsf(kxf) < (float)PF_LATTICE_KMAX && fabsf(kyf) < (float)PF_LATTICE_KMAX) ? wall_memo_record(wm, (int)kxf, (int)kyf) : 0;
     int rank = pos;
     bool dup = pos > 0 && runs[i - 1] == key;
-    for (int r0 = 0; r0 < n_runs; r0 += 4) {
-        int lo[4] = {0, 0, 0, 0};
-        uint32_t pk[4];
-        bool on[4];
-#pragma unroll
-        for (int u = 0; u < 4; u++) {
-            const int r = r0 + u;
-            on[u] = r < n_runs && r != mine && !(r > mine && key == 0u);
-            pk[u] = r < mine ? key : key - 1u;
-        }
-#pragma unroll
-        for (int step = 32; step >= 1; step >>= 1)
+    auto searches = [&](int r_begin, int r_end) {
+        for (int r0 = r_begin; r0 < r_end; r0 += 4) {
+            int lo[4] = {0, 0, 0, 0};
+            uint32_t pk[4];
+            bool on[4];
+#pragma unroll
+            for (int u = 0; u < 4; u++) {
+                const int r = r0 + u;
+                on[u] = r < n_runs && r != mine && !(r > mine && key == 0u);
+                pk[u] = r < mine ? key : key - 1u;
+            }
+#pragma unroll
+            for (int step = 32; step >= 1; step >>= 1)
+#pragma unroll
+                for (int u = 0; u < 4; u++)
+                    if (on[u]) lo[u] += (runs[(r0 + u) * 64 + lo[u] + step - 1] <= pk[u]) ? step : 0;
 #pragma unroll
             for (int u = 0; u < 4; u++)
-                if (on[u]) lo[u] += (runs[(r0 + u) * 64 + lo[u] + step - 1] <= pk[u]) ? step : 0;
-#pragma unroll
-        for (int u = 0; u < 4; u++)
-            if (on[u]) {
-                const int cnt = lo[u] + ((lo[u] == 63 && runs[(r0 + u) * 64 + 63] <= pk[u]) ? 1 : 0);
-                rank += cnt;
-                if (r0 + u < mine && cnt > 0 && runs[(r0 + u) * 64 + cnt - 1] == key) dup = true;
-            }
-    }
+                if (on[u]) {
+                    const int cnt = lo[u] + ((lo[u] == 63 && runs[(r0 + u) * 64 + 63] <= pk[u]) ? 1 : 0);
+                    rank += cnt;
+                    if (r0 + u < mine && cnt > 0 && runs[(r0 + u) * 64 + cnt - 1] == key) dup = true;
+                }
+        }
+    };
+    searches(0, min(8, n_runs));
+    float sBest = INFINITY;
+    int best = 0, head = 0, leaf_memo = -1;
+    const bool memo = PLANAR && wall_memo_get(wm, r1, sBest, best, leaf_memo);
+    if (memo) head = -1;
+    searches(min(8, n_runs), n_runs);
     if (dup) return;
-    const float4 p = cell_to_point((int)key, dimx, resx, resy, scalex, scaley, pose[0], pose[1]);
     int leaf;
-    const int b = pf::kd_resume<PLANAR, false, true>(tree, p.x, p.y, p.z, INFINITY, 0, 0, nullptr, &leaf);
+    const int b = pf::kd_resume<PLANAR, false, true>(tree, p.x, p.y, p.z, sBest, best, head, nullptr, &leaf);
+    if (memo) leaf = leaf_memo;
     const float cellDiag = pf::fsqrt(resx * resx + resy * resy), minDist = cellDiag / 2.0f;
     keys_s[rank] = key;
     xy_s[rank] = make_float2(p.x, p.y);
     c2_s[rank] = b;
     leaf_s[rank] = leaf;
     new_s[rank] = node_dist(tree, b, p) > minDist ? 1 : 0;
+    if (wall_counts) {
+        const int n_memo = __popcll(__ballot(memo)), n_gen = __popcll(__ballot(!memo));
+        const unsigned long long act = __ballot(true);
+        if (lane == __ffsll((long long)act) - 1) {
+            if (n_memo) atomicAdd(&wall_counts[0], n_memo);
+            if (n_gen) atomicAdd(&wall_counts[1], n_gen);
+        }
+    }
 }
 
 template <bool PLANAR>
@@ -1081,11 +1101,11 @@
     if (c.sync_cells) {
         h->cells_passes++;
         hipLaunchKernelGGL(k_cells_update<true>, dim3(PF_CELLS_GRID), dim3(64), 0, K, c.tv, c.geo, h->cell_tab, (const int *)h->cell_list, h->cell_state, h->cell_pool,
-                           h->cell_rec, h->cells_gen, (const int *)nullptr, 0, 0, 0, CellPass{nullptr, nullptr, nullptr, nullptr, 0}, PB(PB_WALK));
+                           h->cell_rec, h->cell_map, h->cells_gen, (const int *)nullptr, 0, 0, 0, CellPass{nullptr, nullptr, nullptr, nullptr, 0}, PB(PB_WALK));
         hipLaunchKernelGGL(k_fs_walked, dim3(1), dim3(64), 0, K, h->fs, (const int *)h->cell_state);
     } else {
         hipLaunchKernelGGL(k_cells_update<false>, dim3(PF_CELLS_WALK_GRID), dim3(64), 0, K, c.tv, c.geo, h->cell_tab, (const int *)h->cell_list, h->cell_state,
-                           h->cell_pool, h->cell_rec, h->cells_gen, (const int *)nullptr, 0, 0, 0,
+                           h->cell_pool, h->cell_rec, h->cell_map, h->cells_gen, (const int *)nullptr, 0, 0, 0,
                            CellPass{h->fs + PF_FS_WALKED + ((seq - 1) & 3), h->fs + PF_FS_WALKED + s4, nullptr, h->fs + PF_FS_BOUND + s4, 0}, PB(PB_WALK));
     }
     HIPCHK(hipGetLastError());
@@ -1290,7 +1310,8 @@
             const int walls_split = 4;
             hipLaunchKernelGGL(k_walls_rank_traverse<true>, dim3(sort_n / 64 * walls_split), dim3(64), (size_t)sort_n * 4, C, (const uint32_t *)h->wall_runs, sort_n,
                                (const float *)h->pose, h->dimx, h->cfg.map_res_x, h->cfg.map_res_y, h->cfg.map_scale_x, h->cfg.map_scale_y, c.tv, h->wall_keys_s,
-                               h->wall_xy2, h->wall_c2s, h->wall_leaf2, h->wall_new2, PB(PB_WALLS_REP), walls_split);
+                               h->wall_xy2, h->wall_c2s, h->wall_leaf2, h->wall_new2, PB(PB_WALLS_REP), walls_split,
+                               WallMemo{(const int *)h->cell_map, (const int *)h->cell_rec, (const int *)h->cell_state, h->cells_gen}, h->cell_state + PF_CS_WALL_MEMO);
             hipLaunchKernelGGL(k_walls<3>, PF_WALLS_ARGS, PB(PB_WALLS), h->wall_xy2, h->wall_leaf2, h->wall_new2, (int *)nullptr, seq, (int *)nullptr,
                                (const uint32_t *)h->wall_keys_s, (const int *)h->wall_c2s);
         }
@@ -1300,7 +1321,7 @@
         const int recut = h->cells_passes > 0 && h->cells_passes % PF_CELLS_RECUT_EVERY == 0 ? 1 : 0;
         if (recut) HIPCHK(hipMemsetAsync(h->cell_state + PF_CS_POOL, 0, 4, C));
         hipLaunchKernelGGL(k_cells_update<true>, dim3(PF_CELLS_GRID), dim3(64), 0, C, c.tv, c.geo, h->cell_tab, (const int *)h->cell_list, h->cell_state, h->cell_pool,
-                           h->cell_rec, h->cells_gen, (const int *)h->cell_touched, (int)(h->cells_passes & 15), recut, 0,
+                           h->cell_rec, h->cell_map, h->cells_gen, (const int *)h->cell_touched, (int)(h->cells_passes & 15), recut, 0,
                            CellPass{nullptr, nullptr, h->fs + PF_FS_WALKED + ((seq - (sync_cells ? 0 : lag)) & 3), nullptr, h->fault}, PB(PB_UPDATE),
                            gates ? fl + PF_FL_TREE : (int *)nullptr, seq);
         HIPCHK(hipGetLastError());
diff --git a/gpu-icp-slam_amd/csrc/pfslam_hip.hip b/gpu-icp-slam_amd/csrc/pfslam_hip.hip
--- a/gpu-icp-slam_amd/csrc/pfslam_hip.hip
+++ b/gpu-icp-slam_amd/csrc/pfslam_hip.hip
@@ -178,6 +178,7 @@
     bool cells_valid = false;
     unsigned *cell_tab = nullptr;
     int *cell_list = nullptr, *cell_state = nullptr, *cell_rec = nullptr;
+    int *cell_map = nullptr;
     int *cell_touched = nullptr;
     uint4 *cell_pool = nullptr;
     bool cells_wipe_pending = false;
@@ -921,6 +922,7 @@
     if (h->cell_state) (void)hipFree(h->cell_state);
     if (h->cell_pool) (void)hipFree(h->cell_pool);
     if (h->cell_rec) (void)hipFree(h->cell_rec);
+    if (h->cell_map) (void)hipFree(h->cell_map);
     if (h->cell_touched) (void)hipFree(h->cell_touched);
     if (h->ev_boxes) (void)hipEventDestroy(h->ev_boxes);
     if (h->ev_marked) (void)hipEventDestroy(h->ev_marked);
@@ -1396,10 +1398,12 @@
 {
     if (threadIdx.x < PF_CS_WORDS)
         cs[threadIdx.x] = threadIdx.x == PF_CS_FLAGS ? PF_CF_NEED_ORIGIN : threadIdx.x == PF_CS_LIST_CAP ? list_cap : threadIdx.x == PF_CS_POOL_CAP ? pool_cap : 0;
+    if (threadIdx.x == 0) cs[PF_CS_WALL_MEMO] = cs[PF_CS_WALL_GENERIC] = 0;
 }
 static int cells_wipe(pfslam_handle *h)
 {
     HIPCHK(hipMemsetAsync(h->cell_tab, 0, (size_t)PF_CELL_WIN * PF_CELL_WIN * 4, h->stream));
+    HIPCHK(hipMemsetAsync(h->cell_map, 0, (size_t)PF_CELL_MAP_SIDE * PF_CELL_MAP_SIDE * 4, h->stream));
     static const int list_cap = getenv("PFSLAM_CELL_LIST_CAP") ? std::min(std::max(atoi(getenv("PFSLAM_CELL_LIST_CAP")), 64), PF_CELL_LIST_CAP) : PF_CELL_LIST_CAP;
     static const int pool_cap = getenv("PFSLAM_CELL_POOL_CAP") ? std::min(std::max(atoi(getenv("PFSLAM_CELL_POOL_CAP")), 64), PF_CELL_POOL_CAP) : PF_CELL_POOL_CAP;
     hipLaunchKernelGGL(k_cells_reset, dim3(1), dim3(64), 0, h->stream, h->cell_state, list_cap, pool_cap);
@@ -1418,7 +1422,7 @@
     const int recut = h->cells_passes > 0 && h->cells_passes % PF_CELLS_RECUT_EVERY == 0 ? 1 : 0;
     if (recut) HIPCHK(hipMemsetAsync(h->cell_state + PF_CS_POOL, 0, 4, st));
     hipLaunchKernelGGL(k_cells_update<true>, dim3(PF_CELLS_GRID), dim3(64), 0, st, kd_view(h), geo, h->cell_tab, (const int *)h->cell_list, h->cell_state,
-                       h->cell_pool, h->cell_rec, h->cells_gen, (const int *)h->cell_touched, (int)(h->cells_passes & 15), recut, h->cells_snap ? 1 : 0);
+                       h->cell_pool, h->cell_rec, h->cell_map, h->cells_gen, (const int *)h->cell_touched, (int)(h->cells_passes & 15), recut, h->cells_snap ? 1 : 0);
     h->update_unsnapped = !h->cells_snap;
     h->cells_snap = false;
     HIPCHK(hipGetLastError());
@@ -1459,6 +1463,7 @@
     HIPCHK(hipMemsetAsync(h->cell_state, 0, PF_CS_ALLOC * 4, h->stream));
     CHK(dalloc(&h->cell_rec, (size_t)PF_CELL_LIST_CAP * PF_REC_WORDS));
     HIPCHK(hipMemsetAsync(h->cell_rec, 0, (size_t)PF_CELL_LIST_CAP * PF_REC_WORDS * 4, h->stream));
+    CHK(dalloc(&h->cell_map, (size_t)PF_CELL_MAP_SIDE * PF_CELL_MAP_SIDE));
     CHK(dalloc(&h->cell_pool, (size_t)PF_CELL_POOL_CAP + PF_ROW_SLACK));
     CHK(dalloc(&h->cell_touched, (size_t)h->max_wall + 1));
     HIPCHK(hipMemsetAsync(h->cell_touched, 0, 4, h->stream));
@@ -1555,7 +1560,7 @@
             HIPCHK(hipEventRecord(h->ev_marked, st));
             h->mark_on_aux = true;
             HIPCHK(hipStreamWaitEvent(st, h->ev_map, 0));
-            hipLaunchKernelGGL(k_cells_update<false>, dim3(PF_CELLS_WALK_GRID), dim3(64), 0, st, kd_view(h), geo, ca.tab, (const int *)ca.list, ca.cs, ca.pool, ca.rec, h->cells_gen, (const int *)nullptr, 0);
+            hipLaunchKernelGGL(k_cells_update<false>, dim3(PF_CELLS_WALK_GRID), dim3(64), 0, st, kd_view(h), geo, ca.tab, (const int *)ca.list, ca.cs, ca.pool, ca.rec, h->cell_map, h->cells_gen, (const int *)nullptr, 0);
             HIPCHK(hipEventRecord(h->ev_walked, st));
             h->walk_pending = true;
             h->cells_snap = true;
@@ -1611,7 +1616,7 @@
         if (use_cells) {
             if (cells_sync) h->cells_passes++;
             if (cells_sync)
-                hipLaunchKernelGGL(k_cells_update<true>, dim3(PF_CELLS_GRID), dim3(64), 0, h->stream, kd_view(h), geo, ca.tab, (const int *)ca.list, ca.cs, ca.pool, ca.rec, h->cells_gen, (const int *)nullptr, 0, 0, 2);
+                hipLaunchKernelGGL(k_cells_update<true>, dim3(PF_CELLS_GRID), dim3(64), 0, h->stream, kd_view(h), geo, ca.tab, (const int *)ca.list, ca.cs, ca.pool, ca.rec, h->cell_map, h->cells_gen, (const int *)nullptr, 0, 0, 2);
             if (cells_sync) h->cells_snap = true;
         } else
             hipLaunchKernelGGL(k_plan, dim3((groups + 63) / 64, h->nb), dim3(64), 0, h->stream, (const pf::KdGroupBox *)h->group_box, groups,
@@ -1911,6 +1916,59 @@
     return 0;
 }
 
+__global__ __launch_bounds__(256) void k_wall_memo_check(pf::KdView tree, CellGeom geo, const int *__restrict__ list, WallMemo wm, unsigned long long *__restrict__ out)
+{
+    const int count = min(wm.cs[PF_CS_COUNT], wm.cs[PF_CS_LIST_CAP]);
+    const int ox = wm.cs[PF_CS_OX], oy = wm.cs[PF_CS_OY];
+    unsigned long long c[2] = {0ull, 0ull};
+    for (int r = blockIdx.x * 256 + threadIdx.x; r < count; r += gridDim.x * 256) {
+        const int *rec = wm.rec + (size_t)r * PF_REC_WORDS;
+        if (rec[3] != wm.gen || ((rec[2] >> 16) & (PF_RF_FRESH | PF_RF_DEAD)) != 0) continue;
+        const int cell = list[r], cyw = cell / PF_CELL_WIN, cxw = cell - cyw * PF_CELL_WIN;
+        const float kxf = (float)((ox + cxw) >> 1), kyf = (float)((oy + cyw) >> 1);
+        const float px = kxf * geo.resx, py = kyf * geo.resy;
+        c[0]++;
+        const int r1 = wall_memo_record(wm, (int)kxf, (int)kyf);
+        float sBest = INFINITY;
+        int best = 0, leaf = -1, b = -1;
+        const bool ok = r1 == r + 1 && wall_memo_get(wm, r1, sBest, best, leaf);
+        if (ok) b = pf::kd_resume<true>(tree, px, py, 0.0f, sBest, best, -1);
+        int leaf_ref = -1;
+        const int b_ref = pf::kd_resume<true, false, true>(tree, px, py, 0.0f, INFINITY, 0, 0, nullptr, &leaf_ref);
+        if (!ok || b != b_ref || leaf != leaf_ref) c[1]++;
+    }
+    for (int k = 0; k < 2; k++) {
+        unsigned long long v = c[k];
+        for (int off = 32; off >= 1; off >>= 1) v += __shfl_xor(v, off, 64);
+        if ((threadIdx.x & 63) == 0 && v) atomicAdd(&out[k], v);
+    }
+}
+extern "C" int pfslam_debug_wall_memo(pfslam_handle *h, long long out[4])
+{
+    if (!h || !out) return fail("pfslam_debug_wall_memo: bad argument");
+    for (int k = 0; k < 4; k++) out[k] = 0;
+    if (!h->cell_tab || !h->cells_valid || h->cells_wipe_pending) return 0;
+    HIPCHK(hipSetDevice(h->cfg.device));
+    CHK(settle(h));
+    unsigned long long *d = nullptr;
+    CHK(dalloc(&d, 2));
+    HIPCHK(hipMemsetAsync(d, 0, 16, h->stream));
+    if (h->planar) {
+        const CellGeom geo{h->cfg.map_res_x, h->cfg.map_res_y, 1.0f / h->cfg.map_res_x, 1.0f / h->cfg.map_res_y};
+        hipLaunchKernelGGL(k_wall_memo_check, dim3(512), dim3(256), 0, h->stream, kd_view(h), geo, (const int *)h->cell_list,
+                           WallMemo{(const int *)h->cell_map, (const int *)h->cell_rec, (const int *)h->cell_state, h->cells_gen}, d);
+        HIPCHK(hipGetLastError());
+    }
+    int wc[2];
+    HIPCHK(hipMemcpyAsync(out + 2, d, 16, hipMemcpyDeviceToHost, h->stream));
+    HIPCHK(hipMemcpyAsync(wc, h->cell_state + PF_CS_WALL_MEMO, 8, hipMemcpyDeviceToHost, h->stream));
+    HIPCHK(hipStreamSynchronize(h->stream));
+    HIPCHK(hipFree(d));
+    out[0] = wc[0];
+    out[1] = wc[1];
+    return 0;
+}
+
 extern "C" int pfslam_set_probe(pfslam_handle *h, int frames)
 {
     if (!h || frames < 0 || frames > 4096) return fail("pfslam_set_probe: 0 .. 4096 frames");
diff --git a/gpu-icp-slam_amd/csrc/pfslam_stages.hip.inc b/gpu-icp-slam_amd/csrc/pfslam_stages.hip.inc
--- a/gpu-icp-slam_amd/csrc/pfslam_stages.hip.inc
+++ b/gpu-icp-slam_amd/csrc/pfslam_stages.hip.inc
@@ -640,15 +640,21 @@
     }
 }
 
+__device__ __forceinline__ float4 cell_to_point_k(int idx, int dimx, float resx, float resy, float scalex, float scaley,
+                                                  float rx, float ry, float &kx, float &ky)
+{
+    const int cx = idx / dimx, cy = idx - cx * dimx;
+    const float px = (float)cx * resx - scalex / 2.0f + rx;
+    const float py = (float)cy * resy - scaley / 2.0f + ry;
+    kx = roundf(pf::fdiv(px, resx));
+    ky = roundf(pf::fdiv(py, resy));
+    return make_float4(kx * resx, ky * resy, 0.0f, 0.0f);
+}
 __device__ __forceinline__ float4 cell_to_point(int idx, int dimx, float resx, float resy, float scalex, float scaley,
                                                 float rx, float ry)
 {
-    const int cx = idx / dimx, cy = idx - cx * dimx;
-    float px = (float)cx * resx - scalex / 2.0f + rx;
-    float py = (float)cy * resy - scaley / 2.0f + ry;
-    px = roundf(pf::fdiv(px, resx)) * resx;
-    py = roundf(pf::fdiv(py, resy)) * resy;
-    return make_float4(px, py, 0.0f, 0.0f);
+    float kx, ky;
+    return cell_to_point_k(idx, dimx, resx, resy, scalex, scaley, rx, ry, kx, ky);
 }
 
 __global__ __launch_bounds__(256) void k_scatter_cells(uint8_t *free_mask, uint8_t *wall_mask,
diff --git a/include/pfslam.h b/include/pfslam.h
--- a/include/pfslam.h
+++ b/include/pfslam.h
@@ -114,6 +114,7 @@
 int pfslam_set_trig(pfslam_handle *h, int devlib);
 int pfslam_set_serial(pfslam_handle *h, int serial);
 int pfslam_debug_check_cells(pfslam_handle *h, long long out[16]);
+int pfslam_debug_wall_memo(pfslam_handle *h, long long out[4]);
 int pfslam_set_probe(pfslam_handle *h, int frames);
 int pfslam_get_probe(pfslam_handle *h, unsigned long long *out, int cap_frames, int *n_frames, int *last_ticket);
 const char *pfslam_probe_name(int slot);
```
